# wyf-ACCEPT/BackToReality

Measured on NVIDIA B200. Metric: Pointnet2Backbone fwd+bwd scenes/sec @40k pts, higher is better.
Workload: dtype tf32 fwd / bf16 bwd operands, f32 accumulate

## Files before the change

### backtoreality_b200/_lib.py

```python
import ctypes
import os

_HERE = os.path.dirname(os.path.abspath(__file__))
LIB_PATH = os.environ.get("B2R_LIB") or os.path.join(_HERE, "libb2r.so")

_vp = ctypes.c_void_p
_i = ctypes.c_int
_f = ctypes.c_float
_ip = ctypes.POINTER(ctypes.c_int)

SIGNATURES = {
    "b2r_version": [],
    "b2r_status_string": [_i],
    "b2r_last_error": [],
    "b2r_struct_bytes": [_i],
    "b2r_ref_block_threads": [_i],
    "b2r_fps": [_vp, _i, _i, _i, _vp, _vp],
    "b2r_fps_ex": [_vp, _i, _i, _i, _vp, _i, _vp],
    "b2r_fps_plan": [_i, _i, _ip, _ip, _ip, _ip],
    "b2r_fps_workspace_bytes": [_i, _i],
    "b2r_fps_ws": [_vp, _i, _i, _i, _vp, _i, _vp, ctypes.c_longlong, _vp],
    "b2r_fps_sort": [_vp, _i, _i, _vp, ctypes.c_longlong, _vp],
    "b2r_fps_ws_presorted": [_vp, _i, _i, _i, _vp, _i, _vp, ctypes.c_longlong, _vp],
    "b2r_gather_fwd": [_vp, _vp, _i, _i, _i, _i, _vp, _vp],
    "b2r_gather_bwd": [_vp, _vp, _i, _i, _i, _i, _vp, _vp],
    "b2r_ball_query": [_vp, _vp, _i, _i, _i, _f, _i, _vp, _vp],
    "b2r_ball_query_workspace_bytes": [_i, _i],
    "b2r_ball_query_grid": [_vp, _vp, _i, _i, _i, _f, _i, _vp, _vp, ctypes.c_longlong, _vp],
    "b2r_group_fwd": [_vp, _vp, _i, _i, _i, _i, _i, _vp, _vp],
    "b2r_group_bwd": [_vp, _vp, _i, _i, _i, _i, _i, _vp, _vp],
    "b2r_three_nn": [_vp, _vp, _i, _i, _i, _vp, _vp, _vp],
    "b2r_three_interp_fwd": [_vp, _vp, _vp, _i, _i, _i, _i, _vp, _vp],
    "b2r_three_interp_bwd": [_vp, _vp, _vp, _i, _i, _i, _i, _vp, _vp],
    "b2r_scatter_plan_bytes": [_i, ctypes.c_longlong, _i, _i, _i],
    "b2r_scatter_plan": [_vp, _vp, _i, ctypes.c_longlong, _i, _i, _vp, ctypes.c_longlong, _vp],
    "b2r_group_bwd_plan": [_vp, _vp, _i, _i, _i, _i, _i, _vp, _vp],
    "b2r_three_interp_bwd_plan": [_vp, _vp, _i, _i, _i, _i, _vp, _vp],
    "b2r_adam_state_bytes": [],
    "b2r_adam_flat_step": [_vp, _vp, _vp, _vp, ctypes.c_longlong, _vp, _f, _f, _f, _f, _f, _f, _vp],
    "b2r_nn_argmin": [_vp, _vp, _i, _i, _i, _i, _i, _f, _vp, _vp, _vp],
    "b2r_query_group_fwd": [_vp, _vp, _vp, _vp, _i, _i, _i, _i, _i, _f, _i, _vp, _vp],
    "b2r_query_group_bwd": [_vp, _vp, _i, _i, _i, _i, _i, _f, _i, _vp, _vp, _vp, _vp],
}
_RESTYPES = {"b2r_status_string": ctypes.c_char_p, "b2r_last_error": ctypes.c_char_p,
             "b2r_fps_workspace_bytes": ctypes.c_longlong,
             "b2r_scatter_plan_bytes": ctypes.c_longlong,
             "b2r_ball_query_workspace_bytes": ctypes.c_longlong,
             "b2r_mlp_weight_image_bytes": ctypes.c_longlong}


class SaLayer(ctypes.Structure):
    _fields_ = [
        ("B", _i), ("N", _i), ("NP", _i), ("NS", _i), ("Cin", _i), ("Cout", _i),
        ("mode", _i), ("epilogue", _i),
        ("xyz", _vp), ("new_xyz", _vp), ("feat_t", _vp), ("idx", _vp),
        ("radius", _f), ("normalize_xyz", _i),
        ("z_prev", _vp), ("scale_prev", _vp), ("shift_prev", _vp),
        ("w_image", _vp), ("z", _vp), ("stats", _vp),
        ("zmax", _vp), ("zmin", _vp), ("amax", _vp), ("amin", _vp),
        ("sm_limit", _i),
        ("cidx", _vp), ("ccen", _vp), ("cmeta", _vp),
    ]


SIGNATURES.update({
    "b2r_mlp_weight_image_bytes": [_i, _i, _i],
    "b2r_mlp_pack_weight": [_vp, _i, _i, _i, _vp, _vp],
    "b2r_sa_layer_fwd": [ctypes.POINTER(SaLayer), _vp],
    "b2r_sa_layer_fwd_supported": [_i, _i, _i, _i, _i, _i, _i],
    "b2r_bn_finalize": [_vp, _i, ctypes.c_double, _vp, _vp, _f, _f, _vp, _vp, _vp, _vp, _vp, _vp,
                        _vp, _vp],
    "b2r_pool_finalize": [_vp, _vp, _vp, _vp, _i, _i, _i, _vp, _vp, _vp],
    "b2r_to_point_major": [_vp, _i, _i, _i, _vp, _vp],
})



class SaLayerBwd(ctypes.Structure):
    _fields_ = [
        ("B", _i), ("N", _i), ("NP", _i), ("NS", _i), ("Cin", _i), ("Cout", _i), ("mode", _i),
        ("xyz", _vp), ("new_xyz", _vp), ("feat_t", _vp), ("idx", _vp),
        ("radius", _f), ("normalize_xyz", _i),
        ("z_prev", _vp), ("scale_prev", _vp), ("shift_prev", _vp),
        ("w_image_bf16", _vp), ("dz", _vp), ("gr", _vp), ("z", _vp),
        ("dysel", _vp), ("asel", _vp),
        ("coef_a", _vp), ("coef_b", _vp), ("coef_c", _vp),
        ("dW", _vp), ("gr_prev", _vp), ("stats_prev", _vp),
        ("g_feat_t", _vp), ("g_xyz", _vp), ("g_new_xyz", _vp),
        ("sm_limit", _i),
        ("cidx", _vp), ("ccen", _vp), ("cmeta", _vp),
    ]


SIGNATURES.update({
    "b2r_mlp_weight_bf16_image_bytes": [_i, _i, _i],
    "b2r_mlp_pack_weight_bf16": [_vp, _i, _i, _i, _vp, _vp],
    "b2r_sa_layer_bwd": [ctypes.POINTER(SaLayerBwd), _vp],
    "b2r_sa_layer_bwd_supported": [_i, _i, _i, _i, _i, _i, _i],
    "b2r_pool_bwd_prep": [_vp, _vp, _vp, _vp, _vp, _vp, _vp, _vp, _i, _i, _i, _vp, _vp, _vp, _vp],
    "b2r_bn_bwd_finalize": [_vp, _i, ctypes.c_double, _vp, _vp, _vp, _i, _vp, _vp, _vp, _vp, _vp,
                            _vp, _vp, _vp, _vp],
})
_RESTYPES["b2r_mlp_weight_bf16_image_bytes"] = ctypes.c_longlong

SIGNATURES.update({
    "b2r_compact_capacity": [_i, _i, _i],
    "b2r_compact_workspace_bytes": [_i, _i],
    "b2r_compact_plan": [_vp, _i, _i, _i, _i, _vp, _vp, _vp, _vp, _vp],
    "b2r_sa_layer_fwd_tile": [_i] * 8,
    "b2r_sa_layer_bwd_tile": [_i] * 9,
})
_RESTYPES["b2r_compact_capacity"] = ctypes.c_longlong
_RESTYPES["b2r_compact_workspace_bytes"] = ctypes.c_longlong



class DenseLayer(ctypes.Structure):
    _fields_ = [
        ("M", _i), ("Cin", _i), ("Cout", _i),
        ("in_", _vp), ("ld_in", _i), ("sc_in", _vp), ("sh_in", _vp),
        ("w_img", _vp), ("bias", _vp), ("z", _vp), ("ld_z", _i), ("stats", _vp),
    ]


class DenseLayerBwd(ctypes.Structure):
    _fields_ = [
        ("M", _i), ("Cin", _i), ("Cout", _i),
        ("in_", _vp), ("ld_in", _i), ("sc_in", _vp), ("sh_in", _vp),
        ("g", _vp), ("zz", _vp), ("ld_g", _i),
        ("ca", _vp), ("cb", _vp), ("cc", _vp),
        ("wt_img", _vp), ("gin", _vp), ("ld_gin", _i), ("stats_in", _vp), ("dW", _vp),
    ]


_ll = ctypes.c_longlong
SIGNATURES.update({
    "b2r_bn_bwd_finalize_ex": [_vp, _i, ctypes.c_double, _vp, _vp, _vp, _i, _vp, _vp, _vp, _vp, _vp,
                               _vp, _vp, _vp, _vp, _vp],
    "b2r_dense_image_bytes": [_i, _i],
    "b2r_dense_pack": [_vp, _i, _i, _vp, _vp, _vp],
    "b2r_dense_fwd": [ctypes.POINTER(DenseLayer), _vp],
    "b2r_dense_bwd": [ctypes.POINTER(DenseLayerBwd), _vp],
    "b2r_interp_cat_fwd": [_vp, _vp, _vp, _vp, _i, _i, _i, _i, _i, _vp, _vp],
    "b2r_interp_cat_bwd": [_vp, _i, _vp, _vp, _i, _i, _i, _i, _i, _vp, _vp, _vp],
    "b2r_vote_tail_fwd": [_vp, _i, _vp, _vp, _ll, _i, _vp, _vp, _vp, _vp],
    "b2r_vote_tail_bwd": [_vp, _vp, _vp, _vp, _ll, _i, _i, _vp, _vp, _vp],
})
_RESTYPES["b2r_dense_image_bytes"] = ctypes.c_longlong

_lib = None


class B2RError(RuntimeError):
    """A libb2r call returned a negative status."""


def lib():
    global _lib
    if _lib is None:
        if not os.path.isfile(LIB_PATH):
            raise ImportError(
                "libb2r.so not found at %s -- build it with "
                "`python -c 'import __graft_entry__ as g; g.build()'` "
                "(there is no CPU or PyTorch fallback for these ops)" % LIB_PATH)
        l = ctypes.CDLL(LIB_PATH)
        for name, argtypes in SIGNATURES.items():
            fn = getattr(l, name)
            fn.argtypes = argtypes
            fn.restype = _RESTYPES.get(name, ctypes.c_int)
        _lib = l
    return _lib


def check(status, what):
    if status != 0:
        l = lib()
        raise B2RError("%s failed: %s (%s)" % (
            what, l.b2r_status_string(status).decode(), l.b2r_last_error().decode()))
```

### backtoreality_b200/csrc/mlp.cu

```cuda
#include "mlp_common.cuh"

namespace b2r {
using namespace mlp;
namespace {

__global__ void pack_weight_kernel(const float *__restrict__ w, int Cout, int Cin, int gather,
                                   int Kp, int Cout_pad, float *__restrict__ image) {
  const int KA = (Kp + 31) >> 5;
  const long long total = (long long)Cout_pad * KA * 32;
  for (long long e = (long long)blockIdx.x * blockDim.x + threadIdx.x; e < total;
       e += (long long)gridDim.x * blockDim.x) {
    const int m = (int)(e / (KA * 32)), kp = (int)(e % (KA * 32));
    float v = 0.f;
    if (m < Cout && kp < Kp) {
      int k = -1;
      if (gather) {
        const int C = Cin - 3, Cf4 = (C + 3) & ~3;
        if (kp < C) k = 3 + kp;
        else if (kp >= Cf4 && kp < Cf4 + 3) k = kp - Cf4;
      } else if (kp < Cin) {
        k = kp;
      }
      if (k >= 0) v = __uint_as_float(to_tf32(w[(size_t)m * Cin + k]));
    }
    const uint32_t off = sw128_off(m, kp >> 2, Cout_pad) + (kp & 3) * 4;
    image[off >> 2] = v;
  }
}

struct LayerArgs {
  int B, N, NP, NS, Cin, Cout, mode, epilogue;
  const float *xyz, *new_xyz, *feat_t;
  const int *idx;
  float radius;
  int normalize_xyz;
  const float *z_prev, *scale_prev, *shift_prev;
  const float *w_image;
  float *z;
  double *stats;
  float *zmax, *zmin;
  int *amax, *amin;
  int Kp, Cout_pad, num_tiles, chf_shift, ns_shift, raw_stage;
  const int *cidx, *ccen, *cmeta;
};

constexpr int kFwdEpiThreads = 256, kFwdProdThreads = 224, kFwdMmaWarp = 8;
constexpr int kFwdThreads = kFwdEpiThreads + 32 + kFwdProdThreads;

struct FwdSmem {
  uint32_t w_off, w_bytes, x_off[2], x_bytes, raw_off[2], raw_bytes, scale_off, idx_off, cen_off,
      bar_off, total;
};
__host__ __device__ inline FwdSmem fwd_smem_layout(int Kp, int Cout_pad, int NT, int raw_cin,
                                                   int cmp = 0) {
  FwdSmem s;
  const uint32_t KA = (uint32_t)(Kp + 31) >> 5;
  s.w_off = 0;
  s.w_bytes = (uint32_t)Cout_pad * KA * 128u;
  s.x_bytes = (uint32_t)NT * KA * 128u;
  s.x_off[0] = s.w_bytes;
  s.x_off[1] = s.w_bytes + s.x_bytes;
  s.raw_bytes = (uint32_t)NT * raw_cin * 4u;
  s.raw_off[0] = s.x_off[1] + s.x_bytes;
  s.raw_off[1] = s.raw_off[0] + s.raw_bytes;
  s.scale_off = s.raw_off[1] + s.raw_bytes;
  s.idx_off = s.scale_off + 2u * Kp * 4u;
  s.cen_off = s.idx_off + (uint32_t)NT * 4u;
  s.bar_off = (s.cen_off + (cmp ? 3u * (uint32_t)NT * 4u + 32u : 0u) + 15u) & ~15u;
  s.total = s.bar_off + 11 * 8 + 16 + 1024;
  return s;
}
__device__ __forceinline__ void fwd_bar_epi() {
  asm volatile("bar.sync 1, %0;" ::"n"(kFwdEpiThreads));
}
__device__ __forceinline__ void fwd_bar_prod() {
  asm volatile("bar.sync 2, %0;" ::"n"(kFwdProdThreads));
}
__device__ __forceinline__ void mbar_arrive1(uint32_t bar) {
  asm volatile("mbarrier.arrive.shared::cta.b64 _, [%0];" ::"r"(bar) : "memory");
}

template <int NT, bool CMP>
__global__ void __launch_bounds__(kFwdThreads, 1) sa_layer_fwd_kernel(const LayerArgs a) {
  extern __shared__ __align__(1024) uint8_t smem_raw[];
  uint8_t *base = reinterpret_cast<uint8_t *>((reinterpret_cast<uintptr_t>(smem_raw) + 1023) &
                                              ~(uintptr_t)1023);
  const FwdSmem L = fwd_smem_layout(a.Kp, a.Cout_pad, NT, a.raw_stage ? a.Cin : 0, CMP ? 1 : 0);
  uint8_t *s_w = base + L.w_off;
  float *s_scale = reinterpret_cast<float *>(base + L.scale_off);
  float *s_shift = s_scale + a.Kp;
  int *s_idx = reinterpret_cast<int *>(base + L.idx_off);
  int *s_cenp = reinterpret_cast<int *>(base + L.cen_off);
  int *s_cene = s_cenp + NT;
  int *s_meta = s_cene + 2 * NT;
  uint64_t *s_bar = reinterpret_cast<uint64_t *>(base + L.bar_off);
  uint32_t *s_tmem = reinterpret_cast<uint32_t *>(s_bar + 11);
  auto bar = [&](int i) { return smem_u32(&s_bar[i]); };

  const int tid = threadIdx.x, warp = tid >> 5, lane = tid & 31;
  const int MT = a.Cout_pad >> 7;
  constexpr int NCH = NT / 32;
  constexpr uint32_t kTmemCols = 512;
  const int grid = (int)gridDim.x;
  int num_tiles = a.num_tiles;
  if constexpr (CMP) {
    num_tiles = __ldg(a.cmeta + 8) / NT;
    if (tid < 8) s_meta[tid] = __ldg(a.cmeta + tid);
  }

  if (tid == 0) {
    for (int i = 0; i < 11; ++i) mbar_init(bar(i), 1);
    asm volatile("fence.mbarrier_init.release.cluster;" ::: "memory");
  }
  if (warp == kFwdMmaWarp) tmem_alloc(smem_u32(s_tmem), kTmemCols);
  for (uint32_t i = tid * 16; i < 2u * L.x_bytes; i += kFwdThreads * 16)
    *reinterpret_cast<uint4 *>(base + L.x_off[0] + i) = make_uint4(0, 0, 0, 0);
  if (a.mode == 1)
    for (int i = tid; i < a.Cin; i += kFwdThreads) {
      s_scale[i] = a.scale_prev[i];
      s_shift[i] = a.shift_prev[i];
    }
  fence_async_smem();
  tc_fence_before();
  __syncthreads();
  tc_fence_after();
  const uint32_t tmem_base = *s_tmem;
  if (tid == 0) {
    mbar_expect_tx(bar(8), L.w_bytes);
    bulk_g2s(smem_u32(s_w), a.w_image, L.w_bytes, bar(8));
  }

  if (warp > kFwdMmaWarp) {
    const int ptid = tid - (kFwdEpiThreads + 32);
    const long long per_scene = (long long)a.NP * a.NS;
    GatherSrc gsrc;
    gsrc.xyz = a.xyz; gsrc.new_xyz = a.new_xyz; gsrc.feat_t = a.feat_t;
    gsrc.N = a.N; gsrc.NP = a.NP; gsrc.NS = a.NS; gsrc.C = a.Cin - 3;
    gsrc.Cf4 = (a.Cin - 3 + 3) & ~3;
    gsrc.chf_shift = a.chf_shift; gsrc.radius = a.radius; gsrc.normalize_xyz = a.normalize_xyz;
    if (a.raw_stage && ptid == 0) {
      for (int k = 0; k < 2; ++k) {
        const long long tile = (long long)blockIdx.x + (long long)k * grid;
        if (tile < num_tiles) {
          mbar_expect_tx(bar(9 + k), L.raw_bytes);
          bulk_g2s(smem_u32(base + L.raw_off[k]), a.z_prev + (size_t)(tile * NT) * a.Cin,
                   L.raw_bytes, bar(9 + k));
        }
      }
    }
    int nidx = 0, ncen = 0;
    for (int k = 0, tile = blockIdx.x; tile < num_tiles; tile += grid, ++k) {
      const int s = k & 1, n = k >> 1;
      mbar_wait(bar(2 + s), (uint32_t)((n & 1) ^ 1));
      const long long pos0 = (long long)tile * NT;
      uint8_t *sx = base + L.x_off[s];
      if (CMP && a.mode == 0) {
        if (ptid < NT) {
          s_idx[ptid] = (k == 0) ? a.cidx[pos0 + ptid] : nidx;
          s_cenp[ptid] = (k == 0) ? a.ccen[pos0 + ptid] : ncen;
          if (tile + grid < num_tiles) {
            nidx = __ldg(a.cidx + pos0 + (long long)grid * NT + ptid);
            ncen = __ldg(a.ccen + pos0 + (long long)grid * NT + ptid);
          }
        }
        fwd_bar_prod();
        build_x_gather<NT, kFwdProdThreads>(gsrc, 0, 0, s_idx, sx, ptid,
                                            [](int row, int ch) { return sw128_off(row, ch, NT); },
                                            s_cenp);
      } else if (a.mode == 0) {
        if (ptid < NT) {
          s_idx[ptid] = (k == 0) ? a.idx[pos0 + ptid] : nidx;
          if (tile + grid < num_tiles) nidx = __ldg(a.idx + pos0 + (long long)grid * NT + ptid);
        }
        fwd_bar_prod();
        const int b = (int)(pos0 / per_scene);
        const int in_scene0 = (int)(pos0 - (long long)b * per_scene);
        build_x_gather<NT, kFwdProdThreads>(gsrc, b, in_scene0, s_idx, sx, ptid,
                                            [](int row, int ch) { return sw128_off(row, ch, NT); });
      } else if (a.raw_stage) {
        const int CH = a.Cin >> 2;
        const int total = NT * CH;
        const int chs = (CH & (CH - 1)) == 0 ? 31 - __clz(CH) : -1;
        mbar_wait(bar(9 + s), (uint32_t)(n & 1));
        const float4 *src = reinterpret_cast<const float4 *>(base + L.raw_off[s]);
        for (int i = ptid; i < total; i += kFwdProdThreads) {
          const float4 t = src[i];
          const int row = chs >= 0 ? (i >> chs) : (i / CH), ch = i - row * CH;
          const float4 sc = *reinterpret_cast<const float4 *>(s_scale + ch * 4);
          const float4 sh = *reinterpret_cast<const float4 *>(s_shift + ch * 4);
          uint4 out;
          out.x = to_tf32(fmaxf(fmaf(t.x, sc.x, sh.x), 0.f));
          out.y = to_tf32(fmaxf(fmaf(t.y, sc.y, sh.y), 0.f));
          out.z = to_tf32(fmaxf(fmaf(t.z, sc.z, sh.z), 0.f));
          out.w = to_tf32(fmaxf(fmaf(t.w, sc.w, sh.w), 0.f));
          *reinterpret_cast<uint4 *>(sx + sw128_off(row, ch, NT)) = out;
        }
      } else {
        const int CH = a.Cin >> 2;
        const int total = NT * CH;
        const int chs = (CH & (CH - 1)) == 0 ? 31 - __clz(CH) : -1;
        if (ptid == 0 && tile + 2 * grid < num_tiles)
          prefetch_l2(a.z_prev + (size_t)(pos0 + 2ll * grid * NT) * a.Cin, (uint32_t)total * 16u);
        const float4 *src = reinterpret_cast<const float4 *>(a.z_prev + (size_t)pos0 * a.Cin);
        for (int i0 = ptid; i0 < total; i0 += kFwdProdThreads * 8) {
          float4 t[8];
#pragma unroll
          for (int u = 0; u < 8; ++u) {
            const int i = i0 + u * kFwdProdThreads;
            if (i < total) t[u] = __ldg(src + i);
          }
#pragma unroll
          for (int u = 0; u < 8; ++u) {
            const int i = i0 + u * kFwdProdThreads;
            if (i < total) {
              const int row = chs >= 0 ? (i >> chs) : (i / CH), ch = i - row * CH;
              const float4 sc = *reinterpret_cast<const float4 *>(s_scale + ch * 4);
              const float4 sh = *reinterpret_cast<const float4 *>(s_shift + ch * 4);
              uint4 out;
              out.x = to_tf32(fmaxf(fmaf(t[u].x, sc.x, sh.x), 0.f));
              out.y = to_tf32(fmaxf(fmaf(t[u].y, sc.y, sh.y), 0.f));
              out.z = to_tf32(fmaxf(fmaf(t[u].z, sc.z, sh.z), 0.f));
              out.w = to_tf32(fmaxf(fmaf(t[u].w, sc.w, sh.w), 0.f));
              *reinterpret_cast<uint4 *>(sx + sw128_off(row, ch, NT)) = out;
            }
          }
        }
      }
      fence_async_smem();
      fwd_bar_prod();
      if (ptid == 0) {
        mbar_arrive1(bar(0 + s));
        if (a.raw_stage && tile + 2 * grid < num_tiles) {
          mbar_expect_tx(bar(9 + s), L.raw_bytes);
          bulk_g2s(smem_u32(base + L.raw_off[s]),
                   a.z_prev + (size_t)(pos0 + 2ll * grid * NT) * a.Cin, L.raw_bytes, bar(9 + s));
        }
      }
    }
  } else if (warp == kFwdMmaWarp) {
    if (lane == 0) {
      mbar_wait(bar(8), 0);
      const uint32_t wa = smem_u32(s_w);
      const int KS = (a.Kp + 7) >> 3;
      const uint32_t idesc = idesc_tf32(NT);
      for (int k = 0, tile = blockIdx.x; tile < num_tiles; tile += grid, ++k) {
        const int s = k & 1, n = k >> 1;
        const uint32_t xa = smem_u32(base + L.x_off[s]);
        mbar_wait(bar(0 + s), (uint32_t)(n & 1));
        mbar_wait(bar(6 + s), (uint32_t)((n & 1) ^ 1));
        tc_fence_after();
        for (int m = 0; m < MT; ++m)
          for (int ks = 0; ks < KS; ++ks) {
            const uint32_t koff = (uint32_t)(ks >> 2) * 1024u;
            const uint64_t da = smem_desc_sw128(wa + koff * (uint32_t)(a.Cout_pad >> 3) +
                                                (uint32_t)m * 16u * 1024u + (uint32_t)(ks & 3) * 32u);
            const uint64_t db =
                smem_desc_sw128(xa + koff * (uint32_t)(NT >> 3) + (uint32_t)(ks & 3) * 32u);
            umma_tf32(tmem_base + (uint32_t)((s * MT + m) * NT), da, db, idesc, ks > 0 ? 1u : 0u);
          }
        umma_commit(bar(4 + s));
        umma_commit(bar(2 + s));
      }
    }
    __syncwarp();
  } else {
    const int q = warp & 3, h = warp >> 2;
    const uint32_t lane_addr = (uint32_t)(q * 32) << 16;
    double acc_s[2] = {0.0, 0.0}, acc_ss[2] = {0.0, 0.0};
    constexpr int kGroups = NT / 8;
    const bool split = a.epilogue == 0 || NT / 2 >= a.NS;
    const int sg_begin = split ? h * (kGroups / 2) : 0;
    const int sg_end = split ? sg_begin + kGroups / 2 : (h == 0 ? kGroups : 0);
    int ncen_e = -1;
    if constexpr (CMP) {
      if (a.epilogue == 1) {
        if (tid < NT)
          s_cene[tid] = ((int)blockIdx.x < num_tiles) ? a.ccen[(long long)blockIdx.x * NT + tid] : -1;
        fwd_bar_epi();
      }
    }
    for (int k = 0, tile = blockIdx.x; tile < num_tiles; tile += grid, ++k) {
      const int s = k & 1, n = k >> 1;
      const long long pos0 = (long long)tile * NT;
      TileClass tc;
      tc.ns = a.NS; tc.live = NT; tc.wx = 0.f;
      if constexpr (CMP) {
        tc = tile_class(s_meta, pos0, a.NS);
        if (a.epilogue == 1 && tid < NT && tile + grid < num_tiles)
          ncen_e = __ldg(a.ccen + pos0 + (long long)grid * NT + tid);
      }
      const int nsm = tc.ns - 1;
      const int p64 = (int)(pos0 & 63);
      mbar_wait(bar(4 + s), (uint32_t)(n & 1));
      tc_fence_after();
#pragma unroll
      for (int m = 0; m < 2; ++m) {
        if (m >= MT) continue;
        const int c = m * 128 + q * 32 + lane;
        const bool c_ok = c < a.Cout;
        float ts = 0.f, tss = 0.f;
        float mx = 0.f, mn = 0.f, mx1 = 0.f, mn1 = 0.f;
        int ax = 0, an = 0, ax1 = 0, an1 = 0;
        const uint32_t t0 = tmem_base + lane_addr + (uint32_t)((s * MT + m) * NT);
        auto process = [&](const uint32_t (&r)[8], int sg) {
          if (!c_ok) return;
          const int col0 = sg * 8;
          if (a.epilogue == 0) {
            float *zp = a.z + (size_t)(pos0 + col0) * a.Cout + c;
#pragma unroll
            for (int i = 0; i < 8; ++i) zp[(size_t)i * a.Cout] = __uint_as_float(r[i]);
          }
          if (col0 >= tc.live) return;
          const int s0 = (p64 + col0) & nsm;
          float t = 0.f, tt = 0.f, tb = 0.f, ttb = 0.f;
#pragma unroll
          for (int i = 0; i < 8; i += 2) {
            const float x = __uint_as_float(r[i]), y = __uint_as_float(r[i + 1]);
            t += x;
            tt = fmaf(x, x, tt);
            tb += y;
            ttb = fmaf(y, y, ttb);
          }
          t += tb;
          tt += ttb;
          if (CMP && s0 == 0) {
            const float x0 = __uint_as_float(r[0]);
            t = fmaf(tc.wx, x0, t);
            tt = fmaf(tc.wx * x0, x0, tt);
          }
          ts += t;
          tss += tt;
          if (a.epilogue == 1) {
            if (s0 == 0) {
              mx = mx1 = -INFINITY; mn = mn1 = INFINITY; ax = an = ax1 = an1 = 0;
            }
#pragma unroll
            for (int i = 0; i < 8; i += 2) {
              const float x = __uint_as_float(r[i]), y = __uint_as_float(r[i + 1]);
              if (x > mx) { mx = x; ax = s0 + i; }
              if (x < mn) { mn = x; an = s0 + i; }
              if (y > mx1) { mx1 = y; ax1 = s0 + i + 1; }
              if (y < mn1) { mn1 = y; an1 = s0 + i + 1; }
            }
            if (s0 + 8 == tc.ns) {
              if (mx1 > mx || (mx1 == mx && ax1 < ax)) { mx = mx1; ax = ax1; }
              if (mn1 < mn || (mn1 == mn && an1 < an)) { mn = mn1; an = an1; }
              long long centre;
              if constexpr (CMP) centre = s_cene[(k & 1) * NT + col0];
              else centre = (pos0 + col0) >> a.ns_shift;
              if (centre >= 0) {
                const size_t o = (size_t)centre * a.Cout + c;
                a.zmax[o] = mx; a.zmin[o] = mn; a.amax[o] = ax; a.amin[o] = an;
              }
            }
          }
        };
        uint32_t ra[8], rb[8];
        if (sg_begin < sg_end) cuda::ptx::tcgen05_ld_32x32b(ra, t0 + (uint32_t)(sg_begin * 8));
#pragma unroll 1
        for (int sg = sg_begin; sg < sg_end; sg += 2) {
          asm volatile("tcgen05.wait::ld.sync.aligned;" ::: "memory");
          if (sg + 1 < sg_end) cuda::ptx::tcgen05_ld_32x32b(rb, t0 + (uint32_t)((sg + 1) * 8));
          process(ra, sg);
          if (sg + 1 < sg_end) {
            asm volatile("tcgen05.wait::ld.sync.aligned;" ::: "memory");
            if (sg + 2 < sg_end) cuda::ptx::tcgen05_ld_32x32b(ra, t0 + (uint32_t)((sg + 2) * 8));
            process(rb, sg + 1);
          }
        }
        acc_s[m] += (double)ts;
        acc_ss[m] += (double)tss;
      }
      if constexpr (CMP) {
        if (a.epilogue == 1 && tid < NT) s_cene[((k + 1) & 1) * NT + tid] = ncen_e;
      }
      tc_fence_before();
      fwd_bar_epi();
      if (tid == 0) mbar_arrive1(bar(6 + s));
    }
    if (a.stats != nullptr) {
#pragma unroll
      for (int m = 0; m < 2; ++m) {
        const int c = m * 128 + q * 32 + lane;
        if (m < MT && c < a.Cout) {
          atomicAdd(a.stats + c, acc_s[m]);
          atomicAdd(a.stats + a.Cout + c, acc_ss[m]);
        }
      }
    }
  }
  tc_fence_before();
  __syncthreads();
  if (warp == kFwdMmaWarp) tmem_dealloc(tmem_base, kTmemCols);
}

__global__ void bn_finalize_kernel(const double *__restrict__ stats, int Cch, double inv_count,
                                   float unbias,
                                   const float *__restrict__ gamma, const float *__restrict__ beta,
                                   float eps, float momentum, float *__restrict__ running_mean,
                                   float *__restrict__ running_var, float *__restrict__ scale,
                                   float *__restrict__ shift, float *__restrict__ mean_out,
                                   float *__restrict__ invstd_out,
                                   long long *__restrict__ num_batches_tracked) {
  const int ch = blockIdx.x * blockDim.x + threadIdx.x;
  if (ch == 0 && num_batches_tracked != nullptr) *num_batches_tracked += 1;
  if (ch >= Cch) return;
  const double mean = stats[ch] * inv_count;
  double var = fma(stats[Cch + ch], inv_count, -mean * mean);
  if (var < 0.0) var = 0.0;
  const float invstd = 1.0f / sqrtf((float)var + eps);
  const float g = gamma ? gamma[ch] : 1.f, bta = beta ? beta[ch] : 0.f;
  scale[ch] = g * invstd;
  shift[ch] = bta - (float)mean * g * invstd;
  if (mean_out) mean_out[ch] = (float)mean;
  if (invstd_out) invstd_out[ch] = invstd;
  if (running_mean) {
    const float unbiased = (float)var * unbias;
    running_mean[ch] = (1.f - momentum) * running_mean[ch] + momentum * (float)mean;
    running_var[ch] = (1.f - momentum) * running_var[ch] + momentum * unbiased;
  }
}

__global__ void pool_finalize_kernel(const float *__restrict__ zmax, const float *__restrict__ zmin,
                                     const float *__restrict__ scale,
                                     const float *__restrict__ shift, int NP, int Cch,
                                     float *__restrict__ out_cm, float *__restrict__ out_pm) {
  __shared__ float t[32][33];
  const int b = blockIdx.z;
  const int j0 = blockIdx.x * 32, c0 = blockIdx.y * 32;
  const int ch = c0 + threadIdx.x;
  const float s = ch < Cch ? scale[ch] : 0.f, sh = ch < Cch ? shift[ch] : 0.f;
  for (int i = threadIdx.y; i < 32; i += blockDim.y) {
    const int j = j0 + i;
    float y = 0.f;
    if (j < NP && ch < Cch) {
      const size_t e = ((size_t)b * NP + j) * Cch + ch;
      const float z = s >= 0.f ? zmax[e] : zmin[e];
      y = fmaxf(fmaf(z, s, sh), 0.f);
      if (out_pm) out_pm[e] = y;
    }
    t[i][threadIdx.x] = y;
  }
  if (out_cm == nullptr) return;
  __syncthreads();
  for (int i = threadIdx.y; i < 32; i += blockDim.y) {
    const int cc = c0 + i, j = j0 + threadIdx.x;
    if (cc < Cch && j < NP) out_cm[((size_t)b * Cch + cc) * NP + j] = t[threadIdx.x][i];
  }
}

__global__ void to_point_major_kernel(const float *__restrict__ in, int Cch, int N,
                                      float *__restrict__ out) {
  __shared__ float t[32][33];
  const int b = blockIdx.z;
  const int n0 = blockIdx.x * 32, c0 = blockIdx.y * 32;
  in += (size_t)b * Cch * N;
  out += (size_t)b * Cch * N;
  for (int i = threadIdx.y; i < 32; i += blockDim.y) {
    const int cc = c0 + i, n = n0 + threadIdx.x;
    t[i][threadIdx.x] = (cc < Cch && n < N) ? in[(size_t)cc * N + n] : 0.f;
  }
  __syncthreads();
  for (int i = threadIdx.y; i < 32; i += blockDim.y) {
    const int n = n0 + i, cc = c0 + threadIdx.x;
    if (n < N && cc < Cch) out[(size_t)n * Cch + cc] = t[threadIdx.x][i];
  }
}

}
}

using namespace b2r;

extern "C" long long b2r_mlp_weight_image_bytes(int Cout, int Cin, int gather) {
  if (Cout <= 0 || Cin <= 0) return 0;
  const int Kp = packed_k(Cin, gather);
  const int KA = (Kp + 31) >> 5;
  const int Cout_pad = (Cout + 127) & ~127;
  return (long long)Cout_pad * KA * 128;
}

extern "C" int b2r_mlp_pack_weight(const float *w, int Cout, int Cin, int gather, float *image,
                                   void *stream) {
  B2R_REQUIRE(w && image && Cout > 0 && Cin > 0, "b2r_mlp_pack_weight: bad argument");
  B2R_REQUIRE(!gather || Cin >= 3, "b2r_mlp_pack_weight: gather layers need Cin >= 3");
  const int Kp = packed_k(Cin, gather);
  const int KA = (Kp + 31) >> 5;
  const int Cout_pad = (Cout + 127) & ~127;
  const long long total = (long long)Cout_pad * KA * 32;
  pack_weight_kernel<<<ceil_div(total, 256), 256, 0, static_cast<cudaStream_t>(stream)>>>(
      w, Cout, Cin, gather, Kp, Cout_pad, image);
  B2R_CHECK_LAUNCH();
  return B2R_OK;
}

namespace {
int fwd_pick_nt(int Kp, int Cout_pad, int Cin, int mode, int epilogue, int NS, long long M,
                long long per_scene, int *raw_stage, int cmp = 0) {
  const int MT = Cout_pad >> 7;
  for (int raw = (mode == 1 ? 1 : 0); raw >= 0; --raw)
    for (int nt : {128, 64, 32}) {
      if (M % nt) continue;
      if (!cmp && mode == 0 && per_scene % nt) continue;
      if (epilogue == 1 && (nt % NS) != 0) continue;
      if (raw && nt < 64) continue;
      const FwdSmem L = fwd_smem_layout(Kp, Cout_pad, nt, raw ? Cin : 0, cmp);
      if (L.total <= 227u * 1024u && 2 * MT * nt <= 512) {
        *raw_stage = raw;
        return nt;
      }
    }
  *raw_stage = 0;
  return 0;
}
}

extern "C" int b2r_sa_layer_fwd_supported(int B, int NP, int NS, int Cin, int Cout, int gather,
                                          int pooled) {
  if (B <= 0 || NP <= 0 || NS <= 0 || Cin <= 0 || Cout <= 0 || Cout > 256) return 0;
  if (gather ? Cin < 3 : (Cin % 4) != 0) return 0;
  if (pooled && !(NS == 16 || NS == 32 || NS == 64)) return 0;
  const long long per_scene = (long long)NP * NS, M = (long long)B * per_scene;
  int raw = 0;
  return fwd_pick_nt(packed_k(Cin, gather), (Cout + 127) & ~127, Cin, gather ? 0 : 1,
                     pooled ? 1 : 0, NS, M, per_scene, &raw) > 0 ? 1 : 0;
}

extern "C" int b2r_sa_layer_fwd_tile(int B, int NP, int NS, int Cin, int Cout, int gather,
                                     int pooled, int compact) {
  if (B <= 0 || NP <= 0 || NS <= 0 || Cin <= 0 || Cout <= 0 || Cout > 256) return 0;
  const long long per_scene = (long long)NP * NS;
  const long long M = compact ? b2r_compact_capacity(B, NP, NS) : (long long)B * per_scene;
  int raw = 0;
  return fwd_pick_nt(packed_k(Cin, gather), (Cout + 127) & ~127, Cin, gather ? 0 : 1,
                     pooled ? 1 : 0, NS, M, per_scene, &raw, compact ? 1 : 0);
}

extern "C" int b2r_sa_layer_fwd(const b2r_sa_layer *d, void *stream) {
  B2R_REQUIRE(d != nullptr, "b2r_sa_layer_fwd: null descriptor");
  B2R_REQUIRE(d->B > 0 && d->NP > 0 && d->NS > 0 && d->Cin > 0 && d->Cout > 0,
              "b2r_sa_layer_fwd: non-positive size");
  B2R_REQUIRE(d->mode == 0 || d->mode == 1, "b2r_sa_layer_fwd: mode must be 0 or 1");
  B2R_REQUIRE(d->epilogue == 0 || d->epilogue == 1, "b2r_sa_layer_fwd: epilogue must be 0 or 1");
  B2R_REQUIRE(d->w_image != nullptr, "b2r_sa_layer_fwd: null weight image");
  LayerArgs a;
  a.B = d->B; a.N = d->N; a.NP = d->NP; a.NS = d->NS; a.Cin = d->Cin; a.Cout = d->Cout;
  a.mode = d->mode; a.epilogue = d->epilogue;
  a.xyz = d->xyz; a.new_xyz = d->new_xyz; a.feat_t = d->feat_t; a.idx = d->idx;
  a.radius = d->radius; a.normalize_xyz = d->normalize_xyz;
  a.z_prev = d->z_prev; a.scale_prev = d->scale_prev; a.shift_prev = d->shift_prev;
  a.w_image = d->w_image; a.z = d->z; a.stats = d->stats;
  a.zmax = d->zmax; a.zmin = d->zmin; a.amax = d->amax; a.amin = d->amin;
  a.Kp = packed_k(d->Cin, d->mode == 0);
  a.Cout_pad = (d->Cout + 127) & ~127;
  a.chf_shift = pow2_shift(((d->Cin - 3 + 3) & ~3) >> 2);
  a.ns_shift = pow2_shift(d->NS);
  a.cidx = d->cidx; a.ccen = d->ccen; a.cmeta = d->cmeta;
  const int cmp = d->cmeta != nullptr ? 1 : 0;
  B2R_REQUIRE(!cmp || (d->cidx && d->ccen), "b2r_sa_layer_fwd: a plan needs cidx, ccen and cmeta");
  if (cmp && !(d->NS == 16 || d->NS == 32 || d->NS == 64)) {
    set_error("b2r_sa_layer_fwd: a compacted plan needs nsample 16/32/64 (got %d)", d->NS);
    return B2R_ERR_UNSUPPORTED;
  }
  const long long M = cmp ? b2r_compact_capacity(d->B, d->NP, d->NS)
                          : (long long)d->B * d->NP * d->NS;
  const long long per_scene = (long long)d->NP * d->NS;
  if (d->mode == 0) {
    B2R_REQUIRE(d->Cin >= 3 && d->xyz && d->new_xyz && (d->idx || cmp) && (d->feat_t || d->Cin == 3),
                "b2r_sa_layer_fwd: gather mode needs xyz, new_xyz, idx (and feat_t when Cin > 3)");
    B2R_REQUIRE(d->Cin == 3 || ((reinterpret_cast<uintptr_t>(d->feat_t) & 15u) == 0),
                "b2r_sa_layer_fwd: feat_t must be 16-byte aligned");
  } else {
    B2R_REQUIRE(d->z_prev && d->scale_prev && d->shift_prev && (d->Cin % 4) == 0,
                "b2r_sa_layer_fwd: dense mode needs z_prev/scale/shift and Cin %% 4 == 0");
  }
  if (d->epilogue == 0) {
    B2R_REQUIRE(d->z != nullptr, "b2r_sa_layer_fwd: epilogue 0 needs z");
  } else {
    B2R_REQUIRE(d->zmax && d->zmin && d->amax && d->amin,
                "b2r_sa_layer_fwd: epilogue 1 needs pool outputs");
    if (!(d->NS == 16 || d->NS == 32 || d->NS == 64)) {
      set_error("b2r_sa_layer_fwd: pooling supports nsample 16/32/64 (got %d)", d->NS);
      return B2R_ERR_UNSUPPORTED;
    }
  }
  if (a.Cout_pad > 256) {
    set_error("b2r_sa_layer_fwd: needs Cout <= 256 (got %d)", d->Cout);
    return B2R_ERR_UNSUPPORTED;
  }
  if (thin::fwd_applicable(d)) return thin::fwd_launch(d, stream);
  const int NT = fwd_pick_nt(a.Kp, a.Cout_pad, d->Cin, d->mode, d->epilogue, d->NS, M, per_scene,
                             &a.raw_stage, cmp);
  if (NT == 0) {
    set_error("b2r_sa_layer_fwd: layer Cin=%d Cout=%d M=%lld NP*NS=%lld does not fit (needs "
              "B*NP*NS %% 32 == 0, gather layers NP*NS %% 32 == 0, operands within 227 KB)",
              d->Cin, d->Cout, M, per_scene);
    return B2R_ERR_UNSUPPORTED;
  }
  const FwdSmem L = fwd_smem_layout(a.Kp, a.Cout_pad, NT, a.raw_stage ? d->Cin : 0, cmp);
  a.num_tiles = (int)(M / NT);
  int sms = kNumSMs;
  if (d->sm_limit > 0 && d->sm_limit < kNumSMs) sms = d->sm_limit;
  const int grid = a.num_tiles < sms ? a.num_tiles : sms;
  cudaStream_t st = static_cast<cudaStream_t>(stream);
#define B2R_LAUNCH_FWD(NTV, CMPV)                                                               \
  do {                                                                                          \
    B2R_CUDA(cudaFuncSetAttribute(sa_layer_fwd_kernel<NTV, CMPV>,                               \
                                  cudaFuncAttributeMaxDynamicSharedMemorySize, (int)L.total));  \
    sa_layer_fwd_kernel<NTV, CMPV><<<grid, kFwdThreads, L.total, st>>>(a);                      \
  } while (0)
  if (cmp) {
    if (NT == 128) B2R_LAUNCH_FWD(128, true);
    else if (NT == 64) B2R_LAUNCH_FWD(64, true);
    else B2R_LAUNCH_FWD(32, true);
  } else {
    if (NT == 128) B2R_LAUNCH_FWD(128, false);
    else if (NT == 64) B2R_LAUNCH_FWD(64, false);
    else B2R_LAUNCH_FWD(32, false);
  }
#undef B2R_LAUNCH_FWD
  B2R_CHECK_LAUNCH();
  return B2R_OK;
}

extern "C" int b2r_bn_finalize(const double *stats, int C, double count, const float *gamma,
                               const float *beta, float eps, float momentum, float *running_mean,
                               float *running_var, float *scale, float *shift, float *mean_out,
                               float *invstd_out, long long *num_batches_tracked, void *stream) {
  B2R_REQUIRE(stats && scale && shift && C > 0 && count > 0, "b2r_bn_finalize: bad argument");
  bn_finalize_kernel<<<ceil_div(C, 128), 128, 0, static_cast<cudaStream_t>(stream)>>>(
      stats, C, 1.0 / count, count > 1.0 ? (float)(count / (count - 1.0)) : 1.0f, gamma, beta, eps,
      momentum, running_mean, running_var, scale, shift,
      mean_out, invstd_out, num_batches_tracked);
  B2R_CHECK_LAUNCH();
  return B2R_OK;
}

extern "C" int b2r_pool_finalize(const float *zmax, const float *zmin, const float *scale,
                                 const float *shift, int B, int NP, int C, float *out_cm,
                                 float *out_pm, void *stream) {
  B2R_REQUIRE(zmax && zmin && scale && shift && B > 0 && NP > 0 && C > 0,
              "b2r_pool_finalize: bad argument");
  B2R_REQUIRE(B <= 65535, "b2r_pool_finalize: B=%d exceeds gridDim.z", B);
  dim3 grid(ceil_div(NP, 32), ceil_div(C, 32), B), block(32, 8);
  pool_finalize_kernel<<<grid, block, 0, static_cast<cudaStream_t>(stream)>>>(
      zmax, zmin, scale, shift, NP, C, out_cm, out_pm);
  B2R_CHECK_LAUNCH();
  return B2R_OK;
}

extern "C" int b2r_to_point_major(const float *in, int B, int C, int N, float *out, void *stream) {
  B2R_REQUIRE(B >= 0 && C >= 0 && N >= 0, "b2r_to_point_major: negative size");
  if (B == 0 || C == 0 || N == 0) return B2R_OK;
  B2R_REQUIRE(in && out, "b2r_to_point_major: null pointer");
  dim3 grid(ceil_div(N, 32), ceil_div(C, 32), B), block(32, 8);
  to_point_major_kernel<<<grid, block, 0, static_cast<cudaStream_t>(stream)>>>(in, C, N, out);
  B2R_CHECK_LAUNCH();
  return B2R_OK;
}
```

### backtoreality_b200/csrc/mlp_bwd.cu

```cuda
#include <cuda_bf16.h>

#include "mlp_common.cuh"

namespace b2r {
using namespace mlp;
namespace {

constexpr int kBwdWarps = 12;
constexpr int kBwdThreads = kBwdWarps * 32;

struct BwdArgs {
  int B, N, NP, NS, Cin, Cout, mode, top;
  const float *xyz, *new_xyz, *feat_t;
  const int *idx;
  float radius;
  int normalize_xyz;
  const float *z_prev, *scale_prev, *shift_prev;
  const void *w_image;
  const float *dz;
  const float *gr, *z;
  const float *dysel;
  const int *asel;
  const float *coef_a, *coef_b, *coef_c;
  float *dW;
  float *gr_prev;
  double *stats_prev;
  float *g_feat_t, *g_xyz, *g_new_xyz;
  int do_dgrad;
  int Kp, KA, WA, Cout_pad, num_tiles;
  int ch8_shift;
  int ns_shift;
  const int *cidx, *ccen, *cmeta;
};

__host__ __device__ inline int packed_k16(int Cin, int gather) {
  if (!gather) return (Cin + 7) & ~7;
  return ((Cin - 3 + 7) & ~7) + 8;
}

struct BwdSmem {
  uint32_t w_off, w_bytes, x_off[2], dz_off[2], x_bytes, dz_bytes, coef_off, scale_off, idx_off,
      cen_off, meta_off, route_off, flush_off, bar_off, total;
};
__host__ __device__ inline BwdSmem bwd_smem_layout(int Kp, int KA, int WA, int Cout, int Cout_pad,
                                                   int NT, int top, int cmp = 0) {
  BwdSmem s;
  s.w_off = 0;
  s.w_bytes = (uint32_t)Cout_pad * WA * 128u;
  s.x_bytes = (uint32_t)NT * KA * 128u;
  s.dz_bytes = (uint32_t)NT * (Cout_pad >> 6) * 128u;
  uint32_t o = s.w_bytes;
  for (int st = 0; st < 2; ++st) {
    s.x_off[st] = o;
    o += s.x_bytes;
    s.dz_off[st] = o;
    o += s.dz_bytes;
  }
  s.coef_off = o;
  s.scale_off = s.coef_off + 3u * Cout * 4u;
  s.idx_off = s.scale_off + 2u * Kp * 4u;
  s.cen_off = s.idx_off + 4u * (uint32_t)NT * 4u;
  s.meta_off = s.cen_off + (cmp ? 4u * (uint32_t)NT * 4u : 0u);
  s.route_off = (s.meta_off + (cmp ? 32u : 0u) + 15u) & ~15u;
  s.flush_off = s.route_off +
                (top ? 4u * (uint32_t)(NT / (cmp ? 8 : 16)) * Cout_pad * 4u : 0u);
  const uint32_t flush_bytes = 8u * 32u * 33u * 4u;
  if (cmp && 2u * (s.x_bytes + s.dz_bytes) >= flush_bytes) {
    s.bar_off = s.flush_off;
    s.flush_off = s.x_off[0];
  } else {
    s.bar_off = s.flush_off + flush_bytes;
  }
  s.total = s.bar_off + 13 * 8 + 16 + 1024;
  return s;
}

__device__ __forceinline__ uint32_t bf_off(int row, int chunk, int rows) {
  const int a = chunk >> 3, c = chunk & 7, g = row >> 3, r8 = row & 7;
  return (uint32_t)(((a * (rows >> 3) + g) << 10) + (r8 << 7) + ((c ^ r8) << 4));
}
__host__ __device__ constexpr uint32_t idesc_bf16(int n, int a_mn, int b_mn) {
  return (1u << 4) | (1u << 7) | (1u << 10) | ((uint32_t)a_mn << 15) | ((uint32_t)b_mn << 16) |
         ((uint32_t)(n >> 3) << 17) | ((128u >> 4) << 24);
}
__device__ __forceinline__ void umma_bf16(uint32_t d_tmem, uint64_t a_desc, uint64_t b_desc,
                                          uint32_t idesc, uint32_t accumulate) {
  asm volatile(
      "{\n\t"
      ".reg .pred p;\n\t"
      "setp.ne.b32 p, %4, 0;\n\t"
      "tcgen05.mma.cta_group::1.kind::f16 [%0], %1, %2, %3, p;\n\t"
      "}" ::"r"(d_tmem),
      "l"(a_desc), "l"(b_desc), "r"(idesc), "r"(accumulate)
      : "memory");
}
__device__ __forceinline__ void mbar_arrive(uint32_t bar) {
  asm volatile("mbarrier.arrive.shared::cta.b64 _, [%0];" ::"r"(bar) : "memory");
}
__device__ __forceinline__ uint32_t pack_bf16(float lo, float hi) {
  const __nv_bfloat162 v = __floats2bfloat162_rn(lo, hi);
  return *reinterpret_cast<const uint32_t *>(&v);
}
template <int N>
__device__ __forceinline__ void bar_named(int id) {
  asm volatile("bar.sync %0, %1;" ::"r"(id), "n"(N));
}

__global__ void pack_weight_bf16_kernel(const float *__restrict__ w, int Cout, int Cin, int gather,
                                        int Kp, int Cout_pad, int WA,
                                        __nv_bfloat16 *__restrict__ image) {
  const long long total = (long long)Cout_pad * WA * 64;
  for (long long e = (long long)blockIdx.x * blockDim.x + threadIdx.x; e < total;
       e += (long long)gridDim.x * blockDim.x) {
    const int co = (int)(e / (WA * 64)), kp = (int)(e % (WA * 64));
    float v = 0.f;
    if (co < Cout && kp < Kp) {
      int k = -1;
      if (gather) {
        const int C = Cin - 3, Cf8 = (C + 7) & ~7;
        if (kp < C) k = 3 + kp;
        else if (kp >= Cf8 && kp < Cf8 + 3) k = kp - Cf8;
      } else if (kp < Cin) {
        k = kp;
      }
      if (k >= 0) v = w[(size_t)co * Cin + k];
    }
    image[(bf_off(co, kp >> 3, Cout_pad) >> 1) + (kp & 7)] = __float2bfloat16_rn(v);
  }
}

template <int NT, int EW, int MODE, int TOP, bool CMP>
__global__ void __launch_bounds__(kBwdThreads, 1) sa_layer_bwd_kernel(const BwdArgs a) {
  constexpr int kMode = MODE;
  constexpr bool kTop = TOP != 0;
  constexpr int kRC = CMP ? NT / 8 : NT / 16;
  constexpr int kEpiThreads = EW * 32, kProdThreads = (kBwdWarps - 1 - EW) * 32;
  auto bar_epi = [] { bar_named<kEpiThreads>(1); };
  auto bar_prod = [] { bar_named<kProdThreads>(2); };
  extern __shared__ __align__(1024) uint8_t smem_raw[];
  uint8_t *base = reinterpret_cast<uint8_t *>((reinterpret_cast<uintptr_t>(smem_raw) + 1023) &
                                              ~(uintptr_t)1023);
  const BwdSmem L = bwd_smem_layout(a.Kp, a.KA, a.WA, a.Cout, a.Cout_pad, NT, kTop, CMP ? 1 : 0);
  uint8_t *s_w = base + L.w_off;
  float *s_ca = reinterpret_cast<float *>(base + L.coef_off);
  float *s_cb = s_ca + a.Cout;
  float *s_cc = s_cb + a.Cout;
  float *s_scale = reinterpret_cast<float *>(base + L.scale_off);
  float *s_shift = s_scale + a.Kp;
  int *s_idx4 = reinterpret_cast<int *>(base + L.idx_off);
  int *s_cen4 = reinterpret_cast<int *>(base + L.cen_off);
  int *s_meta = reinterpret_cast<int *>(base + L.meta_off);
  float *s_dy = reinterpret_cast<float *>(base + L.route_off);
  int *s_as = reinterpret_cast<int *>(s_dy + 2 * kRC * a.Cout_pad);
  uint64_t *s_bar = reinterpret_cast<uint64_t *>(base + L.bar_off);
  uint32_t *s_tmem = reinterpret_cast<uint32_t *>(s_bar + 13);
  auto bar = [&](int i) { return smem_u32(&s_bar[i]); };

  const int tid = threadIdx.x, warp = tid >> 5, lane = tid & 31;
  const int KA = a.KA;
  const int MTp = (KA + 1) >> 1;
  const int MTl = a.Cout_pad >> 7;
  constexpr int NCH = NT / 32;
  const bool has_coef = a.dz == nullptr;
  const int w12 = ((kTop && MTl > (a.do_dgrad ? MTp : 0)) ? MTl : (a.do_dgrad ? MTp : 0)) * NT;
  const uint32_t d3_col0 = 2u * (uint32_t)w12;
  constexpr uint32_t kTmemCols = 512;
  const long long per_scene = (long long)a.NP * a.NS;
  const int C = a.Cin - 3, Cf8 = (C + 7) & ~7;
  int num_tiles = a.num_tiles;
  if constexpr (CMP) {
    num_tiles = __ldg(a.cmeta + 8) / NT;
    if (tid < 8) s_meta[tid] = __ldg(a.cmeta + tid);
  }

  if (tid == 0) {
    for (int i = 0; i < 13; ++i)
      mbar_init(bar(i), (i == 0 || i == 1) ? (uint32_t)(kProdThreads / 32)
                        : (i == 10 || i == 11) ? (uint32_t)EW : 1u);
    asm volatile("fence.mbarrier_init.release.cluster;" ::: "memory");
  }
  if (warp == EW) tmem_alloc(smem_u32(s_tmem), kTmemCols);
  {
    const uint32_t zb = 2u * (L.x_bytes + L.dz_bytes);
    for (uint32_t i = tid * 16; i < zb; i += kBwdThreads * 16)
      *reinterpret_cast<uint4 *>(base + L.x_off[0] + i) = make_uint4(0, 0, 0, 0);
  }
  if (kMode == 1)
    for (int i = tid; i < a.Cin; i += kBwdThreads) {
      s_scale[i] = a.scale_prev[i];
      s_shift[i] = a.shift_prev[i];
    }
  if (has_coef)
    for (int i = tid; i < a.Cout; i += kBwdThreads) {
      s_ca[i] = a.coef_a[i];
      s_cb[i] = a.coef_b[i];
      s_cc[i] = a.coef_c[i];
    }
  fence_async_smem();
  tc_fence_before();
  __syncthreads();
  tc_fence_after();
  const uint32_t tmem_base = *s_tmem;
  const bool need_w = kTop || a.do_dgrad;
  if (tid == 0 && need_w) {
    mbar_expect_tx(bar(12), L.w_bytes);
    bulk_g2s(smem_u32(s_w), a.w_image, L.w_bytes, bar(12));
  }
  const int grid = (int)gridDim.x;

  if (warp > EW) {
    const int ptid = tid - (kEpiThreads + 32);
    const int CH8 = a.Cout >> 3;
    const int ch8s = (CH8 & (CH8 - 1)) == 0 ? 31 - __clz(CH8) : -1;
    const int CHx = a.Cin >> 3;
    const int chxs = (CHx > 0 && (CHx & (CHx - 1)) == 0) ? 31 - __clz(CHx) : -1;
    int nidx = 0, ncen = 0;
    for (int k = 0, tile = blockIdx.x; tile < num_tiles; tile += grid, ++k) {
      const int s = k & 1, n = k >> 1;
      mbar_wait(bar(2 + s), (uint32_t)((n & 1) ^ 1));
      const long long pos0 = (long long)tile * NT;
      uint8_t *sx = base + L.x_off[s], *sdz = base + L.dz_off[s];
      int *s_idx = s_idx4 + (k & 3) * NT;
      int *s_cen = s_cen4 + (k & 3) * NT;
      TileClass tc{};
      int p64 = 0;
      if constexpr (CMP) {
        tc = tile_class(s_meta, pos0, a.NS);
        p64 = (int)(pos0 & 63);
      }
      if (ptid == 0 && tile + 2 * grid < num_tiles) {
        const size_t pn = (size_t)(pos0 + 2ll * grid * NT);
        if (!kTop) {
          if (!has_coef) prefetch_l2(a.dz + pn * a.Cout, (uint32_t)NT * a.Cout * 4u);
          else {
            prefetch_l2(a.gr + pn * a.Cout, (uint32_t)NT * a.Cout * 4u);
            prefetch_l2(a.z + pn * a.Cout, (uint32_t)NT * a.Cout * 4u);
          }
        }
        if (kMode == 1) prefetch_l2(a.z_prev + pn * a.Cin, (uint32_t)NT * a.Cin * 4u);
      }
      if (!kTop) {
        const int total = NT * CH8;
        const size_t o0 = (size_t)pos0 * a.Cout;
        for (int i0 = ptid; i0 < total; i0 += kProdThreads * 4) {
          float4 g[4][2], zz[4][2];
#pragma unroll
          for (int u = 0; u < 4; ++u) {
            const int i = i0 + u * kProdThreads;
            if (i < total) {
              if (!has_coef) {
                const float4 *p = reinterpret_cast<const float4 *>(a.dz + o0) + 2 * i;
                g[u][0] = __ldg(p); g[u][1] = __ldg(p + 1);
              } else {
                const float4 *p = reinterpret_cast<const float4 *>(a.gr + o0) + 2 * i;
                const float4 *qz = reinterpret_cast<const float4 *>(a.z + o0) + 2 * i;
                g[u][0] = __ldg(p); g[u][1] = __ldg(p + 1);
                zz[u][0] = __ldg(qz); zz[u][1] = __ldg(qz + 1);
              }
            }
          }
#pragma unroll
          for (int u = 0; u < 4; ++u) {
            const int i = i0 + u * kProdThreads;
            if (i < total) {
              const int row = ch8s >= 0 ? (i >> ch8s) : (i / CH8), ch = i - row * CH8;
              float v[8] = {g[u][0].x, g[u][0].y, g[u][0].z, g[u][0].w,
                            g[u][1].x, g[u][1].y, g[u][1].z, g[u][1].w};
              if (has_coef) {
                const float zv[8] = {zz[u][0].x, zz[u][0].y, zz[u][0].z, zz[u][0].w,
                                     zz[u][1].x, zz[u][1].y, zz[u][1].z, zz[u][1].w};
                float ca8[8], cb8[8], cc8[8];
                *reinterpret_cast<float4 *>(ca8) = *reinterpret_cast<const float4 *>(s_ca + ch * 8);
                *reinterpret_cast<float4 *>(ca8 + 4) = *reinterpret_cast<const float4 *>(s_ca + ch * 8 + 4);
                *reinterpret_cast<float4 *>(cb8) = *reinterpret_cast<const float4 *>(s_cb + ch * 8);
                *reinterpret_cast<float4 *>(cb8 + 4) = *reinterpret_cast<const float4 *>(s_cb + ch * 8 + 4);
                *reinterpret_cast<float4 *>(cc8) = *reinterpret_cast<const float4 *>(s_cc + ch * 8);
                *reinterpret_cast<float4 *>(cc8 + 4) = *reinterpret_cast<const float4 *>(s_cc + ch * 8 + 4);
                if constexpr (CMP) {
                  const float wgt = row < tc.live
                                        ? ((((p64 + row) & (tc.ns - 1)) == 0) ? 1.f + tc.wx : 1.f)
                                        : 0.f;
#pragma unroll
                  for (int e = 0; e < 8; ++e)
                    v[e] = fmaf(ca8[e], v[e], wgt * fmaf(cb8[e], zv[e], cc8[e]));
                } else {
#pragma unroll
                  for (int e = 0; e < 8; ++e) v[e] = fmaf(ca8[e], v[e], fmaf(cb8[e], zv[e], cc8[e]));
                }
              }
              *reinterpret_cast<uint4 *>(sdz + bf_off(row, ch, NT)) =
                  make_uint4(pack_bf16(v[0], v[1]), pack_bf16(v[2], v[3]), pack_bf16(v[4], v[5]),
                             pack_bf16(v[6], v[7]));
            }
          }
        }
      }
      if (kMode == 0) {
        if constexpr (kProdThreads < NT) {
          for (int r = ptid; r < NT; r += kProdThreads) {
            if constexpr (CMP) {
              s_idx[r] = __ldg(a.cidx + pos0 + r);
              s_cen[r] = __ldg(a.ccen + pos0 + r);
            } else {
              s_idx[r] = __ldg(a.idx + pos0 + r);
            }
          }
        } else if (ptid < NT) {
          if constexpr (CMP) {
            s_idx[ptid] = (k == 0) ? a.cidx[pos0 + ptid] : nidx;
            s_cen[ptid] = (k == 0) ? a.ccen[pos0 + ptid] : ncen;
            if (tile + grid < num_tiles) {
              nidx = __ldg(a.cidx + pos0 + (long long)grid * NT + ptid);
              ncen = __ldg(a.ccen + pos0 + (long long)grid * NT + ptid);
            }
          } else {
            s_idx[ptid] = (k == 0) ? a.idx[pos0 + ptid] : nidx;
            if (tile + grid < num_tiles) nidx = __ldg(a.idx + pos0 + (long long)grid * NT + ptid);
          }
        }
        bar_prod();
        const int b = CMP ? 0 : (int)(pos0 / per_scene);
        const int in_scene0 = CMP ? 0 : (int)(pos0 - (long long)b * per_scene);
        const int CH8f = Cf8 >> 3;
        for (int row = ptid; row < NT; row += kProdThreads) {
          const int p = s_idx[row];
          const int j = CMP ? max(s_cen[row], 0) : (in_scene0 + row) / a.NS;
          const float *pp = a.xyz + ((size_t)b * a.N + p) * 3;
          const float *qq = a.new_xyz + ((size_t)b * a.NP + j) * 3;
          const float px = __ldg(pp), py = __ldg(pp + 1), pz = __ldg(pp + 2);
          const float qx = __ldg(qq), qy = __ldg(qq + 1), qz = __ldg(qq + 2);
          float d0 = __fsub_rn(px, qx), d1 = __fsub_rn(py, qy), d2 = __fsub_rn(pz, qz);
          if (a.normalize_xyz) {
            d0 = __fdiv_rn(d0, a.radius);
            d1 = __fdiv_rn(d1, a.radius);
            d2 = __fdiv_rn(d2, a.radius);
          }
          *reinterpret_cast<uint4 *>(sx + bf_off(row, CH8f, NT)) =
              make_uint4(pack_bf16(d0, d1), pack_bf16(d2, 0.f), 0u, 0u);
        }
        if (CH8f > 0) {
          const float *fb = a.feat_t + (size_t)b * a.N * C;
          const int total = NT * CH8f;
          if ((C & 7) == 0) {
            for (int i0 = ptid; i0 < total; i0 += kProdThreads * 4) {
              float4 t[4][2];
#pragma unroll
              for (int u = 0; u < 4; ++u) {
                const int i = i0 + u * kProdThreads;
                if (i < total) {
                  const int row = a.ch8_shift >= 0 ? (i >> a.ch8_shift) : (i / CH8f);
                  const int ch = i - row * CH8f;
                  const float4 *p =
                      reinterpret_cast<const float4 *>(fb + (size_t)s_idx[row] * C) + 2 * ch;
                  t[u][0] = __ldg(p); t[u][1] = __ldg(p + 1);
                }
              }
#pragma unroll
              for (int u = 0; u < 4; ++u) {
                const int i = i0 + u * kProdThreads;
                if (i < total) {
                  const int row = a.ch8_shift >= 0 ? (i >> a.ch8_shift) : (i / CH8f);
                  const int ch = i - row * CH8f;
                  *reinterpret_cast<uint4 *>(sx + bf_off(row, ch, NT)) =
                      make_uint4(pack_bf16(t[u][0].x, t[u][0].y), pack_bf16(t[u][0].z, t[u][0].w),
                                 pack_bf16(t[u][1].x, t[u][1].y), pack_bf16(t[u][1].z, t[u][1].w));
                }
              }
            }
          } else {
            for (int i = ptid; i < total; i += kProdThreads) {
              const int row = i / CH8f, ch = i - row * CH8f;
              const float *src = fb + (size_t)s_idx[row] * C + ch * 8;
              float f[8];
#pragma unroll
              for (int e = 0; e < 8; ++e) f[e] = (ch * 8 + e < C) ? __ldg(src + e) : 0.f;
              *reinterpret_cast<uint4 *>(sx + bf_off(row, ch, NT)) =
                  make_uint4(pack_bf16(f[0], f[1]), pack_bf16(f[2], f[3]), pack_bf16(f[4], f[5]),
                             pack_bf16(f[6], f[7]));
            }
          }
        }
      } else {
        const int CH = a.Cin >> 3;
        const int total = NT * CH;
        const float4 *src = reinterpret_cast<const float4 *>(a.z_prev + (size_t)pos0 * a.Cin);
        for (int i0 = ptid; i0 < total; i0 += kProdThreads * 4) {
          float4 t[4][2];
#pragma unroll
          for (int u = 0; u < 4; ++u) {
            const int i = i0 + u * kProdThreads;
            if (i < total) { t[u][0] = __ldg(src + 2 * i); t[u][1] = __ldg(src + 2 * i + 1); }
          }
#pragma unroll
          for (int u = 0; u < 4; ++u) {
            const int i = i0 + u * kProdThreads;
            if (i < total) {
              const int row = chxs >= 0 ? (i >> chxs) : (i / CH), ch = i - row * CH;
              const float *sc = s_scale + ch * 8, *sh = s_shift + ch * 8;
              const float x0 = fmaxf(fmaf(t[u][0].x, sc[0], sh[0]), 0.f);
              const float x1 = fmaxf(fmaf(t[u][0].y, sc[1], sh[1]), 0.f);
              const float x2 = fmaxf(fmaf(t[u][0].z, sc[2], sh[2]), 0.f);
              const float x3 = fmaxf(fmaf(t[u][0].w, sc[3], sh[3]), 0.f);
              const float x4 = fmaxf(fmaf(t[u][1].x, sc[4], sh[4]), 0.f);
              const float x5 = fmaxf(fmaf(t[u][1].y, sc[5], sh[5]), 0.f);
              const float x6 = fmaxf(fmaf(t[u][1].z, sc[6], sh[6]), 0.f);
              const float x7 = fmaxf(fmaf(t[u][1].w, sc[7], sh[7]), 0.f);
              *reinterpret_cast<uint4 *>(sx + bf_off(row, ch, NT)) =
                  make_uint4(pack_bf16(x0, x1), pack_bf16(x2, x3), pack_bf16(x4, x5),
                             pack_bf16(x6, x7));
            }
          }
        }
      }
      fence_async_smem();
      __syncwarp();
      if (lane == 0) mbar_arrive(bar(0 + s));
    }
  } else if (warp == EW) {
    if (lane == 0) {
      if (need_w) mbar_wait(bar(12), 0);
      const uint32_t wa = smem_u32(s_w);
      const uint32_t lbo_w = (uint32_t)(a.Cout_pad >> 3) * 1024u;
      const uint32_t lbo_t = (uint32_t)(NT >> 3) * 1024u;
      const int KS16 = (a.Kp + 15) >> 4, KSl16 = (a.Cout + 15) >> 4;
      for (int k = 0, tile = blockIdx.x; tile < num_tiles; tile += grid, ++k) {
        const int s = k & 1, n = k >> 1;
        const uint32_t xa = smem_u32(base + L.x_off[s]), dza = smem_u32(base + L.dz_off[s]);
        const uint32_t d12 = tmem_base + (uint32_t)(s * w12);
        mbar_wait(bar(0 + s), (uint32_t)(n & 1));
        mbar_wait(bar(10 + s), (uint32_t)((n & 1) ^ 1));
        tc_fence_after();
        if (kTop) {
          for (int ml = 0; ml < MTl; ++ml)
            for (int ks = 0; ks < KS16; ++ks) {
              const uint64_t ad = smem_desc_sw128(wa + (uint32_t)(ks >> 2) * lbo_w +
                                                  (uint32_t)ml * 16u * 1024u + (uint32_t)(ks & 3) * 32u);
              const uint64_t bd =
                  smem_desc_sw128(xa + (uint32_t)(ks >> 2) * lbo_t + (uint32_t)(ks & 3) * 32u);
              umma_bf16(d12 + (uint32_t)ml * NT, ad, bd, idesc_bf16(NT, 0, 0), ks > 0 ? 1u : 0u);
            }
          umma_commit(bar(4 + s));
          mbar_wait(bar(6 + s), (uint32_t)(n & 1));
          tc_fence_after();
        }
        if (a.do_dgrad) {
          for (int m = 0; m < MTp; ++m)
            for (int ks = 0; ks < KSl16; ++ks) {
              const uint64_t ad = smem_desc_sw128_mn(
                  wa + (uint32_t)(2 * m) * lbo_w + (uint32_t)ks * 2048u, lbo_w, 1024u);
              const uint64_t bd =
                  smem_desc_sw128(dza + (uint32_t)(ks >> 2) * lbo_t + (uint32_t)(ks & 3) * 32u);
              umma_bf16(d12 + (uint32_t)m * NT, ad, bd, idesc_bf16(NT, 1, 0), ks > 0 ? 1u : 0u);
            }
        }
        for (int ml = 0; ml < MTl; ++ml)
          for (int a0 = 0; a0 < KA; a0 += 4) {
            const int na = (KA - a0) < 4 ? (KA - a0) : 4;
            const uint32_t idw = idesc_bf16(na * 64, 1, 1);
            for (int k16 = 0; k16 < NT / 16; ++k16) {
              const uint64_t ad = smem_desc_sw128_mn(
                  dza + (uint32_t)(2 * ml) * lbo_t + (uint32_t)k16 * 2048u, lbo_t, 1024u);
              const uint64_t bd = smem_desc_sw128_mn(
                  xa + (uint32_t)a0 * lbo_t + (uint32_t)k16 * 2048u, lbo_t, 1024u);
              umma_bf16(tmem_base + d3_col0 + (uint32_t)(ml * KA + a0) * 64u, ad, bd, idw,
                        (k > 0 || k16 > 0) ? 1u : 0u);
            }
          }
        umma_commit(bar(8 + s));
        umma_commit(bar(2 + s));
      }
    }
    __syncwarp();
  } else {
    const int q = warp & 3, h = warp >> 2;
    const uint32_t lane_addr = (uint32_t)(q * 32) << 16;
    float s1[3] = {0.f, 0.f, 0.f}, s2[3] = {0.f, 0.f, 0.f};
    double d1[3] = {0.0, 0.0, 0.0}, d2[3] = {0.0, 0.0, 0.0};
    int ntiles = 0;
    auto fetch_route = [&](int k, int tile) {
      if (tile < num_tiles) {
        const int s = k & 1;
        const long long pos0 = (long long)tile * NT;
        int ns_t = a.NS, shift_t = a.ns_shift;
        if constexpr (CMP) {
          ns_t = tile_class(s_meta, pos0, a.NS).ns;
          shift_t = 31 - __clz(ns_t);
        }
        const long long centre0 = pos0 >> shift_t;
        const int base_s = (int)(pos0 & (ns_t - 1));
        const int ncen = ((base_s + NT - 1) >> shift_t) + 1;
        float *my_dy = s_dy + (size_t)s * kRC * a.Cout_pad;
        int *my_as = s_as + (size_t)s * kRC * a.Cout_pad;
        int cg_lane = -1;
        if constexpr (CMP) {
          if (lane < ncen) cg_lane = __ldg(a.ccen + pos0 + (lane == 0 ? 0 : lane * ns_t - base_s));
        }
        for (int c = 0; c < ncen; ++c) {
          long long cg = centre0 + c;
          if constexpr (CMP) cg = __shfl_sync(0xffffffffu, cg_lane, c);
          for (int ml = 0; ml < MTl; ++ml) {
            const int co = ml * 128 + q * 32 + lane;
            if (co < a.Cout) {
              if constexpr (CMP) {
                if (cg < 0) {
                  my_dy[c * a.Cout_pad + co] = 0.f;
                  my_as[c * a.Cout_pad + co] = -1;
                  continue;
                }
              }
              const size_t o = (size_t)cg * a.Cout + co;
              asm volatile("cp.async.ca.shared.global [%0], [%1], 4;" ::"r"(
                               smem_u32(my_dy + c * a.Cout_pad + co)),
                           "l"(a.dysel + o)
                           : "memory");
              asm volatile("cp.async.ca.shared.global [%0], [%1], 4;" ::"r"(
                               smem_u32(my_as + c * a.Cout_pad + co)),
                           "l"(a.asel + o)
                           : "memory");
            }
          }
        }
      }
      asm volatile("cp.async.commit_group;" ::: "memory");
    };
    auto produce_dz = [&](int k, int tile) {
      const int s = k & 1, n = k >> 1;
      const long long pos0 = (long long)tile * NT;
      const uint32_t d12 = tmem_base + (uint32_t)(s * w12);
      uint8_t *sdz = base + L.dz_off[s];
      TileClass tc{};
      int ns_t = a.NS, shift_t = a.ns_shift;
      if constexpr (CMP) {
        tc = tile_class(s_meta, pos0, a.NS);
        ns_t = tc.ns;
        shift_t = 31 - __clz(ns_t);
      }
      const int ns_mask = ns_t - 1;
      const int base_s = (int)(pos0 & ns_mask);
      const float *my_dy = s_dy + (size_t)s * kRC * a.Cout_pad;
      const int *my_as = s_as + (size_t)s * kRC * a.Cout_pad;
      asm volatile("cp.async.wait_group 1;" ::: "memory");
      mbar_wait(bar(4 + s), (uint32_t)(n & 1));
      tc_fence_after();
#pragma unroll
      for (int ml = 0; ml < 2; ++ml) {
        if (ml >= MTl) continue;
        const int co = ml * 128 + q * 32 + lane;
        const bool ok = co < a.Cout;
        const float ca = ok ? s_ca[co] : 0.f, cb = ok ? s_cb[co] : 0.f, cc = ok ? s_cc[co] : 0.f;
#pragma unroll
        for (int c0 = 0; c0 < NCH; c0 += (EW == 8 ? 2 : 1)) {
          const int ch = c0 + (EW == 8 ? h : 0);
          uint32_t r[32];
          cuda::ptx::tcgen05_ld_32x32b(r, d12 + lane_addr + (uint32_t)(ml * NT + ch * 32));
          asm volatile("tcgen05.wait::ld.sync.aligned;" ::: "memory");
          if (ok && CMP) {
#pragma unroll
            for (int sg = 0; sg < 4; ++sg) {
              const int colb = ch * 32 + sg * 8;
              const int t0 = base_s + colb;
              const int c = t0 >> shift_t;
              const int s0 = t0 & ns_mask;
              const float dyv = my_dy[c * a.Cout_pad + co];
              const int as = my_as[c * a.Cout_pad + co] - s0;
              const float w0 = colb < tc.live ? 1.f : 0.f;
#pragma unroll
              for (int i = 0; i < 8; ++i) {
                const float dy = (i == as) ? dyv : 0.f;
                const float wgt = (s0 + i == 0) ? w0 * (1.f + tc.wx) : w0;
                const float v =
                    fmaf(ca, dy, wgt * fmaf(cb, __uint_as_float(r[sg * 8 + i]), cc));
                *reinterpret_cast<__nv_bfloat16 *>(
                    sdz + bf_off(colb + i, co >> 3, NT) + (co & 7) * 2) = __float2bfloat16_rn(v);
              }
            }
          } else if (ok) {
#pragma unroll
            for (int hf = 0; hf < 2; ++hf) {
              const int t0 = base_s + ch * 32 + hf * 16;
              const int c = t0 >> a.ns_shift;
              const int s0 = t0 & ns_mask;
              const float dyv = my_dy[c * a.Cout_pad + co];
              const int as = my_as[c * a.Cout_pad + co] - s0;
#pragma unroll
              for (int i = 0; i < 16; ++i) {
                const float dy = (i == as) ? dyv : 0.f;
                const float v = fmaf(ca, dy, fmaf(cb, __uint_as_float(r[hf * 16 + i]), cc));
                *reinterpret_cast<__nv_bfloat16 *>(
                    sdz + bf_off(ch * 32 + hf * 16 + i, co >> 3, NT) + (co & 7) * 2) =
                    __float2bfloat16_rn(v);
              }
            }
          }
        }
      }
      tc_fence_before();
      fence_async_smem();
      bar_epi();
      if (tid == 0) mbar_arrive(bar(6 + s));
      fetch_route(k + 2, tile + 2 * grid);
    };
    if (kTop) {
      fetch_route(0, blockIdx.x);
      fetch_route(1, blockIdx.x + grid);
      if ((int)blockIdx.x < num_tiles) produce_dz(0, blockIdx.x);
    }
    for (int k = 0, tile = blockIdx.x; tile < num_tiles; tile += grid, ++k, ++ntiles) {
      const int s = k & 1, n = k >> 1;
      const long long pos0 = (long long)tile * NT;
      const uint32_t d12 = tmem_base + (uint32_t)(s * w12);
      const int *s_idx = s_idx4 + (k & 3) * NT;
      const int *s_cen = s_cen4 + (k & 3) * NT;
      if (kTop && tile + grid < num_tiles) produce_dz(k + 1, tile + grid);
      mbar_wait(bar(8 + s), (uint32_t)(n & 1));
      tc_fence_after();
      if (a.do_dgrad) {
        int tile_b = 0, in_scene0 = 0;
        if (kMode == 0 && !CMP) {
          tile_b = (int)(pos0 / per_scene);
          in_scene0 = (int)(pos0 - (long long)tile_b * per_scene);
        }
        int ns_t = a.NS;
        if constexpr (CMP) {
          if (kMode == 0) {
            ns_t = tile_class(s_meta, pos0, a.NS).ns;
            in_scene0 = (int)(pos0 & 63);
          }
        }
#pragma unroll
        for (int m = 0; m < 3; ++m) {
          if (m >= MTp) continue;
#pragma unroll
          for (int c0 = 0; c0 < NCH; c0 += (EW == 8 ? 2 : 1)) {
            const int cc = c0 + (EW == 8 ? h : 0);
            uint32_t r[32];
            cuda::ptx::tcgen05_ld_32x32b(r, d12 + lane_addr + (uint32_t)(m * NT + cc * 32));
            asm volatile("tcgen05.wait::ld.sync.aligned;" ::: "memory");
            const int kp = m * 128 + q * 32 + lane;
            const long long p0 = pos0 + cc * 32;
            if (kMode == 1) {
              if (kp < a.Cin) {
                const float sc = s_scale[kp], sh = s_shift[kp];
                const float *zp = a.z_prev + (size_t)p0 * a.Cin + kp;
                float *gp = a.gr_prev + (size_t)p0 * a.Cin + kp;
                float t1 = 0.f, t2 = 0.f;
                float zv[32];
#pragma unroll
                for (int i = 0; i < 32; ++i) zv[i] = __ldg(zp + (size_t)i * a.Cin);
#pragma unroll
                for (int i = 0; i < 32; ++i) {
                  const float g = fmaf(zv[i], sc, sh) > 0.f ? __uint_as_float(r[i]) : 0.f;
                  gp[(size_t)i * a.Cin] = g;
                  t1 += g;
                  t2 = fmaf(g, zv[i], t2);
                }
                s1[m] += t1;
                s2[m] += t2;
              }
            } else {
              const bool is_feat = kp < C;
              const int e = kp - Cf8;
              const bool is_xyz = (e >= 0 && e < 3);
              if (is_feat && a.g_feat_t != nullptr) {
                float *gb = a.g_feat_t + (size_t)tile_b * a.N * C + kp;
#pragma unroll
                for (int i = 0; i < 32; ++i)
                  atomicAdd(gb + (size_t)s_idx[cc * 32 + i] * C, __uint_as_float(r[i]));
              } else if (is_xyz && (a.g_xyz != nullptr || a.g_new_xyz != nullptr)) {
                float run = 0.f;
                float *gx = a.g_xyz != nullptr ? a.g_xyz + (size_t)tile_b * a.N * 3 + e : nullptr;
#pragma unroll
                for (int i = 0; i < 32; ++i) {
                  const int ins = in_scene0 + cc * 32 + i;
                  float v = __uint_as_float(r[i]);
                  if (a.normalize_xyz) v = __fdiv_rn(v, a.radius);
                  if (gx != nullptr) atomicAdd(gx + (size_t)s_idx[cc * 32 + i] * 3, v);
                  run += v;
                  if constexpr (CMP) {
                    if (((ins + 1) & (ns_t - 1)) == 0 || i == 31) {
                      const int cg = s_cen[cc * 32 + i];
                      if (a.g_new_xyz != nullptr && cg >= 0)
                        atomicAdd(a.g_new_xyz + (size_t)cg * 3 + e, -run);
                      run = 0.f;
                    }
                  } else if (((ins + 1) % a.NS) == 0 || i == 31) {
                    if (a.g_new_xyz != nullptr)
                      atomicAdd(a.g_new_xyz + ((size_t)tile_b * a.NP + ins / a.NS) * 3 + e, -run);
                    run = 0.f;
                  }
                }
              }
            }
          }
        }
        if (kMode == 1) {
#pragma unroll
          for (int m = 0; m < 3; ++m) {
            d1[m] += (double)s1[m];
            d2[m] += (double)s2[m];
            s1[m] = 0.f;
            s2[m] = 0.f;
          }
        }
      }
      tc_fence_before();
      __syncwarp();
      if (lane == 0) mbar_arrive(bar(10 + s));
    }

    if (a.do_dgrad && kMode == 1 && a.stats_prev != nullptr) {
#pragma unroll
      for (int m = 0; m < 3; ++m) {
        const int kp = m * 128 + q * 32 + lane;
        if (m < MTp && kp < a.Cin) {
          atomicAdd(a.stats_prev + kp, d1[m]);
          atomicAdd(a.stats_prev + a.Cin + kp, d2[m]);
        }
      }
    }
    if (ntiles > 0) {
      tc_fence_after();
      float *stg = reinterpret_cast<float *>(base + L.flush_off) + warp * (32 * 33);
      for (int ml = 0; ml < MTl; ++ml) {
        const int co0 = ml * 128 + q * 32;
        for (int at = (EW == 8 ? h : 0); at < KA * 2; at += (EW == 8 ? 2 : 1)) {
          uint32_t r[32];
          cuda::ptx::tcgen05_ld_32x32b(
              r, tmem_base + lane_addr + d3_col0 + (uint32_t)(ml * KA * 64 + at * 32));
          asm volatile("tcgen05.wait::ld.sync.aligned;" ::: "memory");
#pragma unroll
          for (int i = 0; i < 32; ++i) stg[lane * 33 + i] = __uint_as_float(r[i]);
          __syncwarp();
          const int kp = at * 32 + lane;
          int kk = -1;
          if (kMode == 0) {
            if (kp < C) kk = 3 + kp;
            else if (kp >= Cf8 && kp < Cf8 + 3) kk = kp - Cf8;
          } else if (kp < a.Cin) {
            kk = kp;
          }
          if (kk >= 0) {
            const int rows = min(32, a.Cout - co0);
            for (int rr = 0; rr < rows; ++rr)
              atomicAdd(a.dW + (size_t)(co0 + rr) * a.Cin + kk, stg[rr * 33 + lane]);
          }
          __syncwarp();
        }
      }
    }
  }
  tc_fence_before();
  __syncthreads();
  if (warp == EW) tmem_dealloc(tmem_base, kTmemCols);
}

__global__ void pool_bwd_prep_kernel(const float *__restrict__ dout_cm,
                                     const float *__restrict__ dout_pm,
                                     const float *__restrict__ zmax, const float *__restrict__ zmin,
                                     const int *__restrict__ amax, const int *__restrict__ amin,
                                     const float *__restrict__ scale,
                                     const float *__restrict__ shift, int NP, int Cch,
                                     float *__restrict__ dysel, int *__restrict__ asel,
                                     double *__restrict__ stats) {
  __shared__ float t[32][33];
  __shared__ double r1[8][32], r2[8][32];
  const int b = blockIdx.z;
  const int j0 = blockIdx.x * 32, c0 = blockIdx.y * 32;
  if (dout_cm != nullptr) {
    for (int i = threadIdx.y; i < 32; i += blockDim.y) {
      const int cc = c0 + i, j = j0 + threadIdx.x;
      t[i][threadIdx.x] = (cc < Cch && j < NP) ? dout_cm[((size_t)b * Cch + cc) * NP + j] : 0.f;
    }
    __syncthreads();
  }
  const int ch = c0 + threadIdx.x;
  const float s = ch < Cch ? scale[ch] : 0.f, sh = ch < Cch ? shift[ch] : 0.f;
  const bool pos = s >= 0.f;
  double a1 = 0.0, a2 = 0.0;
  for (int i = threadIdx.y; i < 32; i += blockDim.y) {
    const int j = j0 + i;
    if (j < NP && ch < Cch) {
      const size_t o = ((size_t)b * NP + j) * Cch + ch;
      const float zs = pos ? zmax[o] : zmin[o];
      const int as = pos ? amax[o] : amin[o];
      float g = dout_cm != nullptr ? t[threadIdx.x][i] : 0.f;
      if (dout_pm != nullptr) g += dout_pm[o];
      g = fmaf(zs, s, sh) > 0.f ? g : 0.f;
      dysel[o] = g;
      asel[o] = as;
      a1 += (double)g;
      a2 += (double)g * (double)zs;
    }
  }
  r1[threadIdx.y][threadIdx.x] = a1;
  r2[threadIdx.y][threadIdx.x] = a2;
  __syncthreads();
  if (threadIdx.y == 0 && ch < Cch) {
    for (int k = 1; k < 8; ++k) {
      a1 += r1[k][threadIdx.x];
      a2 += r2[k][threadIdx.x];
    }
    atomicAdd(stats + ch, a1);
    atomicAdd(stats + Cch + ch, a2);
  }
}

__global__ void bn_bwd_finalize_kernel(const double *__restrict__ stats, int Cch, double count,
                                       double inv_count,
                                       const float *__restrict__ gamma,
                                       const float *__restrict__ mean,
                                       const float *__restrict__ invstd, int training,
                                       float *__restrict__ coef_a, float *__restrict__ coef_b,
                                       float *__restrict__ coef_c, float *__restrict__ k1_out,
                                       float *__restrict__ k2_out, float *__restrict__ gs_out,
                                       float *__restrict__ dgamma, float *__restrict__ dbeta,
                                       float *__restrict__ dbias_conv) {
  const int ch = blockIdx.x * blockDim.x + threadIdx.x;
  if (ch >= Cch) return;
  const double S1 = stats[ch], S2 = stats[Cch + ch];
  const double mu = (double)mean[ch], is = (double)invstd[ch];
  const double g = gamma ? (double)gamma[ch] : 1.0;
  const double sx = (S2 - mu * S1) * is;
  const double gs = g * is;
  double k1 = 0.0, k2 = 0.0;
  if (training) {
    k1 = S1 * inv_count;
    k2 = sx * inv_count;
  }
  const double b = -gs * k2 * is;
  if (coef_a) coef_a[ch] = (float)gs;
  if (coef_b) coef_b[ch] = (float)b;
  if (coef_c) coef_c[ch] = (float)(-gs * k1 - b * mu);
  if (k1_out) k1_out[ch] = (float)k1;
  if (k2_out) k2_out[ch] = (float)k2;
  if (gs_out) gs_out[ch] = (float)gs;
  if (dgamma) dgamma[ch] = (float)sx;
  if (dbeta) dbeta[ch] = (float)S1;
  if (dbias_conv) dbias_conv[ch] = (float)(gs * S1 + count * (b * mu + (-gs * k1 - b * mu)));
}

}

}

using namespace b2r;

namespace {
struct Geometry {
  int Kp, KA, WA, Cout_pad;
};
Geometry bwd_geometry(int Cout, int Cin, int gather) {
  Geometry g;
  g.Kp = packed_k16(Cin, gather);
  g.KA = (g.Kp + 63) >> 6;
  const int MTp = (g.KA + 1) >> 1;
  g.WA = g.KA > 2 * MTp ? g.KA : 2 * MTp;
  g.Cout_pad = (Cout + 127) & ~127;
  return g;
}
}

namespace {
int bwd_pick_nt(const Geometry &g, int Cout, int mode, int top, int do_dgrad, int NS, long long M,
                long long per_scene, int cmp = 0) {
  const int MTp = (g.KA + 1) >> 1, MTl = g.Cout_pad >> 7;
  if (MTp > 3) return 0;
  for (int nt : {128, 64, 32}) {
    if (M % nt) continue;
    if (!cmp && mode == 0 && per_scene % nt) continue;
    if (top && (nt % NS) != 0 && (NS % nt) != 0) continue;
    const BwdSmem L = bwd_smem_layout(g.Kp, g.KA, g.WA, Cout, g.Cout_pad, nt, top, cmp);
    const int w12 = ((top && MTl > (do_dgrad ? MTp : 0)) ? MTl : (do_dgrad ? MTp : 0)) * nt;
    const int cols = 2 * w12 + MTl * g.KA * 64;
    if (L.total <= 227u * 1024u && cols <= 512) return nt;
  }
  return 0;
}
}

extern "C" int b2r_sa_layer_bwd_supported(int B, int NP, int NS, int Cin, int Cout, int gather,
                                          int top) {
  if (B <= 0 || NP <= 0 || NS <= 0 || Cin <= 0 || Cout <= 0) return 0;
  if (Cout > 256 || (Cout % 8) != 0 || (!gather && (Cin % 8) != 0) || (gather && Cin < 3)) return 0;
  if (top && pow2_shift(NS) < 0) return 0;
  const Geometry g = bwd_geometry(Cout, Cin, gather);
  const long long per_scene = (long long)NP * NS, M = (long long)B * per_scene;
  return bwd_pick_nt(g, Cout, gather ? 0 : 1, top, 1, NS, M, per_scene) > 0 ? 1 : 0;
}

extern "C" int b2r_sa_layer_bwd_tile(int B, int NP, int NS, int Cin, int Cout, int gather, int top,
                                     int dgrad, int compact) {
  if (B <= 0 || NP <= 0 || NS <= 0 || Cin <= 0 || Cout <= 0) return 0;
  const Geometry g = bwd_geometry(Cout, Cin, gather);
  const long long per_scene = (long long)NP * NS;
  const long long M = compact ? b2r_compact_capacity(B, NP, NS) : (long long)B * per_scene;
  return bwd_pick_nt(g, Cout, gather ? 0 : 1, top, dgrad, NS, M, per_scene, compact ? 1 : 0);
}

extern "C" long long b2r_mlp_weight_bf16_image_bytes(int Cout, int Cin, int gather) {
  if (Cout <= 0 || Cin <= 0) return 0;
  const Geometry g = bwd_geometry(Cout, Cin, gather);
  return (long long)g.Cout_pad * g.WA * 128;
}

extern "C" int b2r_mlp_pack_weight_bf16(const float *w, int Cout, int Cin, int gather, void *image,
                                        void *stream) {
  B2R_REQUIRE(w && image && Cout > 0 && Cin > 0, "b2r_mlp_pack_weight_bf16: bad argument");
  B2R_REQUIRE(!gather || Cin >= 3, "b2r_mlp_pack_weight_bf16: gather layers need Cin >= 3");
  const Geometry g = bwd_geometry(Cout, Cin, gather);
  const long long total = (long long)g.Cout_pad * g.WA * 64;
  pack_weight_bf16_kernel<<<ceil_div(total, 256), 256, 0, static_cast<cudaStream_t>(stream)>>>(
      w, Cout, Cin, gather, g.Kp, g.Cout_pad, g.WA, static_cast<__nv_bfloat16 *>(image));
  B2R_CHECK_LAUNCH();
  return B2R_OK;
}

extern "C" int b2r_sa_layer_bwd(const b2r_sa_layer_bwd_desc *d, void *stream) {
  B2R_REQUIRE(d != nullptr, "b2r_sa_layer_bwd: null descriptor");
  B2R_REQUIRE(d->B > 0 && d->NP > 0 && d->NS > 0 && d->Cin > 0 && d->Cout > 0,
              "b2r_sa_layer_bwd: non-positive size");
  B2R_REQUIRE(d->mode == 0 || d->mode == 1, "b2r_sa_layer_bwd: mode must be 0 or 1");
  B2R_REQUIRE(d->dW != nullptr, "b2r_sa_layer_bwd: null dW");
  const bool top = d->dysel != nullptr;
  B2R_REQUIRE(d->dz != nullptr || (d->coef_a && d->coef_b && d->coef_c &&
                                   ((d->gr && d->z) || (top && d->asel))),
              "b2r_sa_layer_bwd: needs dz, or gr + z + coef_a/b/c, or dysel + asel + coef_a/b/c");
  BwdArgs a;
  a.B = d->B; a.N = d->N; a.NP = d->NP; a.NS = d->NS; a.Cin = d->Cin; a.Cout = d->Cout;
  a.mode = d->mode;
  a.top = (d->dz == nullptr && top) ? 1 : 0;
  a.xyz = d->xyz; a.new_xyz = d->new_xyz; a.feat_t = d->feat_t; a.idx = d->idx;
  a.radius = d->radius; a.normalize_xyz = d->normalize_xyz;
  a.z_prev = d->z_prev; a.scale_prev = d->scale_prev; a.shift_prev = d->shift_prev;
  a.w_image = d->w_image_bf16;
  a.dz = d->dz; a.gr = d->gr; a.z = d->z; a.dysel = d->dysel; a.asel = d->asel;
  a.coef_a = d->coef_a; a.coef_b = d->coef_b; a.coef_c = d->coef_c;
  a.dW = d->dW; a.gr_prev = d->gr_prev; a.stats_prev = d->stats_prev;
  a.g_feat_t = d->g_feat_t; a.g_xyz = d->g_xyz; a.g_new_xyz = d->g_new_xyz;
  const Geometry g = bwd_geometry(d->Cout, d->Cin, d->mode == 0);
  a.Kp = g.Kp; a.KA = g.KA; a.WA = g.WA; a.Cout_pad = g.Cout_pad;
  a.ch8_shift = pow2_shift((((d->Cin - 3 + 7) & ~7) >> 3));
  a.ns_shift = pow2_shift(d->NS);
  a.cidx = d->cidx; a.ccen = d->ccen; a.cmeta = d->cmeta;
  const int cmp = d->cmeta != nullptr ? 1 : 0;
  B2R_REQUIRE(!cmp || (d->cidx && d->ccen), "b2r_sa_layer_bwd: a plan needs cidx, ccen and cmeta");
  if (cmp && !(d->NS == 16 || d->NS == 32 || d->NS == 64)) {
    set_error("b2r_sa_layer_bwd: a compacted plan needs nsample 16/32/64 (got %d)", d->NS);
    return B2R_ERR_UNSUPPORTED;
  }
  if (a.top && a.ns_shift < 0) {
    set_error("b2r_sa_layer_bwd: the pooled top layer needs a power-of-two nsample (got %d)", d->NS);
    return B2R_ERR_UNSUPPORTED;
  }
  a.num_tiles = 0;
  if (d->mode == 0) {
    B2R_REQUIRE(d->Cin >= 3 && d->xyz && d->new_xyz && (d->idx || cmp) && (d->feat_t || d->Cin == 3),
                "b2r_sa_layer_bwd: gather mode needs xyz, new_xyz, idx (and feat_t when Cin > 3)");
    a.do_dgrad = (d->g_feat_t != nullptr && d->Cin > 3) || d->g_xyz != nullptr ||
                 d->g_new_xyz != nullptr;
  } else {
    B2R_REQUIRE(d->z_prev && d->scale_prev && d->shift_prev,
                "b2r_sa_layer_bwd: dense mode needs z_prev/scale/shift");
    B2R_REQUIRE(d->gr_prev != nullptr, "b2r_sa_layer_bwd: dense mode needs gr_prev");
    a.do_dgrad = 1;
  }
  B2R_REQUIRE(!(a.do_dgrad || a.top) || d->w_image_bf16 != nullptr,
              "b2r_sa_layer_bwd: null weight image");
  if (thin::bwd_applicable(d)) return thin::bwd_launch(d, stream);
  const long long M = cmp ? b2r_compact_capacity(d->B, d->NP, d->NS)
                          : (long long)d->B * d->NP * d->NS;
  const long long per_scene = (long long)d->NP * d->NS;
  if (a.Cout_pad > 256 || (d->Cout % 8) != 0 || (d->mode == 1 && (d->Cin % 8) != 0)) {
    set_error("b2r_sa_layer_bwd: needs Cout %% 8 == 0, Cout <= 256, dense Cin %% 8 == 0 "
              "(Cin=%d Cout=%d)", d->Cin, d->Cout);
    return B2R_ERR_UNSUPPORTED;
  }
  const int NT = bwd_pick_nt(g, d->Cout, d->mode, a.top, a.do_dgrad, d->NS, M, per_scene, cmp);
  if (NT == 0) {
    set_error("b2r_sa_layer_bwd: layer Cin=%d Cout=%d M=%lld does not fit shared memory / TMEM",
              d->Cin, d->Cout, M);
    return B2R_ERR_UNSUPPORTED;
  }
  const BwdSmem L = bwd_smem_layout(a.Kp, a.KA, a.WA, a.Cout, a.Cout_pad, NT, a.top, cmp);
  a.num_tiles = (int)(M / NT);
  int sms = kNumSMs;
  if (d->sm_limit > 0 && d->sm_limit < kNumSMs) sms = d->sm_limit;
  const int grid = a.num_tiles < sms ? a.num_tiles : sms;
  cudaStream_t st = static_cast<cudaStream_t>(stream);
#define B2R_LAUNCH_BWD2(NTV, EWV, MV, TV, CV)                                                   \
  do {                                                                                          \
    B2R_CUDA(cudaFuncSetAttribute(sa_layer_bwd_kernel<NTV, EWV, MV, TV, CV>,                    \
                                  cudaFuncAttributeMaxDynamicSharedMemorySize, (int)L.total));  \
    sa_layer_bwd_kernel<NTV, EWV, MV, TV, CV><<<grid, kBwdThreads, L.total, st>>>(a);           \
  } while (0)
#define B2R_LAUNCH_BWD1(NTV, EWV, MV, TV)                                                       \
  do {                                                                                          \
    if (cmp) B2R_LAUNCH_BWD2(NTV, EWV, MV, TV, true); else B2R_LAUNCH_BWD2(NTV, EWV, MV, TV, false); \
  } while (0)
#define B2R_LAUNCH_BWD(NTV, EWTOP)                                                              \
  do {                                                                                          \
    if (a.top) {                                                                                \
      if (a.mode == 0) B2R_LAUNCH_BWD1(NTV, EWTOP, 0, 1); else B2R_LAUNCH_BWD1(NTV, EWTOP, 1, 1); \
    } else {                                                                                    \
      if (a.mode == 0) B2R_LAUNCH_BWD1(NTV, 4, 0, 0); else B2R_LAUNCH_BWD1(NTV, 4, 1, 0);       \
    }                                                                                           \
  } while (0)
  if (NT == 128) B2R_LAUNCH_BWD(128, 8);
  else if (NT == 64) B2R_LAUNCH_BWD(64, 8);
  else B2R_LAUNCH_BWD(32, 4);
#undef B2R_LAUNCH_BWD
#undef B2R_LAUNCH_BWD1
#undef B2R_LAUNCH_BWD2
  B2R_CHECK_LAUNCH();
  return B2R_OK;
}

extern "C" int b2r_pool_bwd_prep(const float *dout_cm, const float *dout_pm, const float *zmax,
                                 const float *zmin, const int *amax, const int *amin,
                                 const float *scale, const float *shift, int B, int NP, int C,
                                 float *dysel, int *asel, double *stats, void *stream) {
  B2R_REQUIRE((dout_cm || dout_pm) && zmax && zmin && amax && amin && scale && shift && dysel &&
                  asel && stats && B > 0 && NP > 0 && C > 0 && C <= 1024,
              "b2r_pool_bwd_prep: bad argument");
  B2R_REQUIRE(B <= 65535, "b2r_pool_bwd_prep: B=%d exceeds gridDim.z", B);
  dim3 grid(ceil_div(NP, 32), ceil_div(C, 32), B), block(32, 8);
  pool_bwd_prep_kernel<<<grid, block, 0, static_cast<cudaStream_t>(stream)>>>(
      dout_cm, dout_pm, zmax, zmin, amax, amin, scale, shift, NP, C, dysel, asel, stats);
  B2R_CHECK_LAUNCH();
  return B2R_OK;
}

extern "C" int b2r_bn_bwd_finalize_ex(const double *stats, int C, double count, const float *gamma,
                                      const float *mean, const float *invstd, int training,
                                      float *coef_a, float *coef_b, float *coef_c, float *k1,
                                      float *k2, float *gs, float *dgamma, float *dbeta,
                                      float *dbias_conv, void *stream) {
  B2R_REQUIRE(stats && mean && invstd && C > 0 && count > 0, "b2r_bn_bwd_finalize: bad argument");
  bn_bwd_finalize_kernel<<<ceil_div(C, 128), 128, 0, static_cast<cudaStream_t>(stream)>>>(
      stats, C, count, 1.0 / count, gamma, mean, invstd, training, coef_a, coef_b, coef_c, k1, k2, gs, dgamma,
      dbeta, dbias_conv);
  B2R_CHECK_LAUNCH();
  return B2R_OK;
}

extern "C" int b2r_bn_bwd_finalize(const double *stats, int C, double count, const float *gamma,
                                   const float *mean, const float *invstd, int training,
                                   float *coef_a, float *coef_b, float *coef_c, float *k1,
                                   float *k2, float *gs, float *dgamma, float *dbeta,
                                   void *stream) {
  return b2r_bn_bwd_finalize_ex(stats, C, count, gamma, mean, invstd, training, coef_a, coef_b,
                                coef_c, k1, k2, gs, dgamma, dbeta, nullptr, stream);
}
```

### backtoreality_b200/csrc/mlp_common.cuh

```cuda
#pragma once
#include <cuda/ptx>

#include "common.cuh"

namespace b2r {
namespace mlp {


__device__ __forceinline__ uint32_t to_tf32(float x) {
  uint32_t r;
  asm("cvt.rna.tf32.f32 %0, %1;" : "=r"(r) : "f"(x));
  return r;
}
__device__ __forceinline__ void mbar_init(uint32_t bar, uint32_t count) {
  asm volatile("mbarrier.init.shared::cta.b64 [%0], %1;" ::"r"(bar), "r"(count) : "memory");
}
__device__ __forceinline__ void mbar_expect_tx(uint32_t bar, uint32_t bytes) {
  asm volatile("mbarrier.arrive.expect_tx.shared::cta.b64 _, [%0], %1;" ::"r"(bar), "r"(bytes)
               : "memory");
}
__device__ __forceinline__ void mbar_wait(uint32_t bar, uint32_t parity) {
  asm volatile(
      "{\n\t"
      ".reg .pred p;\n\t"
      "MLP_WAIT_%=:\n\t"
      "mbarrier.try_wait.parity.shared::cta.b64 p, [%0], %1;\n\t"
      "@p bra MLP_DONE_%=;\n\t"
      "bra MLP_WAIT_%=;\n\t"
      "MLP_DONE_%=:\n\t"
      "}" ::"r"(bar),
      "r"(parity)
      : "memory");
}
__device__ __forceinline__ void bulk_g2s(uint32_t dst, const void *src, uint32_t bytes,
                                         uint32_t bar) {
  asm volatile(
      "cp.async.bulk.shared::cluster.global.mbarrier::complete_tx::bytes [%0], [%1], %2, [%3];" ::
          "r"(dst),
      "l"(src), "r"(bytes), "r"(bar)
      : "memory");
}
__device__ __forceinline__ void prefetch_l2(const void *p, uint32_t bytes) {
  asm volatile("cp.async.bulk.prefetch.L2.global [%0], %1;" ::"l"(p), "r"(bytes) : "memory");
}
__device__ __forceinline__ void fence_async_smem() {
  asm volatile("fence.proxy.async.shared::cta;" ::: "memory");
}
__device__ __forceinline__ void tc_fence_before() {
  asm volatile("tcgen05.fence::before_thread_sync;" ::: "memory");
}
__device__ __forceinline__ void tc_fence_after() {
  asm volatile("tcgen05.fence::after_thread_sync;" ::: "memory");
}
__device__ __forceinline__ void tmem_alloc(uint32_t smem_dst, uint32_t ncols) {
  asm volatile("tcgen05.alloc.cta_group::1.sync.aligned.shared::cta.b32 [%0], %1;" ::"r"(smem_dst),
               "r"(ncols)
               : "memory");
  asm volatile("tcgen05.relinquish_alloc_permit.cta_group::1.sync.aligned;" ::: "memory");
}
__device__ __forceinline__ void tmem_dealloc(uint32_t taddr, uint32_t ncols) {
  asm volatile("tcgen05.dealloc.cta_group::1.sync.aligned.b32 %0, %1;" ::"r"(taddr), "r"(ncols)
               : "memory");
}
__device__ __forceinline__ void umma_tf32(uint32_t d_tmem, uint64_t a_desc, uint64_t b_desc,
                                          uint32_t idesc, uint32_t accumulate) {
  asm volatile(
      "{\n\t"
      ".reg .pred p;\n\t"
      "setp.ne.b32 p, %4, 0;\n\t"
      "tcgen05.mma.cta_group::1.kind::tf32 [%0], %1, %2, %3, p;\n\t"
      "}" ::"r"(d_tmem),
      "l"(a_desc), "l"(b_desc), "r"(idesc), "r"(accumulate)
      : "memory");
}
__device__ __forceinline__ void umma_commit(uint32_t bar) {
  asm volatile("tcgen05.commit.cta_group::1.mbarrier::arrive::one.shared::cluster.b64 [%0];" ::"r"(
                   bar)
               : "memory");
}

__device__ __forceinline__ uint64_t smem_desc_sw128(uint32_t saddr) {
  uint64_t d = 0;
  d |= (uint64_t)((saddr >> 4) & 0x3fffu);
  d |= (uint64_t)1 << 16;
  d |= (uint64_t)(1024u >> 4) << 32;
  d |= (uint64_t)1 << 46;
  d |= (uint64_t)2 << 61;
  return d;
}
__host__ __device__ constexpr uint32_t idesc_tf32(int n) {
  return (1u << 4) | (2u << 7) | (2u << 10) | ((uint32_t)(n >> 3) << 17) | ((128u >> 4) << 24);
}

__device__ __forceinline__ uint64_t smem_desc_sw128_mn(uint32_t saddr, uint32_t lbo, uint32_t sbo) {
  uint64_t d = 0;
  d |= (uint64_t)((saddr >> 4) & 0x3fffu);
  d |= (uint64_t)((lbo >> 4) & 0x3fffu) << 16;
  d |= (uint64_t)((sbo >> 4) & 0x3fffu) << 32;
  d |= (uint64_t)1 << 46;
  d |= (uint64_t)2 << 61;
  return d;
}
__device__ __forceinline__ uint32_t sw128_off(int row, int chunk, int rows) {
  const int a = chunk >> 3, c = chunk & 7, g = row >> 3, r8 = row & 7;
  return (uint32_t)(((a * (rows >> 3) + g) << 10) + (r8 << 7) + ((c ^ r8) << 4));
}

__host__ __device__ inline int packed_k(int Cin, int gather) {
  if (!gather) return (Cin + 3) & ~3;
  const int C = Cin - 3;
  return ((C + 3) & ~3) + 4;
}

struct GatherSrc {
  const float *xyz, *new_xyz, *feat_t;
  int N, NP, NS, C, Cf4;
  int chf_shift;
  float radius;
  int normalize_xyz;
};

template <int NT, int NTHREADS, class OffFn>
__device__ __forceinline__ void build_x_gather(const GatherSrc &g, int b, int in_scene0,
                                               const int *s_idx, uint8_t *s_x, int tid,
                                               OffFn off, const int *s_cen = nullptr) {
  const int C = g.C, CHf = g.Cf4 >> 2;
  for (int row = tid; row < NT; row += NTHREADS) {
    const int p = s_idx[row];
    const int j = s_cen != nullptr ? max(s_cen[row], 0) : (in_scene0 + row) / g.NS;
    const float *pp = g.xyz + ((size_t)b * g.N + p) * 3;
    const float *qq = g.new_xyz + ((size_t)b * g.NP + j) * 3;
    const float px = __ldg(pp), py = __ldg(pp + 1), pz = __ldg(pp + 2);
    const float qx = __ldg(qq), qy = __ldg(qq + 1), qz = __ldg(qq + 2);
    float d0 = __fsub_rn(px, qx), d1 = __fsub_rn(py, qy), d2 = __fsub_rn(pz, qz);
    if (g.normalize_xyz) {
      d0 = __fdiv_rn(d0, g.radius);
      d1 = __fdiv_rn(d1, g.radius);
      d2 = __fdiv_rn(d2, g.radius);
    }
    *reinterpret_cast<uint4 *>(s_x + off(row, CHf)) =
        make_uint4(to_tf32(d0), to_tf32(d1), to_tf32(d2), 0u);
  }
  if (CHf == 0) return;
  const float *fb = g.feat_t + (size_t)b * g.N * C;
  const int total = NT * CHf;
  if ((C & 3) == 0) {
    for (int i0 = tid; i0 < total; i0 += NTHREADS * 8) {
      float4 t[8];
#pragma unroll
      for (int u = 0; u < 8; ++u) {
        const int i = i0 + u * NTHREADS;
        if (i < total) {
          const int row = g.chf_shift >= 0 ? (i >> g.chf_shift) : (i / CHf);
          const int ch = i - row * CHf;
          t[u] = __ldg(reinterpret_cast<const float4 *>(fb + (size_t)s_idx[row] * C) + ch);
        }
      }
#pragma unroll
      for (int u = 0; u < 8; ++u) {
        const int i = i0 + u * NTHREADS;
        if (i < total) {
          const int row = g.chf_shift >= 0 ? (i >> g.chf_shift) : (i / CHf);
          const int ch = i - row * CHf;
          *reinterpret_cast<uint4 *>(s_x + off(row, ch)) =
              make_uint4(to_tf32(t[u].x), to_tf32(t[u].y), to_tf32(t[u].z), to_tf32(t[u].w));
        }
      }
    }
  } else {
    for (int i = tid; i < total; i += NTHREADS) {
      const int row = g.chf_shift >= 0 ? (i >> g.chf_shift) : (i / CHf);
      const int ch = i - row * CHf;
      const float *src = fb + (size_t)s_idx[row] * C + ch * 4;
      float f[4] = {0.f, 0.f, 0.f, 0.f};
#pragma unroll
      for (int e = 0; e < 4; ++e)
        if (ch * 4 + e < C) f[e] = __ldg(src + e);
      *reinterpret_cast<uint4 *>(s_x + off(row, ch)) =
          make_uint4(to_tf32(f[0]), to_tf32(f[1]), to_tf32(f[2]), to_tf32(f[3]));
    }
  }
}

struct TileClass {
  int ns;
  int live;
  float wx;
};
__device__ __forceinline__ TileClass tile_class(const int *m, long long pos0, int NS) {
  const int p = (int)pos0;
  const int c = (p >= m[0]) + (p >= m[1]) + (p >= m[2]);
  TileClass t;
  t.ns = 8 << c;
  t.live = m[4 + c] - p;
  t.wx = (float)(NS - t.ns);
  return t;
}

inline int pow2_shift(int v) {
  if (v < 1 || (v & (v - 1))) return -1;
  int s = 0;
  while ((1 << s) < v) ++s;
  return s;
}

}

namespace thin {
bool fwd_applicable(const b2r_sa_layer *d);
int fwd_launch(const b2r_sa_layer *d, void *stream);
bool bwd_applicable(const b2r_sa_layer_bwd_desc *d);
int bwd_launch(const b2r_sa_layer_bwd_desc *d, void *stream);
}
}
```

### backtoreality_b200/csrc/mlp_thin.cu

```cuda
#include <stdlib.h>

#include "mlp_common.cuh"

namespace b2r {
namespace thin {
namespace {

using mlp::sw128_off;
using mlp::to_tf32;

constexpr int kThreads = 256, kWarps = kThreads / 32;
constexpr int kCtasPerSM = 2;
constexpr int kMaxK = 8;

struct ThinArgs {
  int N, NP, NS, C, K, Cout;
  long long M, per_scene;
  const float *xyz, *new_xyz, *feat_t;
  const int *idx;
  float radius;
  int normalize_xyz;
  const float *w_image;
  int Cout_pad, Cf4;
  float *z;
  double *stats;
  const float *gr, *zin, *coef_a, *coef_b, *coef_c;
  float *dW;
  const int *cidx, *ccen, *cmeta;
};

template <int KM, bool CMP>
__device__ __forceinline__ void gather_row(const ThinArgs &a, long long pos, float (&x)[KM]) {
  size_t prow;
  long long centre;
  if constexpr (CMP) {
    prow = (size_t)__ldg(a.cidx + pos);
    centre = max(__ldg(a.ccen + pos), 0);
  } else {
    const int b = (int)(pos / a.per_scene);
    centre = pos / a.NS;
    prow = (size_t)b * a.N + __ldg(a.idx + pos);
  }
  const float *pp = a.xyz + prow * 3;
  const float *qq = a.new_xyz + (size_t)centre * 3;
  float d0 = __fsub_rn(__ldg(pp), __ldg(qq));
  float d1 = __fsub_rn(__ldg(pp + 1), __ldg(qq + 1));
  float d2 = __fsub_rn(__ldg(pp + 2), __ldg(qq + 2));
  if (a.normalize_xyz) {
    d0 = __fdiv_rn(d0, a.radius);
    d1 = __fdiv_rn(d1, a.radius);
    d2 = __fdiv_rn(d2, a.radius);
  }
  x[0] = d0; x[1] = d1; x[2] = d2;
  const float *ff = a.feat_t + prow * a.C;
#pragma unroll
  for (int c = 0; c < KM - 3; ++c) x[3 + c] = c < a.C ? __ldg(ff + c) : 0.f;
}

template <int LP, int KM, bool CMP>
__global__ void __launch_bounds__(kThreads, kCtasPerSM) thin_fwd_kernel(const ThinArgs a) {
  constexpr int PPW = 32 / LP, ITERS = 32 / PPW;
  const int lane = threadIdx.x & 31, warp = threadIdx.x >> 5;
  const int sub = lane / LP, c4 = (lane % LP) * 4;
  __shared__ double s_red[kWarps][2][LP * 4];
  __shared__ int s_meta[8];
  long long M = a.M;
  if constexpr (CMP) {
    M = __ldg(a.cmeta + 8);
    if (threadIdx.x < 8) s_meta[threadIdx.x] = __ldg(a.cmeta + threadIdx.x);
    __syncthreads();
  }

  float w[4][KM];
#pragma unroll
  for (int e = 0; e < 4; ++e)
#pragma unroll
    for (int k = 0; k < KM; ++k) {
      float v = 0.f;
      if (k < a.K) {
        const int kp = k < 3 ? a.Cf4 + k : k - 3;
        v = a.w_image[(sw128_off(c4 + e, kp >> 2, a.Cout_pad) >> 2) + (kp & 3)];
      }
      w[e][k] = v;
    }

  double acc_s[4] = {0, 0, 0, 0}, acc_ss[4] = {0, 0, 0, 0};
  const long long nchunks = M >> 5, cstride = (long long)gridDim.x * kWarps;
  long long chunk = (long long)blockIdx.x * kWarps + warp;
  float xn[KM];
  if (chunk < nchunks) gather_row<KM, CMP>(a, (chunk << 5) + lane, xn);
  for (; chunk < nchunks; chunk += cstride) {
    const long long pos0 = chunk << 5;
    float x[KM];
#pragma unroll
    for (int k = 0; k < KM; ++k) x[k] = __uint_as_float(to_tf32(xn[k]));
    if (chunk + cstride < nchunks) gather_row<KM, CMP>(a, ((chunk + cstride) << 5) + lane, xn);
    mlp::TileClass tc{};
    int p64 = 0;
    if constexpr (CMP) {
      tc = mlp::tile_class(s_meta, pos0, a.NS);
      p64 = (int)(pos0 & 63);
    }
    float ts[4] = {0, 0, 0, 0}, tss[4] = {0, 0, 0, 0};
    float *zrow = a.z + (size_t)pos0 * a.Cout + c4;
#pragma unroll 4
    for (int it = 0; it < ITERS; ++it) {
      const int src = it * PPW + sub;
      float xr[KM];
#pragma unroll
      for (int k = 0; k < KM; ++k) xr[k] = __shfl_sync(0xffffffffu, x[k], src);
      float zz[4];
      float wgt = 1.f;
      if constexpr (CMP)
        wgt = src < tc.live ? ((((p64 + src) & (tc.ns - 1)) == 0) ? 1.f + tc.wx : 1.f) : 0.f;
#pragma unroll
      for (int e = 0; e < 4; ++e) {
        float s = 0.f;
#pragma unroll
        for (int k = 0; k < KM; ++k)
          if (k < a.K) s = fmaf(w[e][k], xr[k], s);
        zz[e] = s;
        if constexpr (CMP) {
          ts[e] = fmaf(wgt, s, ts[e]);
          tss[e] = fmaf(wgt * s, s, tss[e]);
        } else {
          ts[e] += s;
          tss[e] = fmaf(s, s, tss[e]);
        }
      }
      stg_stream_v4(reinterpret_cast<float4 *>(zrow + (size_t)src * a.Cout),
                    make_float4(zz[0], zz[1], zz[2], zz[3]));
    }
#pragma unroll
    for (int e = 0; e < 4; ++e) {
      acc_s[e] += (double)ts[e];
      acc_ss[e] += (double)tss[e];
    }
  }
  if (a.stats == nullptr) return;
#pragma unroll
  for (int e = 0; e < 4; ++e) {
#pragma unroll
    for (int o = LP; o < 32; o <<= 1) {
      acc_s[e] += __shfl_xor_sync(0xffffffffu, acc_s[e], o);
      acc_ss[e] += __shfl_xor_sync(0xffffffffu, acc_ss[e], o);
    }
    if (sub == 0) {
      s_red[warp][0][c4 + e] = acc_s[e];
      s_red[warp][1][c4 + e] = acc_ss[e];
    }
  }
  __syncthreads();
  for (int i = threadIdx.x; i < 2 * LP * 4; i += kThreads) {
    const int which = i / (LP * 4), c = i % (LP * 4);
    double t = 0.0;
#pragma unroll
    for (int wv = 0; wv < kWarps; ++wv) t += s_red[wv][which][c];
    atomicAdd(a.stats + (size_t)which * a.Cout + c, t);
  }
}

template <int LP, int KM, bool CMP>
__global__ void __launch_bounds__(kThreads, kCtasPerSM) thin_bwd_kernel(const ThinArgs a) {
  constexpr int PPW = 32 / LP, ITERS = 32 / PPW, UN = 4;
  const int lane = threadIdx.x & 31, warp = threadIdx.x >> 5;
  const int sub = lane / LP, c4 = (lane % LP) * 4;
  __shared__ float s_red[kWarps][LP * 4][KM];
  __shared__ int s_meta[8];
  long long M = a.M;
  if constexpr (CMP) {
    M = __ldg(a.cmeta + 8);
    if (threadIdx.x < 8) s_meta[threadIdx.x] = __ldg(a.cmeta + threadIdx.x);
    __syncthreads();
  }

  float ca[4], cb[4], cc[4];
#pragma unroll
  for (int e = 0; e < 4; ++e) {
    ca[e] = a.coef_a[c4 + e];
    cb[e] = a.coef_b[c4 + e];
    cc[e] = a.coef_c[c4 + e];
  }
  float acc[4][KM];
#pragma unroll
  for (int e = 0; e < 4; ++e)
#pragma unroll
    for (int k = 0; k < KM; ++k) acc[e][k] = 0.f;

  const long long nchunks = M >> 5, cstride = (long long)gridDim.x * kWarps;
  long long chunk = (long long)blockIdx.x * kWarps + warp;
  float xn[KM];
  if (chunk < nchunks) gather_row<KM, CMP>(a, (chunk << 5) + lane, xn);
  for (; chunk < nchunks; chunk += cstride) {
    const long long pos0 = chunk << 5;
    float x[KM];
#pragma unroll
    for (int k = 0; k < KM; ++k) x[k] = xn[k];
    if (chunk + cstride < nchunks) gather_row<KM, CMP>(a, ((chunk + cstride) << 5) + lane, xn);
    mlp::TileClass tc{};
    int p64 = 0;
    if constexpr (CMP) {
      tc = mlp::tile_class(s_meta, pos0, a.NS);
      p64 = (int)(pos0 & 63);
    }
    const int4 *grow = reinterpret_cast<const int4 *>(a.gr + (size_t)pos0 * a.Cout + c4);
    const int4 *zrow = reinterpret_cast<const int4 *>(a.zin + (size_t)pos0 * a.Cout + c4);
    const size_t rstride = (size_t)a.Cout >> 2;
#pragma unroll 1
    for (int it0 = 0; it0 < ITERS; it0 += UN) {
      int4 g[UN], zz[UN];
#pragma unroll
      for (int u = 0; u < UN; ++u) {
        const size_t r = (size_t)((it0 + u) * PPW + sub) * rstride;
        g[u] = ldg_stream_v4(grow + r);
        zz[u] = ldg_stream_v4(zrow + r);
      }
#pragma unroll
      for (int u = 0; u < UN; ++u) {
        const int src = (it0 + u) * PPW + sub;
        float xr[KM];
#pragma unroll
        for (int k = 0; k < KM; ++k) xr[k] = __shfl_sync(0xffffffffu, x[k], src);
        const float gv[4] = {__int_as_float(g[u].x), __int_as_float(g[u].y),
                             __int_as_float(g[u].z), __int_as_float(g[u].w)};
        const float zv[4] = {__int_as_float(zz[u].x), __int_as_float(zz[u].y),
                             __int_as_float(zz[u].z), __int_as_float(zz[u].w)};
        float wgt = 1.f;
        if constexpr (CMP)
          wgt = src < tc.live ? ((((p64 + src) & (tc.ns - 1)) == 0) ? 1.f + tc.wx : 1.f) : 0.f;
#pragma unroll
        for (int e = 0; e < 4; ++e) {
          const float dz = CMP ? fmaf(ca[e], gv[e], wgt * fmaf(cb[e], zv[e], cc[e]))
                               : fmaf(ca[e], gv[e], fmaf(cb[e], zv[e], cc[e]));
#pragma unroll
          for (int k = 0; k < KM; ++k)
            if (k < a.K) acc[e][k] = fmaf(dz, xr[k], acc[e][k]);
        }
      }
    }
  }
#pragma unroll
  for (int e = 0; e < 4; ++e)
#pragma unroll
    for (int k = 0; k < KM; ++k) {
#pragma unroll
      for (int o = LP; o < 32; o <<= 1) acc[e][k] += __shfl_xor_sync(0xffffffffu, acc[e][k], o);
      if (sub == 0) s_red[warp][c4 + e][k] = acc[e][k];
    }
  __syncthreads();
  for (int i = threadIdx.x; i < LP * 4 * a.K; i += kThreads) {
    const int c = i / a.K, k = i % a.K;
    float t = 0.f;
#pragma unroll
    for (int wv = 0; wv < kWarps; ++wv) t += s_red[wv][c][k];
    atomicAdd(a.dW + (size_t)c * a.K + k, t);
  }
}

bool disabled() {
  const char *v = getenv("B2R_NO_THIN");
  return v && *v && *v != '0';
}

bool shape_ok(int Cin, int Cout, long long M, long long per_scene) {
  if (disabled()) return false;
  if (Cin < 3 || Cin > kMaxK) return false;
  if (!(Cout == 32 || Cout == 64 || Cout == 128)) return false;
  return M > 0 && (per_scene % 32) == 0;
}

int grid_for(long long M, int sm_limit) {
  int sms = kNumSMs;
  if (sm_limit > 0 && sm_limit < kNumSMs) sms = sm_limit;
  const long long want = ((M >> 5) + kWarps - 1) / kWarps;
  const long long cap = (long long)sms * kCtasPerSM;
  return (int)(want < cap ? want : cap);
}

}

bool fwd_applicable(const b2r_sa_layer *d) {
  return d->mode == 0 && d->epilogue == 0 &&
         shape_ok(d->Cin, d->Cout, (long long)d->B * d->NP * d->NS, (long long)d->NP * d->NS);
}

int fwd_launch(const b2r_sa_layer *d, void *stream) {
  ThinArgs a = {};
  a.N = d->N; a.NP = d->NP; a.NS = d->NS; a.C = d->Cin - 3; a.K = d->Cin; a.Cout = d->Cout;
  a.per_scene = (long long)d->NP * d->NS;
  a.M = a.per_scene * d->B;
  a.xyz = d->xyz; a.new_xyz = d->new_xyz; a.feat_t = d->feat_t; a.idx = d->idx;
  a.radius = d->radius; a.normalize_xyz = d->normalize_xyz;
  a.w_image = d->w_image;
  a.Cout_pad = (d->Cout + 127) & ~127;
  a.Cf4 = (a.C + 3) & ~3;
  a.z = d->z; a.stats = d->stats;
  a.cidx = d->cidx; a.ccen = d->ccen; a.cmeta = d->cmeta;
  const bool cmp = d->cmeta != nullptr;
  const int grid = grid_for(cmp ? b2r_compact_capacity(d->B, d->NP, d->NS) : a.M, d->sm_limit);
  cudaStream_t st = static_cast<cudaStream_t>(stream);
#define B2R_THIN(LPV)                                                                  \
  do {                                                                               \
    if (cmp) {                                                                       \
      if (a.K <= 4) thin_fwd_kernel<LPV, 4, true><<<grid, kThreads, 0, st>>>(a);     \
      else thin_fwd_kernel<LPV, 8, true><<<grid, kThreads, 0, st>>>(a);              \
    } else {                                                                         \
      if (a.K <= 4) thin_fwd_kernel<LPV, 4, false><<<grid, kThreads, 0, st>>>(a);    \
      else thin_fwd_kernel<LPV, 8, false><<<grid, kThreads, 0, st>>>(a);             \
    }                                                                                \
  } while (0)
  switch (d->Cout) {
    case 32: B2R_THIN(8); break;
    case 64: B2R_THIN(16); break;
    default: B2R_THIN(32); break;
  }
#undef B2R_THIN
  B2R_CHECK_LAUNCH();
  return B2R_OK;
}

bool bwd_applicable(const b2r_sa_layer_bwd_desc *d) {
  const bool dgrad = (d->g_feat_t != nullptr && d->Cin > 3) || d->g_xyz != nullptr ||
                     d->g_new_xyz != nullptr;
  return d->mode == 0 && !dgrad && d->dz == nullptr && d->dysel == nullptr && d->gr && d->z &&
         d->coef_a && d->coef_b && d->coef_c &&
         shape_ok(d->Cin, d->Cout, (long long)d->B * d->NP * d->NS, (long long)d->NP * d->NS);
}

int bwd_launch(const b2r_sa_layer_bwd_desc *d, void *stream) {
  ThinArgs a = {};
  a.N = d->N; a.NP = d->NP; a.NS = d->NS; a.C = d->Cin - 3; a.K = d->Cin; a.Cout = d->Cout;
  a.per_scene = (long long)d->NP * d->NS;
  a.M = a.per_scene * d->B;
  a.xyz = d->xyz; a.new_xyz = d->new_xyz; a.feat_t = d->feat_t; a.idx = d->idx;
  a.radius = d->radius; a.normalize_xyz = d->normalize_xyz;
  a.gr = d->gr; a.zin = d->z;
  a.coef_a = d->coef_a; a.coef_b = d->coef_b; a.coef_c = d->coef_c;
  a.dW = d->dW;
  a.cidx = d->cidx; a.ccen = d->ccen; a.cmeta = d->cmeta;
  const bool cmp = d->cmeta != nullptr;
  const int grid = grid_for(cmp ? b2r_compact_capacity(d->B, d->NP, d->NS) : a.M, d->sm_limit);
  cudaStream_t st = static_cast<cudaStream_t>(stream);
#define B2R_THIN(LPV)                                                                  \
  do {                                                                               \
    if (cmp) {                                                                       \
      if (a.K <= 4) thin_bwd_kernel<LPV, 4, true><<<grid, kThreads, 0, st>>>(a);     \
      else thin_bwd_kernel<LPV, 8, true><<<grid, kThreads, 0, st>>>(a);              \
    } else {                                                                         \
      if (a.K <= 4) thin_bwd_kernel<LPV, 4, false><<<grid, kThreads, 0, st>>>(a);    \
      else thin_bwd_kernel<LPV, 8, false><<<grid, kThreads, 0, st>>>(a);             \
    }                                                                                \
  } while (0)
  switch (d->Cout) {
    case 32: B2R_THIN(8); break;
    case 64: B2R_THIN(16); break;
    default: B2R_THIN(32); break;
  }
#undef B2R_THIN
  B2R_CHECK_LAUNCH();
  return B2R_OK;
}

}
}
```

### backtoreality_b200/fused_sa.py

```python
import ctypes
import os

import torch

from . import _ext, _lib, step_arena

_vp = ctypes.c_void_p


def _ptr(t):
    return _vp(t.data_ptr()) if t is not None else None


def to_point_major(features):
    B, C, N = features.shape
    out = torch.empty((B, N, C), dtype=torch.float32, device=features.device)
    _lib.check(_lib.lib().b2r_to_point_major(_ptr(features), B, C, N, _ptr(out), _ext._stream()),
               "to_point_major")
    _ext.LAUNCHES += 1
    return out


def pack_weight(weight, gather):
    Cout, Cin = weight.shape[0], weight.shape[1]
    w = weight.detach().reshape(Cout, Cin).contiguous()
    nbytes = _lib.lib().b2r_mlp_weight_image_bytes(Cout, Cin, 1 if gather else 0)
    image = torch.empty(nbytes // 4, dtype=torch.float32, device=weight.device)
    _lib.check(_lib.lib().b2r_mlp_pack_weight(_ptr(w), Cout, Cin, 1 if gather else 0, _ptr(image),
                                              _ext._stream()), "mlp_pack_weight")
    _ext.LAUNCHES += 1
    return image


_PREPACKED = {}
_PACK_STREAMS = {}
_PACK_EVENTS = {}


def prepack(mlp_modules, backward=None):
    mlp_modules = [m for m in mlp_modules if m is not None and len(m) > 0]
    if not mlp_modules or not mlp_modules[0][0].conv.weight.is_cuda:
        if not torch.cuda.is_available():
            return
        dev = torch.device("cuda", torch.cuda.current_device())
    else:
        dev = mlp_modules[0][0].conv.weight.device
    for key in [k for k, ent in list(_PREPACKED.items()) if ent[3].device == dev]:
        _PREPACKED.pop(key, None)
    _PACK_EVENTS[dev] = []
    if not mlp_modules or not mlp_modules[0][0].conv.weight.is_cuda:
        return
    if backward is None:
        backward = torch.is_grad_enabled()
    main = torch.cuda.current_stream(dev)
    side = _PACK_STREAMS.get(dev)
    if side is None:
        side = _PACK_STREAMS[dev] = torch.cuda.Stream(device=dev)
    side.wait_stream(main)
    with torch.cuda.stream(side), torch.no_grad():
        for kind in (("tf32", "bf16") if backward else ("tf32",)):
            for mlp in mlp_modules:
                entries = []
                for i, blk in enumerate(mlp):
                    w = blk.conv.weight
                    if kind == "bf16" and not w.requires_grad:
                        continue
                    image = (pack_weight if kind == "tf32" else pack_weight_bf16)(w, gather=(i == 0))
                    entries.append(((id(w), kind), image, w._version, w))
                ev = torch.cuda.Event()
                ev.record(side)
                _PACK_EVENTS[dev].append(ev)
                for key, image, version, w in entries:
                    _PREPACKED[key] = (image, ev, version, w)


def prepack_join():
    if not torch.cuda.is_available():
        return
    dev = torch.device("cuda", torch.cuda.current_device())
    for ev in _PACK_EVENTS.pop(dev, []):
        torch.cuda.current_stream().wait_event(ev)


def _take(weight, kind):
    ent = _PREPACKED.pop((id(weight), kind), None)
    if ent is None or ent[3] is not weight or ent[2] != weight._version:
        return None
    image, ev = ent[0], ent[1]
    main = torch.cuda.current_stream(weight.device)
    main.wait_event(ev)
    image.record_stream(main)
    return image


COMPACT = os.environ.get("B2R_COMPACT", "1") not in ("0", "")
COMPACT_MIN_NS = 32
PLAN_KEYS = ("cidx", "ccen", "cmeta")


def compact_wanted(nsample):
    return COMPACT and nsample in (32, 64) and nsample >= COMPACT_MIN_NS


def compact_plan(idx, N):
    B, NP, NS = idx.shape
    lib = _lib.lib()
    cap = int(lib.b2r_compact_capacity(B, NP, NS))
    dev = idx.device
    cidx = torch.empty(cap, dtype=torch.int32, device=dev)
    ccen = torch.empty(cap, dtype=torch.int32, device=dev)
    cmeta = torch.empty(16, dtype=torch.int32, device=dev)
    ws = torch.empty(int(lib.b2r_compact_workspace_bytes(B, NP)), dtype=torch.uint8, device=dev)
    _lib.check(lib.b2r_compact_plan(_ptr(idx), B, int(N), NP, NS, _ptr(cidx), _ptr(ccen),
                                    _ptr(cmeta), _ptr(ws), _ext._stream()), "compact_plan")
    _ext.LAUNCHES += 3
    return {"cidx": cidx, "ccen": ccen, "cmeta": cmeta}


def supported(mlp_module, xyz, features, idx, pooling="max"):
    if pooling != "max" or not xyz.is_cuda:
        return False
    B, NP, NS = idx.shape
    blocks = list(mlp_module)
    if len(blocks) == 0:
        return False
    lib = _lib.lib()
    for i, blk in enumerate(blocks):
        if not hasattr(blk, "bn") or blk.conv.bias is not None:
            return False
        bn = blk.bn.bn
        if bn.momentum is None or not bn.track_running_stats or not bn.affine:
            return False
        cout, cin = blk.conv.out_channels, blk.conv.in_channels
        gather, top = (1 if i == 0 else 0), (1 if i == len(blocks) - 1 else 0)
        if not lib.b2r_sa_layer_fwd_supported(B, NP, NS, cin, cout, gather, top):
            return False
        if not lib.b2r_sa_layer_bwd_supported(B, NP, NS, cin, cout, gather, top):
            return False
    return True


def _layer_work(B, N, NP, NS, Cin, Cout, gather, pooled, backward):
    M = B * NP * NS
    flops = 2.0 * M * Cin * Cout
    byts = 4.0 * Cin * Cout
    if gather:
        byts += B * (4.0 * (Cin - 3) * N + 12.0 * N + 4.0 * NP * NS)
    if pooled:
        byts += 4.0 * Cout * B * NP
    if backward:
        flops, byts = 2 * flops, 2 * byts
    return (byts, flops)


def sa_mlp_forward(xyz, new_xyz, feat_t, idx, radius, normalize_xyz, mlp_module, training,
                   want_point_major=True, save=None, sm_limit=0, plan=None):
    lib = _lib.lib()
    st = _ext._stream()
    dev = xyz.device
    B, N = xyz.shape[0], xyz.shape[1]
    NP, NS = idx.shape[1], idx.shape[2]
    M = B * NP * NS
    rows = M if plan is None else int(plan["cidx"].shape[0])
    blocks = list(mlp_module)
    L = len(blocks)
    z_prev = scale = shift = None
    zs, bn_saved, images = [], [], []
    stats_all = None
    if training:
        stats_all = step_arena.zeros(sum(2 * b.conv.out_channels for b in blocks), dtype=torch.float64,
                                device=dev)
    stats_off = 0
    zmax = zmin = amax = amin = None
    for i, blk in enumerate(blocks):
        conv, bn = blk.conv, blk.bn.bn
        Cin, Cout = conv.in_channels, conv.out_channels
        last = i == L - 1
        image = _take(conv.weight, "tf32")
        if image is None:
            image = pack_weight(conv.weight, gather=(i == 0))
        images.append(image)
        stats = None
        if training:
            stats = stats_all[stats_off:stats_off + 2 * Cout]
            stats_off += 2 * Cout
        d = _lib.SaLayer()
        d.B, d.N, d.NP, d.NS, d.Cin, d.Cout = B, N, NP, NS, Cin, Cout
        d.mode = 0 if i == 0 else 1
        d.epilogue = 1 if last else 0
        if i == 0:
            d.xyz, d.new_xyz, d.feat_t, d.idx = _ptr(xyz), _ptr(new_xyz), _ptr(feat_t), _ptr(idx)
            d.radius, d.normalize_xyz = float(radius), 1 if normalize_xyz else 0
        else:
            d.z_prev, d.scale_prev, d.shift_prev = _ptr(z_prev), _ptr(scale), _ptr(shift)
        d.w_image = _ptr(image)
        d.sm_limit = int(sm_limit)
        if plan is not None:
            d.cidx, d.ccen, d.cmeta = _ptr(plan["cidx"]), _ptr(plan["ccen"]), _ptr(plan["cmeta"])
        z = None
        if last:
            zmax = torch.empty((B * NP, Cout), dtype=torch.float32, device=dev)
            zmin = torch.empty_like(zmax)
            amax = torch.empty((B * NP, Cout), dtype=torch.int32, device=dev)
            amin = torch.empty_like(amax)
            d.zmax, d.zmin, d.amax, d.amin = _ptr(zmax), _ptr(zmin), _ptr(amax), _ptr(amin)
        else:
            z = torch.empty((rows, Cout), dtype=torch.float32, device=dev)
            d.z = _ptr(z)
        d.stats = _ptr(stats)
        with _ext._timed("sa_layer_fwd", _layer_work(B, N, NP, NS, Cin, Cout, i == 0, last, False)):
            _lib.check(lib.b2r_sa_layer_fwd(ctypes.byref(d), st), "sa_layer_fwd")
        if training:
            scale = torch.empty(Cout, dtype=torch.float32, device=dev)
            shift = torch.empty_like(scale)
            mean = torch.empty_like(scale)
            invstd = torch.empty_like(scale)
            _lib.check(lib.b2r_bn_finalize(_ptr(stats), Cout, float(M), _ptr(bn.weight),
                                           _ptr(bn.bias), float(bn.eps), float(bn.momentum),
                                           _ptr(bn.running_mean), _ptr(bn.running_var),
                                           _ptr(scale), _ptr(shift), _ptr(mean), _ptr(invstd),
                                           _ptr(bn.num_batches_tracked), st),
                       "bn_finalize")
            _ext.LAUNCHES += 1
        else:
            invstd = torch.rsqrt(bn.running_var + bn.eps)
            mean = bn.running_mean
            scale = (bn.weight * invstd).contiguous()
            shift = (bn.bias - bn.running_mean * scale).contiguous()
        zs.append(z)
        bn_saved.append((mean, invstd, scale, shift))
        z_prev = z
    Cl = blocks[-1].conv.out_channels
    out_cm = torch.empty((B, Cl, NP), dtype=torch.float32, device=dev)
    out_pm = torch.empty((B, NP, Cl), dtype=torch.float32, device=dev) if want_point_major else None
    _lib.check(lib.b2r_pool_finalize(_ptr(zmax), _ptr(zmin), _ptr(scale), _ptr(shift), B, NP, Cl,
                                     _ptr(out_cm), _ptr(out_pm), st), "pool_finalize")
    _ext.LAUNCHES += 1
    if save is not None:
        save.update(zs=zs, bn=bn_saved, zmax=zmax, zmin=zmin, amax=amax, amin=amin, images=images,
                    plan=plan)
    return out_cm, out_pm


def pack_weight_bf16(weight, gather):
    Cout, Cin = weight.shape[0], weight.shape[1]
    w = weight.detach().reshape(Cout, Cin).contiguous()
    nbytes = _lib.lib().b2r_mlp_weight_bf16_image_bytes(Cout, Cin, 1 if gather else 0)
    image = torch.empty(nbytes // 2, dtype=torch.bfloat16, device=weight.device)
    _lib.check(_lib.lib().b2r_mlp_pack_weight_bf16(_ptr(w), Cout, Cin, 1 if gather else 0,
                                                   _ptr(image), _ext._stream()),
               "mlp_pack_weight_bf16")
    _ext.LAUNCHES += 1
    return image


def sa_mlp_backward(g_out_cm, xyz, new_xyz, feat_t, idx, radius, normalize_xyz, weights, gammas,
                    training, saved, need_feat, need_xyz, need_new_xyz, sm_limit=0, versioned=None,
                    g_out_pm=None):
    lib = _lib.lib()
    st = _ext._stream()
    dev = xyz.device
    assert g_out_cm is not None or g_out_pm is not None
    B, N = xyz.shape[0], xyz.shape[1]
    NP, NS = idx.shape[1], idx.shape[2]
    M = B * NP * NS
    plan = saved.get("plan")
    rows = M if plan is None else int(plan["cidx"].shape[0])
    L = len(weights)
    zs, bn, images = saved["zs"], saved["bn"], saved["images"]
    f32 = dict(dtype=torch.float32, device=dev)
    dWs, dgammas, dbetas = [None] * L, [None] * L, [None] * L
    tr = 1 if training else 0

    top = L - 1
    Ct = weights[top].shape[0]
    mean, invstd, scale, shift = bn[top]
    stats_all = step_arena.zeros(sum(2 * w.shape[0] for w in weights), dtype=torch.float64, device=dev)
    dW_all = step_arena.zeros(sum(w.numel() for w in weights), **f32)
    s_off, w_off = [0], [0]
    for w in weights:
        s_off.append(s_off[-1] + 2 * w.shape[0])
        w_off.append(w_off[-1] + w.numel())
    stats = stats_all[s_off[top]:s_off[top + 1]]
    dysel = torch.empty((B * NP, Ct), **f32)
    asel = torch.empty((B * NP, Ct), dtype=torch.int32, device=dev)
    _lib.check(lib.b2r_pool_bwd_prep(_ptr(g_out_cm), _ptr(g_out_pm), _ptr(saved["zmax"]), _ptr(saved["zmin"]),
                                     _ptr(saved["amax"]), _ptr(saved["amin"]), _ptr(scale),
                                     _ptr(shift), B, NP, Ct, _ptr(dysel), _ptr(asel), _ptr(stats),
                                     st), "pool_bwd_prep")
    coef = [torch.empty(Ct, **f32) for _ in range(3)]
    dgammas[top], dbetas[top] = torch.empty(Ct, **f32), torch.empty(Ct, **f32)
    _lib.check(lib.b2r_bn_bwd_finalize(_ptr(stats), Ct, float(M), _ptr(gammas[top]), _ptr(mean),
                                       _ptr(invstd), tr, _ptr(coef[0]), _ptr(coef[1]),
                                       _ptr(coef[2]), None, None, None, _ptr(dgammas[top]),
                                       _ptr(dbetas[top]), st), "bn_bwd_finalize")
    _ext.LAUNCHES += 2

    g_feat_t = g_xyz = g_new_xyz = None
    gr = None
    for l in range(L - 1, -1, -1):
        Cout, Cin = weights[l].shape[0], weights[l].shape[1]
        b = _lib.SaLayerBwd()
        b.B, b.N, b.NP, b.NS, b.Cin, b.Cout = B, N, NP, NS, Cin, Cout
        b.mode = 0 if l == 0 else 1
        b.sm_limit = int(sm_limit)
        if plan is not None:
            b.cidx, b.ccen, b.cmeta = _ptr(plan["cidx"]), _ptr(plan["ccen"]), _ptr(plan["cmeta"])
        if l == top:
            b.dysel, b.asel = _ptr(dysel), _ptr(asel)
        else:
            b.gr, b.z = _ptr(gr), _ptr(zs[l])
        b.coef_a, b.coef_b, b.coef_c = _ptr(coef[0]), _ptr(coef[1]), _ptr(coef[2])
        dWs[l] = dW_all[w_off[l]:w_off[l + 1]].view(Cout, Cin)
        b.dW = _ptr(dWs[l])
        need_dgrad = True
        gr_prev = stats_prev = None
        if l == 0:
            b.xyz, b.new_xyz, b.feat_t, b.idx = _ptr(xyz), _ptr(new_xyz), _ptr(feat_t), _ptr(idx)
            b.radius, b.normalize_xyz = float(radius), 1 if normalize_xyz else 0
            if need_feat and feat_t is not None:
                g_feat_t = step_arena.zeros_like(feat_t)
                b.g_feat_t = _ptr(g_feat_t)
            if need_xyz:
                g_xyz = step_arena.zeros_like(xyz)
                b.g_xyz = _ptr(g_xyz)
            if need_new_xyz:
                g_new_xyz = step_arena.zeros_like(new_xyz)
                b.g_new_xyz = _ptr(g_new_xyz)
            need_dgrad = g_feat_t is not None or need_xyz or need_new_xyz
        else:
            b.z_prev, b.scale_prev, b.shift_prev = _ptr(zs[l - 1]), _ptr(bn[l - 1][2]), _ptr(bn[l - 1][3])
            gr_prev = torch.empty((rows, Cin), **f32)
            stats_prev = stats_all[s_off[l - 1]:s_off[l]]
            b.gr_prev, b.stats_prev = _ptr(gr_prev), _ptr(stats_prev)
        image = None
        if need_dgrad or l == top:
            image = _take(versioned[l], "bf16") if versioned is not None else None
            if image is None:
                image = pack_weight_bf16(weights[l], gather=(l == 0))
        b.w_image_bf16 = _ptr(image)
        with _ext._timed("sa_layer_bwd", _layer_work(B, N, NP, NS, Cin, Cout, l == 0, l == top, True)):
            _lib.check(lib.b2r_sa_layer_bwd(ctypes.byref(b), st), "sa_layer_bwd")
        if l > 0:
            mean, invstd, _, _ = bn[l - 1]
            coef = [torch.empty(Cin, **f32) for _ in range(3)]
            dgammas[l - 1], dbetas[l - 1] = torch.empty(Cin, **f32), torch.empty(Cin, **f32)
            _lib.check(lib.b2r_bn_bwd_finalize(_ptr(stats_prev), Cin, float(M), _ptr(gammas[l - 1]),
                                               _ptr(mean), _ptr(invstd), tr, _ptr(coef[0]),
                                               _ptr(coef[1]), _ptr(coef[2]), None, None, None,
                                               _ptr(dgammas[l - 1]), _ptr(dbetas[l - 1]), st),
                       "bn_bwd_finalize")
            _ext.LAUNCHES += 1
            gr = gr_prev
    return g_feat_t, g_xyz, g_new_xyz, dWs, dgammas, dbetas


class _FusedSABlock(torch.autograd.Function):

    @staticmethod
    def forward(ctx, xyz, new_xyz, features, features_pm, idx, radius, normalize_xyz, mlp_module,
                training, sm_limit, want_pm, plan, *params):
        if features_pm is not None:
            feat_t = features_pm
        elif features is None:
            feat_t = None
        elif features.shape[1] == 1:
            feat_t = features.contiguous().reshape(features.shape[0], features.shape[2], 1)
        else:
            feat_t = to_point_major(features.contiguous())
        need = any(ctx.needs_input_grad)
        save = {} if need else None
        fwd_limit, bwd_limit = sm_limit if isinstance(sm_limit, tuple) else (sm_limit, 0)
        out_cm, out_pm = sa_mlp_forward(xyz, new_xyz, feat_t, idx, radius, normalize_xyz,
                                        mlp_module, training, want_point_major=bool(want_pm),
                                        save=save, sm_limit=fwd_limit, plan=plan)
        ctx.set_materialize_grads(False)
        if need:
            ctx.saved = (xyz, new_xyz, feat_t, idx, float(radius), bool(normalize_xyz),
                         bool(training), save, params)
            ctx.bwd_sm_limit = int(bwd_limit)
            ctx.from_pm = features_pm is not None
        if want_pm:
            return out_cm, out_pm
        return out_cm, None

    @staticmethod
    def backward(ctx, g_cm, g_pm):
        xyz, new_xyz, feat_t, idx, radius, normalize_xyz, training, save, params = ctx.saved
        L = len(params) // 3
        n_in = 12
        if g_cm is None and g_pm is None:
            return (None,) * (n_in + 3 * L)
        weights = [params[3 * i].detach().reshape(params[3 * i].shape[0], -1) for i in range(L)]
        gammas = [params[3 * i + 1].detach() for i in range(L)]
        nig = ctx.needs_input_grad
        g_feat_t, g_xyz, g_new_xyz, dWs, dgs, dbs = sa_mlp_backward(
            g_cm.contiguous() if g_cm is not None else None, xyz, new_xyz, feat_t, idx, radius,
            normalize_xyz, weights, gammas, training, save, need_feat=nig[2] or nig[3],
            need_xyz=nig[0], need_new_xyz=nig[1], sm_limit=ctx.bwd_sm_limit,
            versioned=[params[3 * i] for i in range(L)],
            g_out_pm=g_pm.contiguous() if g_pm is not None else None)
        g_features = g_features_pm = None
        if g_feat_t is not None:
            if ctx.from_pm:
                g_features_pm = g_feat_t
            elif g_feat_t.shape[2] == 1:
                g_features = g_feat_t.reshape(g_feat_t.shape[0], 1, g_feat_t.shape[1])
            else:
                g_features = g_feat_t.transpose(1, 2).contiguous()
        out = [g_xyz, g_new_xyz, g_features, g_features_pm] + [None] * (n_in - 4)
        for i in range(L):
            out += [dWs[i].view_as(params[3 * i]), dgs[i], dbs[i]]
        return tuple(out)


def sa_block(xyz, new_xyz, features, idx, radius, normalize_xyz, mlp_module, training,
             sm_limit=0, features_pm=None, want_pm=False, plan=None):
    if plan is None and compact_wanted(idx.shape[2]):
        plan = compact_plan(idx, xyz.shape[1])
    params = []
    for blk in mlp_module:
        params += [blk.conv.weight, blk.bn.bn.weight, blk.bn.bn.bias]
    return _FusedSABlock.apply(xyz, new_xyz, features, features_pm, idx, radius, normalize_xyz,
                               mlp_module, training, sm_limit, bool(want_pm), plan, *params)


NUM_SMS = 148

ENABLED = os.environ.get("B2R_FUSED", "1") not in ("0", "")
```

### include/b2r.h

```cpp
#ifndef B2R_H_
#define B2R_H_

#if defined(__GNUC__)
#define B2R_API __attribute__((visibility("default")))
#else
#define B2R_API
#endif

#ifdef __cplusplus
extern "C" {
#endif

typedef enum b2r_status {
  B2R_OK = 0,
  B2R_ERR_INVALID_ARG = -1,
  B2R_ERR_CUDA = -2,
  B2R_ERR_UNSUPPORTED = -3
} b2r_status;

B2R_API int b2r_version(void);
B2R_API const char *b2r_status_string(int status);
B2R_API const char *b2r_last_error(void);
B2R_API int b2r_struct_bytes(int which);

B2R_API int b2r_ref_block_threads(int work_size);

B2R_API int b2r_fps(const float *xyz, int B, int N, int npoint, int *idx, void *stream);

B2R_API int b2r_fps_ex(const float *xyz, int B, int N, int npoint, int *idx, int cluster_hint,
                       void *stream);

B2R_API long long b2r_fps_workspace_bytes(int B, int N);
B2R_API int b2r_fps_ws(const float *xyz, int B, int N, int npoint, int *idx, int cluster_hint,
                       void *workspace, long long workspace_bytes, void *stream);
B2R_API int b2r_fps_sort(const float *xyz, int B, int N, void *workspace, long long workspace_bytes,
                         void *stream);
B2R_API int b2r_fps_ws_presorted(const float *xyz, int B, int N, int npoint, int *idx, int cluster_hint,
                                 void *workspace, long long workspace_bytes, void *stream);

B2R_API int b2r_fps_plan(int B, int N, int *cluster_size, int *threads, int *points_per_thread,
                 int *smem_bytes);

B2R_API int b2r_gather_fwd(const float *features, const int *idx, int B, int C, int N, int M, float *out,
                   void *stream);

B2R_API int b2r_gather_bwd(const float *grad_out, const int *idx, int B, int C, int N, int M,
                   float *grad_features, void *stream);

B2R_API int b2r_ball_query(const float *new_xyz, const float *xyz, int B, int N, int M, float radius,
                   int nsample, int *idx, void *stream);

B2R_API long long b2r_ball_query_workspace_bytes(int B, int N);
B2R_API int b2r_ball_query_grid(const float *new_xyz, const float *xyz, int B, int N, int M,
                                float radius, int nsample, int *idx, void *workspace,
                                long long workspace_bytes, void *stream);

B2R_API int b2r_group_fwd(const float *features, const int *idx, int B, int C, int N, int NP, int NS,
                  float *out, void *stream);

B2R_API int b2r_group_bwd(const float *grad_out, const int *idx, int B, int C, int N, int NP, int NS,
                  float *grad_features, void *stream);

B2R_API int b2r_three_nn(const float *unknown, const float *known, int B, int n, int m, float *dist2,
                 int *idx, void *stream);

B2R_API int b2r_three_interp_fwd(const float *features, const int *idx, const float *weight, int B, int C,
                         int m, int n, float *out, void *stream);

B2R_API int b2r_three_interp_bwd(const float *grad_out, const int *idx, const float *weight, int B, int C,
                         int n, int m, float *grad_features, void *stream);

B2R_API long long b2r_scatter_plan_bytes(int B, long long entries, int N, int entries_per_source,
                                         int weighted);
B2R_API int b2r_scatter_plan(const int *idx, const float *weight, int B, long long entries, int N,
                             int entries_per_source, void *plan, long long plan_bytes, void *stream);
B2R_API int b2r_group_bwd_plan(const float *grad_out, const void *plan, int B, int C, int N, int NP,
                               int NS, float *grad_features, void *stream);
B2R_API int b2r_three_interp_bwd_plan(const float *grad_out, const void *plan, int B, int C, int n,
                                      int m, float *grad_features, void *stream);

B2R_API int b2r_query_group_fwd(const float *xyz, const float *new_xyz, const float *features,
                        const int *idx, int B, int C, int N, int NP, int NS, float radius,
                        int normalize_xyz, float *out, void *stream);

B2R_API int b2r_query_group_bwd(const float *grad_out, const int *idx, int B, int C, int N, int NP, int NS,
                        float radius, int normalize_xyz, float *grad_xyz, float *grad_new_xyz,
                        float *grad_features, void *stream);


typedef struct b2r_sa_layer {
  int B, N, NP, NS;
  int Cin, Cout;
  int mode, epilogue;
  const float *xyz;
  const float *new_xyz;
  const float *feat_t;
  const int *idx;
  float radius;
  int normalize_xyz;
  const float *z_prev;
  const float *scale_prev;
  const float *shift_prev;
  const float *w_image;
  float *z;
  double *stats;
  float *zmax, *zmin;
  int *amax, *amin;
  int sm_limit;
  const int *cidx, *ccen, *cmeta;
} b2r_sa_layer;

B2R_API long long b2r_mlp_weight_image_bytes(int Cout, int Cin, int gather);
B2R_API int b2r_mlp_pack_weight(const float *w, int Cout, int Cin, int gather, float *image,
                                void *stream);
B2R_API int b2r_sa_layer_fwd(const b2r_sa_layer *desc, void *stream);
B2R_API int b2r_sa_layer_fwd_supported(int B, int NP, int NS, int Cin, int Cout, int gather,
                                       int pooled);

B2R_API int b2r_sa_layer_fwd_tile(int B, int NP, int NS, int Cin, int Cout, int gather, int pooled,
                                  int compact);

B2R_API int b2r_bn_finalize(const double *stats, int C, double count, const float *gamma,
                            const float *beta, float eps, float momentum, float *running_mean,
                            float *running_var, float *scale, float *shift, float *mean_out,
                            float *invstd_out, long long *num_batches_tracked, void *stream);

B2R_API int b2r_pool_finalize(const float *zmax, const float *zmin, const float *scale,
                              const float *shift, int B, int NP, int C, float *out_cm,
                              float *out_pm, void *stream);

B2R_API int b2r_to_point_major(const float *in, int B, int C, int N, float *out, void *stream);

typedef struct b2r_sa_layer_bwd_desc {
  int B, N, NP, NS;
  int Cin, Cout;
  int mode;
  const float *xyz, *new_xyz, *feat_t;
  const int *idx;
  float radius;
  int normalize_xyz;
  const float *z_prev, *scale_prev, *shift_prev;
  const void *w_image_bf16;
  const float *dz;
  const float *gr, *z;
  const float *dysel;
  const int *asel;
  const float *coef_a, *coef_b, *coef_c;
  float *dW;
  float *gr_prev;
  double *stats_prev;
  float *g_feat_t;
  float *g_xyz;
  float *g_new_xyz;
  int sm_limit;
  const int *cidx, *ccen, *cmeta;
} b2r_sa_layer_bwd_desc;

B2R_API long long b2r_mlp_weight_bf16_image_bytes(int Cout, int Cin, int gather);
B2R_API int b2r_mlp_pack_weight_bf16(const float *w, int Cout, int Cin, int gather, void *image,
                                     void *stream);
B2R_API int b2r_sa_layer_bwd(const b2r_sa_layer_bwd_desc *desc, void *stream);
B2R_API int b2r_sa_layer_bwd_supported(int B, int NP, int NS, int Cin, int Cout, int gather,
                                       int top);

B2R_API int b2r_sa_layer_bwd_tile(int B, int NP, int NS, int Cin, int Cout, int gather, int top,
                                  int dgrad, int compact);

B2R_API int b2r_pool_bwd_prep(const float *dout_cm, const float *dout_pm, const float *zmax,
                              const float *zmin, const int *amax, const int *amin,
                              const float *scale, const float *shift, int B, int NP, int C,
                              float *dysel, int *asel, double *stats, void *stream);

B2R_API int b2r_bn_bwd_finalize(const double *stats, int C, double count, const float *gamma,
                                const float *mean, const float *invstd, int training,
                                float *coef_a, float *coef_b, float *coef_c, float *k1, float *k2,
                                float *gs, float *dgamma, float *dbeta, void *stream);
B2R_API int b2r_bn_bwd_finalize_ex(const double *stats, int C, double count, const float *gamma,
                                   const float *mean, const float *invstd, int training,
                                   float *coef_a, float *coef_b, float *coef_c, float *k1,
                                   float *k2, float *gs, float *dgamma, float *dbeta,
                                   float *dbias_conv, void *stream);

B2R_API long long b2r_compact_capacity(int B, int NP, int NS);
B2R_API long long b2r_compact_workspace_bytes(int B, int NP);
B2R_API int b2r_compact_plan(const int *idx, int B, int N, int NP, int NS, int *cidx, int *ccen,
                             int *meta, void *workspace, void *stream);

typedef struct b2r_dense_layer {
  int M, Cin, Cout;
  const float *in;
  int ld_in;
  const float *sc_in, *sh_in;
  const float *w_img;
  const float *bias;
  float *z;
  int ld_z;
  double *stats;
} b2r_dense_layer;

typedef struct b2r_dense_layer_bwd {
  int M, Cin, Cout;
  const float *in;
  int ld_in;
  const float *sc_in, *sh_in;
  const float *g, *zz;
  int ld_g;
  const float *ca, *cb, *cc;
  const float *wt_img;
  float *gin;
  int ld_gin;
  double *stats_in;
  float *dW;
} b2r_dense_layer_bwd;

B2R_API long long b2r_dense_image_bytes(int rows, int k);
B2R_API int b2r_dense_pack(const float *w, int Cout, int Cin, float *w_img, float *wt_img,
                           void *stream);
B2R_API int b2r_dense_fwd(const b2r_dense_layer *desc, void *stream);
B2R_API int b2r_dense_bwd(const b2r_dense_layer_bwd *desc, void *stream);

B2R_API int b2r_interp_cat_fwd(const float *known, const float *skip, const int *idx,
                               const float *weight, int B, int n, int m, int C2, int C1,
                               float *out, void *stream);
B2R_API int b2r_interp_cat_bwd(const float *g, int ld_g, const int *idx, const float *weight, int B,
                               int n, int m, int C2, int C1, float *g_known, float *g_skip,
                               void *stream);
B2R_API int b2r_vote_tail_fwd(const float *net, int ld_net, const float *seed_xyz,
                              const float *seed_feat, long long M, int C, float *vote_xyz,
                              float *out, float *norm, void *stream);
B2R_API int b2r_vote_tail_bwd(const float *g_out, const float *g_vote_xyz, const float *out,
                              const float *norm, long long M, int C, int ld_net, float *g_net,
                              float *g_seed_feat, void *stream);

B2R_API int b2r_nn_argmin(const float *pc1, const float *pc2, int B, int N, int M, int C, int mode,
                          float delta, long long *idx1, long long *idx2, void *stream);

B2R_API int b2r_adam_state_bytes(void);
B2R_API int b2r_adam_flat_step(float *params, const float *grads, float *exp_avg, float *exp_avg_sq,
                               long long n, void *state, float lr, float beta1, float beta2, float eps,
                               float weight_decay, float grad_scale, void *stream);

#ifdef __cplusplus
}
#endif
#endif
```

Measured before the change: 2452.

## Recompute thin first SA layer inside second layer instead of materializing z

When the first SA MLP layer has at most 4 input channels and no input gradients are needed, its output z is no longer written. The second layer's forward and backward kernels instead re-gather the raw xyz/feature row and recompute the thin layer plus BN/ReLU in the producer warps. The first layer's weight gradient is folded from accumulated double-precision sums by a new small kernel, and the separate layer-0 backward pass is dropped. This removes a large activation write and read at the widest layer, at the cost of extra per-tile gather and recompute work, more shared memory, and new template variants.

```diff
diff --git a/backtoreality_b200/_lib.py b/backtoreality_b200/_lib.py
--- a/backtoreality_b200/_lib.py
+++ b/backtoreality_b200/_lib.py
@@ -60,10 +60,12 @@
         ("zmax", _vp), ("zmin", _vp), ("amax", _vp), ("amin", _vp),
         ("sm_limit", _i),
         ("cidx", _vp), ("ccen", _vp), ("cmeta", _vp),
+        ("w_image_prev", _vp), ("Cin_prev", _i),
     ]
 
 
 SIGNATURES.update({
+    "b2r_sa_thin_recompute": [_i, _i, _i, _i, _i],
     "b2r_mlp_weight_image_bytes": [_i, _i, _i],
     "b2r_mlp_pack_weight": [_vp, _i, _i, _i, _vp, _vp],
     "b2r_sa_layer_fwd": [ctypes.POINTER(SaLayer), _vp],
@@ -89,10 +91,12 @@
         ("g_feat_t", _vp), ("g_xyz", _vp), ("g_new_xyz", _vp),
         ("sm_limit", _i),
         ("cidx", _vp), ("ccen", _vp), ("cmeta", _vp),
+        ("w_image_prev", _vp), ("Cin_prev", _i), ("thin_sums", _vp),
     ]
 
 
 SIGNATURES.update({
+    "b2r_thin_fold_dw": [_vp, _vp, _vp, _vp, _i, _i, _vp, _vp],
     "b2r_mlp_weight_bf16_image_bytes": [_i, _i, _i],
     "b2r_mlp_pack_weight_bf16": [_vp, _i, _i, _i, _vp, _vp],
     "b2r_sa_layer_bwd": [ctypes.POINTER(SaLayerBwd), _vp],
diff --git a/backtoreality_b200/csrc/mlp.cu b/backtoreality_b200/csrc/mlp.cu
--- a/backtoreality_b200/csrc/mlp.cu
+++ b/backtoreality_b200/csrc/mlp.cu
@@ -35,6 +35,8 @@
   float radius;
   int normalize_xyz;
   const float *z_prev, *scale_prev, *shift_prev;
+  const float *w_prev;
+  int Cin_prev;
   const float *w_image;
   float *z;
   double *stats;
@@ -49,10 +51,10 @@
 
 struct FwdSmem {
   uint32_t w_off, w_bytes, x_off[2], x_bytes, raw_off[2], raw_bytes, scale_off, idx_off, cen_off,
-      bar_off, total;
+      thin_off, bar_off, total;
 };
 __host__ __device__ inline FwdSmem fwd_smem_layout(int Kp, int Cout_pad, int NT, int raw_cin,
-                                                   int cmp = 0) {
+                                                   int cmp = 0, int thin = 0) {
   FwdSmem s;
   const uint32_t KA = (uint32_t)(Kp + 31) >> 5;
   s.w_off = 0;
@@ -66,7 +68,8 @@
   s.scale_off = s.raw_off[1] + s.raw_bytes;
   s.idx_off = s.scale_off + 2u * Kp * 4u;
   s.cen_off = s.idx_off + (uint32_t)NT * 4u;
-  s.bar_off = (s.cen_off + (cmp ? 3u * (uint32_t)NT * 4u + 32u : 0u) + 15u) & ~15u;
+  s.thin_off = (s.cen_off + (cmp ? 3u * (uint32_t)NT * 4u + 32u : 0u) + 15u) & ~15u;
+  s.bar_off = s.thin_off + (thin ? ((uint32_t)Kp + (uint32_t)NT) * 32u : 0u);
   s.total = s.bar_off + 11 * 8 + 16 + 1024;
   return s;
 }
@@ -80,12 +83,13 @@
   asm volatile("mbarrier.arrive.shared::cta.b64 _, [%0];" ::"r"(bar) : "memory");
 }
 
-template <int NT, bool CMP>
+template <int NT, bool CMP, int XK>
 __global__ void __launch_bounds__(kFwdThreads, 1) sa_layer_fwd_kernel(const LayerArgs a) {
   extern __shared__ __align__(1024) uint8_t smem_raw[];
   uint8_t *base = reinterpret_cast<uint8_t *>((reinterpret_cast<uintptr_t>(smem_raw) + 1023) &
                                               ~(uintptr_t)1023);
-  const FwdSmem L = fwd_smem_layout(a.Kp, a.Cout_pad, NT, a.raw_stage ? a.Cin : 0, CMP ? 1 : 0);
+  const FwdSmem L =
+      fwd_smem_layout(a.Kp, a.Cout_pad, NT, a.raw_stage ? a.Cin : 0, CMP ? 1 : 0, XK > 0 ? 1 : 0);
   uint8_t *s_w = base + L.w_off;
   float *s_scale = reinterpret_cast<float *>(base + L.scale_off);
   float *s_shift = s_scale + a.Kp;
@@ -93,6 +97,8 @@
   int *s_cenp = reinterpret_cast<int *>(base + L.cen_off);
   int *s_cene = s_cenp + NT;
   int *s_meta = s_cene + 2 * NT;
+  float *s_w0 = reinterpret_cast<float *>(base + L.thin_off);
+  float *s_xr = s_w0 + a.Kp * 8;
   uint64_t *s_bar = reinterpret_cast<uint64_t *>(base + L.bar_off);
   uint32_t *s_tmem = reinterpret_cast<uint32_t *>(s_bar + 11);
   auto bar = [&](int i) { return smem_u32(&s_bar[i]); };
@@ -120,6 +126,7 @@
       s_scale[i] = a.scale_prev[i];
       s_shift[i] = a.shift_prev[i];
     }
+  if constexpr (XK > 0) load_thin_weights(a.w_prev, a.Cin, a.Cin_prev, s_w0, tid, kFwdThreads);
   fence_async_smem();
   tc_fence_before();
   __syncthreads();
@@ -149,12 +156,59 @@
       }
     }
     int nidx = 0, ncen = 0;
+    constexpr int XKA = XK > 0 ? XK : 4;
+    ThinRowRaw<XKA> raw{};
+    ThinRowSrc src{};
+    if constexpr (XK > 0)
+      if (ptid < NT) {
+        if ((int)blockIdx.x < num_tiles)
+          raw = thin_row_fetch<XKA>(a, a.Cin_prev - 3,
+                                    thin_row_src<CMP>(a, per_scene, (long long)blockIdx.x * NT + ptid));
+        if ((int)blockIdx.x + grid < num_tiles)
+          src = thin_row_src<CMP>(a, per_scene, (long long)(blockIdx.x + grid) * NT + ptid);
+      }
     for (int k = 0, tile = blockIdx.x; tile < num_tiles; tile += grid, ++k) {
       const int s = k & 1, n = k >> 1;
       mbar_wait(bar(2 + s), (uint32_t)((n & 1) ^ 1));
       const long long pos0 = (long long)tile * NT;
       uint8_t *sx = base + L.x_off[s];
-      if (CMP && a.mode == 0) {
+      if constexpr (XK > 0) {
+        static_assert(kFwdProdThreads >= NT, "one producer thread per row");
+        if (ptid < NT) {
+          float xr[XK];
+          thin_row_finish<XK>(a, raw, xr);
+          round_tf32(xr);
+#pragma unroll
+          for (int kk = 0; kk < XK; ++kk) s_xr[ptid * 8 + kk] = xr[kk];
+          if (tile + grid < num_tiles) raw = thin_row_fetch<XK>(a, a.Cin_prev - 3, src);
+          if (tile + 2 * grid < num_tiles)
+            src = thin_row_src<CMP>(a, per_scene, pos0 + 2ll * grid * NT + ptid);
+        }
+        fwd_bar_prod();
+        const int CH = a.Cin >> 2;
+        const int total = NT * CH;
+        const int chs = (CH & (CH - 1)) == 0 ? 31 - __clz(CH) : -1;
+        for (int i = ptid; i < total; i += kFwdProdThreads) {
+          const int row = chs >= 0 ? (i >> chs) : (i / CH), ch = i - row * CH;
+          float x[XK];
+#pragma unroll
+          for (int kk = 0; kk < XK; ++kk) x[kk] = s_xr[row * 8 + kk];
+          float w[4][XK];
+#pragma unroll
+          for (int kk = 0; kk < XK; ++kk) {
+            const float4 t = *reinterpret_cast<const float4 *>(s_w0 + kk * a.Cin + ch * 4);
+            w[0][kk] = t.x; w[1][kk] = t.y; w[2][kk] = t.z; w[3][kk] = t.w;
+          }
+          uint32_t o[4];
+#pragma unroll
+          for (int e = 0; e < 4; ++e) {
+            const int c = ch * 4 + e;
+            const float z = thin_z<XK>(w[e], x, a.Cin_prev);
+            o[e] = to_tf32(fmaxf(fmaf(z, s_scale[c], s_shift[c]), 0.f));
+          }
+          *reinterpret_cast<uint4 *>(sx + sw128_off(row, ch, NT)) = make_uint4(o[0], o[1], o[2], o[3]);
+        }
+      } else if (CMP && a.mode == 0) {
         if (ptid < NT) {
           s_idx[ptid] = (k == 0) ? a.cidx[pos0 + ptid] : nidx;
           s_cenp[ptid] = (k == 0) ? a.ccen[pos0 + ptid] : ncen;
@@ -496,15 +550,15 @@
 
 namespace {
 int fwd_pick_nt(int Kp, int Cout_pad, int Cin, int mode, int epilogue, int NS, long long M,
-                long long per_scene, int *raw_stage, int cmp = 0) {
+                long long per_scene, int *raw_stage, int cmp = 0, int thin = 0) {
   const int MT = Cout_pad >> 7;
-  for (int raw = (mode == 1 ? 1 : 0); raw >= 0; --raw)
+  for (int raw = (mode == 1 && !thin ? 1 : 0); raw >= 0; --raw)
     for (int nt : {128, 64, 32}) {
       if (M % nt) continue;
       if (!cmp && mode == 0 && per_scene % nt) continue;
       if (epilogue == 1 && (nt % NS) != 0) continue;
       if (raw && nt < 64) continue;
-      const FwdSmem L = fwd_smem_layout(Kp, Cout_pad, nt, raw ? Cin : 0, cmp);
+      const FwdSmem L = fwd_smem_layout(Kp, Cout_pad, nt, raw ? Cin : 0, cmp, thin);
       if (L.total <= 227u * 1024u && 2 * MT * nt <= 512) {
         *raw_stage = raw;
         return nt;
@@ -524,6 +578,10 @@
   int raw = 0;
   return fwd_pick_nt(packed_k(Cin, gather), (Cout + 127) & ~127, Cin, gather ? 0 : 1,
                      pooled ? 1 : 0, NS, M, per_scene, &raw) > 0 ? 1 : 0;
+}
+
+extern "C" int b2r_sa_thin_recompute(int B, int NP, int NS, int Cin, int Cout) {
+  return thin::recompute_ok(B, NP, NS, Cin, Cout) ? 1 : 0;
 }
 
 extern "C" int b2r_sa_layer_fwd_tile(int B, int NP, int NS, int Cin, int Cout, int gather,
@@ -549,6 +607,7 @@
   a.xyz = d->xyz; a.new_xyz = d->new_xyz; a.feat_t = d->feat_t; a.idx = d->idx;
   a.radius = d->radius; a.normalize_xyz = d->normalize_xyz;
   a.z_prev = d->z_prev; a.scale_prev = d->scale_prev; a.shift_prev = d->shift_prev;
+  a.w_prev = d->w_image_prev; a.Cin_prev = d->Cin_prev;
   a.w_image = d->w_image; a.z = d->z; a.stats = d->stats;
   a.zmax = d->zmax; a.zmin = d->zmin; a.amax = d->amax; a.amin = d->amin;
   a.Kp = packed_k(d->Cin, d->mode == 0);
@@ -570,12 +629,19 @@
                 "b2r_sa_layer_fwd: gather mode needs xyz, new_xyz, idx (and feat_t when Cin > 3)");
     B2R_REQUIRE(d->Cin == 3 || ((reinterpret_cast<uintptr_t>(d->feat_t) & 15u) == 0),
                 "b2r_sa_layer_fwd: feat_t must be 16-byte aligned");
+  } else if (d->w_image_prev != nullptr) {
+    B2R_REQUIRE(d->scale_prev && d->shift_prev && (d->Cin % 4) == 0 && d->Cin <= 128 &&
+                    d->Cin_prev >= 3 && d->Cin_prev <= 4 && d->xyz && d->new_xyz &&
+                    (d->idx || cmp) && (d->feat_t || d->Cin_prev == 3),
+                "b2r_sa_layer_fwd: a layer above a thin first layer needs scale/shift, Cin %% 4 "
+                "== 0, Cin <= 128, 3 <= Cin_prev <= 4 and that layer's gather inputs");
   } else {
     B2R_REQUIRE(d->z_prev && d->scale_prev && d->shift_prev && (d->Cin % 4) == 0,
                 "b2r_sa_layer_fwd: dense mode needs z_prev/scale/shift and Cin %% 4 == 0");
   }
   if (d->epilogue == 0) {
-    B2R_REQUIRE(d->z != nullptr, "b2r_sa_layer_fwd: epilogue 0 needs z");
+    B2R_REQUIRE(d->z != nullptr || (d->stats != nullptr && thin::fwd_applicable(d)),
+                "b2r_sa_layer_fwd: epilogue 0 needs z (a thin first layer: z or stats)");
   } else {
     B2R_REQUIRE(d->zmax && d->zmin && d->amax && d->amin,
                 "b2r_sa_layer_fwd: epilogue 1 needs pool outputs");
@@ -589,25 +655,37 @@
     return B2R_ERR_UNSUPPORTED;
   }
   if (thin::fwd_applicable(d)) return thin::fwd_launch(d, stream);
-  const int NT = fwd_pick_nt(a.Kp, a.Cout_pad, d->Cin, d->mode, d->epilogue, d->NS, M, per_scene,
-                             &a.raw_stage, cmp);
+  const int xk = d->mode == 1 && d->w_image_prev != nullptr ? 4 : 0;
+  int NT = fwd_pick_nt(a.Kp, a.Cout_pad, d->Cin, d->mode, d->epilogue, d->NS, M, per_scene,
+                       &a.raw_stage, cmp);
+  if (xk > 0) {
+    a.raw_stage = 0;
+    if (NT > 0 && fwd_smem_layout(a.Kp, a.Cout_pad, NT, 0, cmp, 1).total > 227u * 1024u)
+      NT = fwd_pick_nt(a.Kp, a.Cout_pad, d->Cin, d->mode, d->epilogue, d->NS, M, per_scene,
+                       &a.raw_stage, cmp, 1);
+  }
   if (NT == 0) {
     set_error("b2r_sa_layer_fwd: layer Cin=%d Cout=%d M=%lld NP*NS=%lld does not fit (needs "
               "B*NP*NS %% 32 == 0, gather layers NP*NS %% 32 == 0, operands within 227 KB)",
               d->Cin, d->Cout, M, per_scene);
     return B2R_ERR_UNSUPPORTED;
   }
-  const FwdSmem L = fwd_smem_layout(a.Kp, a.Cout_pad, NT, a.raw_stage ? d->Cin : 0, cmp);
+  const FwdSmem L = fwd_smem_layout(a.Kp, a.Cout_pad, NT, a.raw_stage ? d->Cin : 0, cmp, xk > 0);
   a.num_tiles = (int)(M / NT);
   int sms = kNumSMs;
   if (d->sm_limit > 0 && d->sm_limit < kNumSMs) sms = d->sm_limit;
   const int grid = a.num_tiles < sms ? a.num_tiles : sms;
   cudaStream_t st = static_cast<cudaStream_t>(stream);
+#define B2R_LAUNCH_FWD2(NTV, CMPV, XKV)                                                         \
+  do {                                                                                          \
+    B2R_CUDA(cudaFuncSetAttribute(sa_layer_fwd_kernel<NTV, CMPV, XKV>,                          \
+                                  cudaFuncAttributeMaxDynamicSharedMemorySize, (int)L.total));  \
+    sa_layer_fwd_kernel<NTV, CMPV, XKV><<<grid, kFwdThreads, L.total, st>>>(a);                 \
+  } while (0)
 #define B2R_LAUNCH_FWD(NTV, CMPV)                                                               \
   do {                                                                                          \
-    B2R_CUDA(cudaFuncSetAttribute(sa_layer_fwd_kernel<NTV, CMPV>,                               \
-                                  cudaFuncAttributeMaxDynamicSharedMemorySize, (int)L.total));  \
-    sa_layer_fwd_kernel<NTV, CMPV><<<grid, kFwdThreads, L.total, st>>>(a);                      \
+    if (xk == 4) B2R_LAUNCH_FWD2(NTV, CMPV, 4);                                                 \
+    else B2R_LAUNCH_FWD2(NTV, CMPV, 0);                                                         \
   } while (0)
   if (cmp) {
     if (NT == 128) B2R_LAUNCH_FWD(128, true);
@@ -619,6 +697,7 @@
     else B2R_LAUNCH_FWD(32, false);
   }
 #undef B2R_LAUNCH_FWD
+#undef B2R_LAUNCH_FWD2
   B2R_CHECK_LAUNCH();
   return B2R_OK;
 }
diff --git a/backtoreality_b200/csrc/mlp_bwd.cu b/backtoreality_b200/csrc/mlp_bwd.cu
--- a/backtoreality_b200/csrc/mlp_bwd.cu
+++ b/backtoreality_b200/csrc/mlp_bwd.cu
@@ -16,6 +16,9 @@
   float radius;
   int normalize_xyz;
   const float *z_prev, *scale_prev, *shift_prev;
+  const float *w_prev;
+  int Cin_prev;
+  double *thin_sums;
   const void *w_image;
   const float *dz;
   const float *gr, *z;
@@ -40,10 +43,10 @@
 
 struct BwdSmem {
   uint32_t w_off, w_bytes, x_off[2], dz_off[2], x_bytes, dz_bytes, coef_off, scale_off, idx_off,
-      cen_off, meta_off, route_off, flush_off, bar_off, total;
+      cen_off, meta_off, thin_off, route_off, flush_off, bar_off, total;
 };
 __host__ __device__ inline BwdSmem bwd_smem_layout(int Kp, int KA, int WA, int Cout, int Cout_pad,
-                                                   int NT, int top, int cmp = 0) {
+                                                   int NT, int top, int cmp = 0, int thin = 0) {
   BwdSmem s;
   s.w_off = 0;
   s.w_bytes = (uint32_t)Cout_pad * WA * 128u;
@@ -61,7 +64,8 @@
   s.idx_off = s.scale_off + 2u * Kp * 4u;
   s.cen_off = s.idx_off + 4u * (uint32_t)NT * 4u;
   s.meta_off = s.cen_off + (cmp ? 4u * (uint32_t)NT * 4u : 0u);
-  s.route_off = (s.meta_off + (cmp ? 32u : 0u) + 15u) & ~15u;
+  s.thin_off = (s.meta_off + (cmp ? 32u : 0u) + 15u) & ~15u;
+  s.route_off = s.thin_off + (thin ? ((uint32_t)Kp + 4u * (uint32_t)NT) * 32u : 0u);
   s.flush_off = s.route_off +
                 (top ? 4u * (uint32_t)(NT / (cmp ? 8 : 16)) * Cout_pad * 4u : 0u);
   const uint32_t flush_bytes = 8u * 32u * 33u * 4u;
@@ -129,7 +133,7 @@
   }
 }
 
-template <int NT, int EW, int MODE, int TOP, bool CMP>
+template <int NT, int EW, int MODE, int TOP, bool CMP, int XK>
 __global__ void __launch_bounds__(kBwdThreads, 1) sa_layer_bwd_kernel(const BwdArgs a) {
   constexpr int kMode = MODE;
   constexpr bool kTop = TOP != 0;
@@ -140,7 +144,9 @@
   extern __shared__ __align__(1024) uint8_t smem_raw[];
   uint8_t *base = reinterpret_cast<uint8_t *>((reinterpret_cast<uintptr_t>(smem_raw) + 1023) &
                                               ~(uintptr_t)1023);
-  const BwdSmem L = bwd_smem_layout(a.Kp, a.KA, a.WA, a.Cout, a.Cout_pad, NT, kTop, CMP ? 1 : 0);
+  static_assert(XK == 0 || (MODE == 1 && TOP == 0), "thin recompute: dense non-top layers only");
+  const BwdSmem L =
+      bwd_smem_layout(a.Kp, a.KA, a.WA, a.Cout, a.Cout_pad, NT, kTop, CMP ? 1 : 0, XK > 0 ? 1 : 0);
   uint8_t *s_w = base + L.w_off;
   float *s_ca = reinterpret_cast<float *>(base + L.coef_off);
   float *s_cb = s_ca + a.Cout;
@@ -150,6 +156,8 @@
   int *s_idx4 = reinterpret_cast<int *>(base + L.idx_off);
   int *s_cen4 = reinterpret_cast<int *>(base + L.cen_off);
   int *s_meta = reinterpret_cast<int *>(base + L.meta_off);
+  float *s_w0 = reinterpret_cast<float *>(base + L.thin_off);
+  float *s_xr4 = s_w0 + a.Kp * 8;
   float *s_dy = reinterpret_cast<float *>(base + L.route_off);
   int *s_as = reinterpret_cast<int *>(s_dy + 2 * kRC * a.Cout_pad);
   uint64_t *s_bar = reinterpret_cast<uint64_t *>(base + L.bar_off);
@@ -190,6 +198,7 @@
       s_scale[i] = a.scale_prev[i];
       s_shift[i] = a.shift_prev[i];
     }
+  if constexpr (XK > 0) load_thin_weights(a.w_prev, a.Cin, a.Cin_prev, s_w0, tid, kBwdThreads);
   if (has_coef)
     for (int i = tid; i < a.Cout; i += kBwdThreads) {
       s_ca[i] = a.coef_a[i];
@@ -215,6 +224,20 @@
     const int CHx = a.Cin >> 3;
     const int chxs = (CHx > 0 && (CHx & (CHx - 1)) == 0) ? 31 - __clz(CHx) : -1;
     int nidx = 0, ncen = 0;
+    constexpr int XKA = XK > 0 ? XK : 4;
+    ThinRowRaw<XKA> raw{};
+    double sxa[XKA];
+#pragma unroll
+    for (int kk = 0; kk < XKA; ++kk) sxa[kk] = 0.0;
+    ThinRowSrc src{};
+    if constexpr (XK > 0)
+      if (ptid < NT) {
+        if ((int)blockIdx.x < num_tiles)
+          raw = thin_row_fetch<XKA>(a, a.Cin_prev - 3,
+                                    thin_row_src<CMP>(a, per_scene, (long long)blockIdx.x * NT + ptid));
+        if ((int)blockIdx.x + grid < num_tiles)
+          src = thin_row_src<CMP>(a, per_scene, (long long)(blockIdx.x + grid) * NT + ptid);
+      }
     for (int k = 0, tile = blockIdx.x; tile < num_tiles; tile += grid, ++k) {
       const int s = k & 1, n = k >> 1;
       mbar_wait(bar(2 + s), (uint32_t)((n & 1) ^ 1));
@@ -237,7 +260,7 @@
             prefetch_l2(a.z + pn * a.Cout, (uint32_t)NT * a.Cout * 4u);
           }
         }
-        if (kMode == 1) prefetch_l2(a.z_prev + pn * a.Cin, (uint32_t)NT * a.Cin * 4u);
+        if (kMode == 1 && XK == 0) prefetch_l2(a.z_prev + pn * a.Cin, (uint32_t)NT * a.Cin * 4u);
       }
       if (!kTop) {
         const int total = NT * CH8;
@@ -380,6 +403,55 @@
             }
           }
         }
+      } else if constexpr (XK > 0) {
+        static_assert(kProdThreads >= NT, "one producer thread per row");
+        float *s_xr = s_xr4 + (k & 3) * NT * 8;
+        if (ptid < NT) {
+          float xn[XK];
+          thin_row_finish<XK>(a, raw, xn);
+          float wgt = 1.f;
+          if constexpr (CMP)
+            wgt = ptid < tc.live ? ((((p64 + ptid) & (tc.ns - 1)) == 0) ? 1.f + tc.wx : 1.f) : 0.f;
+#pragma unroll
+          for (int kk = 0; kk < XK; ++kk) {
+            s_xr[ptid * 8 + kk] = xn[kk];
+            sxa[kk] += (double)(wgt * xn[kk]);
+          }
+          round_tf32(xn);
+#pragma unroll
+          for (int kk = 0; kk < XK; ++kk) s_xr[ptid * 8 + 4 + kk] = xn[kk];
+          if (tile + grid < num_tiles) raw = thin_row_fetch<XK>(a, a.Cin_prev - 3, src);
+          if (tile + 2 * grid < num_tiles)
+            src = thin_row_src<CMP>(a, per_scene, pos0 + 2ll * grid * NT + ptid);
+        }
+        bar_prod();
+        const int CH = a.Cin >> 3;
+        const int total = NT * CH;
+        for (int i = ptid; i < total; i += kProdThreads) {
+          const int row = chxs >= 0 ? (i >> chxs) : (i / CH), ch = i - row * CH;
+          float x[XK];
+#pragma unroll
+          for (int kk = 0; kk < XK; ++kk) x[kk] = s_xr[row * 8 + 4 + kk];
+          float v[8];
+#pragma unroll
+          for (int h4 = 0; h4 < 8; h4 += 4) {
+            float w[4][XK];
+#pragma unroll
+            for (int kk = 0; kk < XK; ++kk) {
+              const float4 t = *reinterpret_cast<const float4 *>(s_w0 + kk * a.Cin + ch * 8 + h4);
+              w[0][kk] = t.x; w[1][kk] = t.y; w[2][kk] = t.z; w[3][kk] = t.w;
+            }
+#pragma unroll
+            for (int e = 0; e < 4; ++e) {
+              const int c = ch * 8 + h4 + e;
+              v[h4 + e] =
+                  fmaxf(fmaf(thin_z<XK>(w[e], x, a.Cin_prev), s_scale[c], s_shift[c]), 0.f);
+            }
+          }
+          *reinterpret_cast<uint4 *>(sx + bf_off(row, ch, NT)) =
+              make_uint4(pack_bf16(v[0], v[1]), pack_bf16(v[2], v[3]), pack_bf16(v[4], v[5]),
+                         pack_bf16(v[6], v[7]));
+        }
       } else {
         const int CH = a.Cin >> 3;
         const int total = NT * CH;
@@ -415,6 +487,15 @@
       fence_async_smem();
       __syncwarp();
       if (lane == 0) mbar_arrive(bar(0 + s));
+    }
+    if constexpr (XK > 0) {
+#pragma unroll
+      for (int kk = 0; kk < XK; ++kk) {
+#pragma unroll
+        for (int o = 16; o > 0; o >>= 1) sxa[kk] += __shfl_xor_sync(0xffffffffu, sxa[kk], o);
+        if (lane == 0 && kk < a.Cin_prev)
+          atomicAdd(a.thin_sums + 2 * (size_t)a.Cin * a.Cin_prev + kk, sxa[kk]);
+      }
     }
   } else if (warp == EW) {
     if (lane == 0) {
@@ -476,6 +557,22 @@
     const uint32_t lane_addr = (uint32_t)(q * 32) << 16;
     float s1[3] = {0.f, 0.f, 0.f}, s2[3] = {0.f, 0.f, 0.f};
     double d1[3] = {0.0, 0.0, 0.0}, d2[3] = {0.0, 0.0, 0.0};
+    constexpr int XKA = XK > 0 ? XK : 1;
+    float tg[XKA], tz[XKA];
+    double dg[XKA], dzs[XKA];
+    float w0[XKA];
+#pragma unroll
+    for (int kk = 0; kk < XKA; ++kk) {
+      tg[kk] = tz[kk] = 0.f;
+      dg[kk] = dzs[kk] = 0.0;
+      w0[kk] = 0.f;
+    }
+    if constexpr (XK > 0) {
+      const int kp = q * 32 + lane;
+      if (kp < a.Cin)
+#pragma unroll
+        for (int kk = 0; kk < XK; ++kk) w0[kk] = s_w0[kk * a.Cin + kp];
+    }
     int ntiles = 0;
     auto fetch_route = [&](int k, int tile) {
       if (tile < num_tiles) {
@@ -638,7 +735,43 @@
             asm volatile("tcgen05.wait::ld.sync.aligned;" ::: "memory");
             const int kp = m * 128 + q * 32 + lane;
             const long long p0 = pos0 + cc * 32;
-            if (kMode == 1) {
+            if constexpr (XK > 0) {
+              if (kp < a.Cin) {
+                const float sc = s_scale[kp], sh = s_shift[kp];
+                const float *xr = s_xr4 + (k & 3) * NT * 8 + cc * 32 * 8;
+                TileClass tc{};
+                if constexpr (CMP) tc = tile_class(s_meta, pos0, a.NS);
+                const int p64 = (int)(pos0 & 63);
+                float t1 = 0.f, t2 = 0.f;
+#pragma unroll 4
+                for (int i = 0; i < 32; ++i) {
+                  float x[XK], xt[XK];
+#pragma unroll
+                  for (int kk = 0; kk < XK; ++kk) {
+                    x[kk] = xr[i * 8 + kk];
+                    xt[kk] = xr[i * 8 + 4 + kk];
+                  }
+                  const float z = thin_z<XK>(w0, xt, a.Cin_prev);
+                  const float g = fmaf(z, sc, sh) > 0.f ? __uint_as_float(r[i]) : 0.f;
+                  t1 += g;
+                  t2 = fmaf(g, z, t2);
+                  float wgt = 1.f;
+                  if constexpr (CMP) {
+                    const int row = cc * 32 + i;
+                    wgt = row < tc.live ? ((((p64 + row) & (tc.ns - 1)) == 0) ? 1.f + tc.wx : 1.f)
+                                        : 0.f;
+                  }
+                  const float wz = wgt * z;
+#pragma unroll
+                  for (int kk = 0; kk < XK; ++kk) {
+                    tg[kk] = fmaf(g, x[kk], tg[kk]);
+                    tz[kk] = fmaf(wz, x[kk], tz[kk]);
+                  }
+                }
+                s1[m] += t1;
+                s2[m] += t2;
+              }
+            } else if (kMode == 1) {
               if (kp < a.Cin) {
                 const float sc = s_scale[kp], sh = s_shift[kp];
                 const float *zp = a.z_prev + (size_t)p0 * a.Cin + kp;
@@ -702,6 +835,14 @@
             s2[m] = 0.f;
           }
         }
+        if constexpr (XK > 0) {
+#pragma unroll
+          for (int kk = 0; kk < XK; ++kk) {
+            dg[kk] += (double)tg[kk];
+            dzs[kk] += (double)tz[kk];
+            tg[kk] = tz[kk] = 0.f;
+          }
+        }
       }
       tc_fence_before();
       __syncwarp();
@@ -716,6 +857,18 @@
           atomicAdd(a.stats_prev + kp, d1[m]);
           atomicAdd(a.stats_prev + a.Cin + kp, d2[m]);
         }
+      }
+    }
+    if constexpr (XK > 0) {
+      const int kp = q * 32 + lane, K = a.Cin_prev;
+      if (ntiles > 0 && kp < a.Cin) {
+        double *S1 = a.thin_sums, *Sz = S1 + (size_t)a.Cin * K;
+#pragma unroll
+        for (int kk = 0; kk < XK; ++kk)
+          if (kk < K) {
+            atomicAdd(S1 + kp * K + kk, dg[kk]);
+            atomicAdd(Sz + kp * K + kk, dzs[kk]);
+          }
       }
     }
     if (ntiles > 0) {
@@ -839,6 +992,16 @@
   if (dbias_conv) dbias_conv[ch] = (float)(gs * S1 + count * (b * mu + (-gs * k1 - b * mu)));
 }
 
+__global__ void thin_fold_dw_kernel(const double *__restrict__ sums, const float *__restrict__ ca,
+                                    const float *__restrict__ cb, const float *__restrict__ cc,
+                                    int Cout, int K, float *__restrict__ dW) {
+  const int i = blockIdx.x * blockDim.x + threadIdx.x;
+  if (i >= Cout * K) return;
+  const int c = i / K, k = i - c * K;
+  const double *S1 = sums, *Sz = S1 + (size_t)Cout * K, *sx = Sz + (size_t)Cout * K;
+  dW[i] = (float)((double)ca[c] * S1[i] + (double)cb[c] * Sz[i] + (double)cc[c] * sx[k]);
+}
+
 }
 
 }
@@ -862,14 +1025,14 @@
 
 namespace {
 int bwd_pick_nt(const Geometry &g, int Cout, int mode, int top, int do_dgrad, int NS, long long M,
-                long long per_scene, int cmp = 0) {
+                long long per_scene, int cmp = 0, int thin = 0) {
   const int MTp = (g.KA + 1) >> 1, MTl = g.Cout_pad >> 7;
   if (MTp > 3) return 0;
   for (int nt : {128, 64, 32}) {
     if (M % nt) continue;
     if (!cmp && mode == 0 && per_scene % nt) continue;
     if (top && (nt % NS) != 0 && (NS % nt) != 0) continue;
-    const BwdSmem L = bwd_smem_layout(g.Kp, g.KA, g.WA, Cout, g.Cout_pad, nt, top, cmp);
+    const BwdSmem L = bwd_smem_layout(g.Kp, g.KA, g.WA, Cout, g.Cout_pad, nt, top, cmp, thin);
     const int w12 = ((top && MTl > (do_dgrad ? MTp : 0)) ? MTl : (do_dgrad ? MTp : 0)) * nt;
     const int cols = 2 * w12 + MTl * g.KA * 64;
     if (L.total <= 227u * 1024u && cols <= 512) return nt;
@@ -932,6 +1095,7 @@
   a.xyz = d->xyz; a.new_xyz = d->new_xyz; a.feat_t = d->feat_t; a.idx = d->idx;
   a.radius = d->radius; a.normalize_xyz = d->normalize_xyz;
   a.z_prev = d->z_prev; a.scale_prev = d->scale_prev; a.shift_prev = d->shift_prev;
+  a.w_prev = d->w_image_prev; a.Cin_prev = d->Cin_prev; a.thin_sums = d->thin_sums;
   a.w_image = d->w_image_bf16;
   a.dz = d->dz; a.gr = d->gr; a.z = d->z; a.dysel = d->dysel; a.asel = d->asel;
   a.coef_a = d->coef_a; a.coef_b = d->coef_b; a.coef_c = d->coef_c;
@@ -958,6 +1122,13 @@
                 "b2r_sa_layer_bwd: gather mode needs xyz, new_xyz, idx (and feat_t when Cin > 3)");
     a.do_dgrad = (d->g_feat_t != nullptr && d->Cin > 3) || d->g_xyz != nullptr ||
                  d->g_new_xyz != nullptr;
+  } else if (d->w_image_prev != nullptr) {
+    B2R_REQUIRE(d->scale_prev && d->shift_prev && d->thin_sums && !a.top && d->Cin <= 128 &&
+                    d->Cin_prev >= 3 && d->Cin_prev <= 4 && d->xyz && d->new_xyz &&
+                    (d->idx || cmp) && (d->feat_t || d->Cin_prev == 3),
+                "b2r_sa_layer_bwd: a layer above a thin first layer needs scale/shift, thin_sums, "
+                "a non-pooled layer with Cin <= 128, 3 <= Cin_prev <= 4 and the gather inputs");
+    a.do_dgrad = 1;
   } else {
     B2R_REQUIRE(d->z_prev && d->scale_prev && d->shift_prev,
                 "b2r_sa_layer_bwd: dense mode needs z_prev/scale/shift");
@@ -975,23 +1146,34 @@
               "(Cin=%d Cout=%d)", d->Cin, d->Cout);
     return B2R_ERR_UNSUPPORTED;
   }
-  const int NT = bwd_pick_nt(g, d->Cout, d->mode, a.top, a.do_dgrad, d->NS, M, per_scene, cmp);
+  const int xk = d->mode == 1 && d->w_image_prev != nullptr ? 4 : 0;
+  const int NT =
+      bwd_pick_nt(g, d->Cout, d->mode, a.top, a.do_dgrad, d->NS, M, per_scene, cmp, xk > 0);
   if (NT == 0) {
     set_error("b2r_sa_layer_bwd: layer Cin=%d Cout=%d M=%lld does not fit shared memory / TMEM",
               d->Cin, d->Cout, M);
     return B2R_ERR_UNSUPPORTED;
   }
-  const BwdSmem L = bwd_smem_layout(a.Kp, a.KA, a.WA, a.Cout, a.Cout_pad, NT, a.top, cmp);
+  const BwdSmem L = bwd_smem_layout(a.Kp, a.KA, a.WA, a.Cout, a.Cout_pad, NT, a.top, cmp, xk > 0);
   a.num_tiles = (int)(M / NT);
   int sms = kNumSMs;
   if (d->sm_limit > 0 && d->sm_limit < kNumSMs) sms = d->sm_limit;
   const int grid = a.num_tiles < sms ? a.num_tiles : sms;
   cudaStream_t st = static_cast<cudaStream_t>(stream);
-#define B2R_LAUNCH_BWD2(NTV, EWV, MV, TV, CV)                                                   \
+#define B2R_LAUNCH_BWD3(NTV, EWV, MV, TV, CV, XKV)                                              \
   do {                                                                                          \
-    B2R_CUDA(cudaFuncSetAttribute(sa_layer_bwd_kernel<NTV, EWV, MV, TV, CV>,                    \
+    B2R_CUDA(cudaFuncSetAttribute(sa_layer_bwd_kernel<NTV, EWV, MV, TV, CV, XKV>,               \
                                   cudaFuncAttributeMaxDynamicSharedMemorySize, (int)L.total));  \
-    sa_layer_bwd_kernel<NTV, EWV, MV, TV, CV><<<grid, kBwdThreads, L.total, st>>>(a);           \
+    sa_layer_bwd_kernel<NTV, EWV, MV, TV, CV, XKV><<<grid, kBwdThreads, L.total, st>>>(a);      \
+  } while (0)
+#define B2R_LAUNCH_BWD2(NTV, EWV, MV, TV, CV) B2R_LAUNCH_BWD3(NTV, EWV, MV, TV, CV, 0)
+#define B2R_LAUNCH_THIN1(NTV, XKV)                                                              \
+  do {                                                                                          \
+    if (cmp) B2R_LAUNCH_BWD3(NTV, 4, 1, 0, true, XKV); else B2R_LAUNCH_BWD3(NTV, 4, 1, 0, false, XKV); \
+  } while (0)
+#define B2R_LAUNCH_THIN(NTV)                                                                    \
+  do {                                                                                          \
+    B2R_LAUNCH_THIN1(NTV, 4);                                                                   \
   } while (0)
 #define B2R_LAUNCH_BWD1(NTV, EWV, MV, TV)                                                       \
   do {                                                                                          \
@@ -1005,12 +1187,29 @@
       if (a.mode == 0) B2R_LAUNCH_BWD1(NTV, 4, 0, 0); else B2R_LAUNCH_BWD1(NTV, 4, 1, 0);       \
     }                                                                                           \
   } while (0)
-  if (NT == 128) B2R_LAUNCH_BWD(128, 8);
+  if (xk > 0) {
+    if (NT == 128) B2R_LAUNCH_THIN(128);
+    else if (NT == 64) B2R_LAUNCH_THIN(64);
+    else B2R_LAUNCH_THIN(32);
+  } else if (NT == 128) B2R_LAUNCH_BWD(128, 8);
   else if (NT == 64) B2R_LAUNCH_BWD(64, 8);
   else B2R_LAUNCH_BWD(32, 4);
 #undef B2R_LAUNCH_BWD
 #undef B2R_LAUNCH_BWD1
 #undef B2R_LAUNCH_BWD2
+#undef B2R_LAUNCH_BWD3
+#undef B2R_LAUNCH_THIN
+#undef B2R_LAUNCH_THIN1
+  B2R_CHECK_LAUNCH();
+  return B2R_OK;
+}
+
+extern "C" int b2r_thin_fold_dw(const double *thin_sums, const float *coef_a, const float *coef_b,
+                                const float *coef_c, int Cout, int K, float *dW, void *stream) {
+  B2R_REQUIRE(thin_sums && coef_a && coef_b && coef_c && dW && Cout > 0 && K > 0,
+              "b2r_thin_fold_dw: bad argument");
+  thin_fold_dw_kernel<<<ceil_div(Cout * K, 256), 256, 0, static_cast<cudaStream_t>(stream)>>>(
+      thin_sums, coef_a, coef_b, coef_c, Cout, K, dW);
   B2R_CHECK_LAUNCH();
   return B2R_OK;
 }
diff --git a/backtoreality_b200/csrc/mlp_common.cuh b/backtoreality_b200/csrc/mlp_common.cuh
--- a/backtoreality_b200/csrc/mlp_common.cuh
+++ b/backtoreality_b200/csrc/mlp_common.cuh
@@ -197,6 +197,88 @@
   return t;
 }
 
+struct ThinRowSrc {
+  long long base;
+  int p, c;
+};
+template <bool CMP, class A>
+__device__ __forceinline__ ThinRowSrc thin_row_src(const A &a, long long per_scene, long long pos) {
+  ThinRowSrc s;
+  if constexpr (CMP) {
+    s.base = 0;
+    s.p = __ldg(a.cidx + pos);
+    s.c = __ldg(a.ccen + pos);
+  } else {
+    s.base = (pos / per_scene) * a.N;
+    s.p = __ldg(a.idx + pos);
+    s.c = (int)(pos / a.NS);
+  }
+  return s;
+}
+template <int KM>
+struct ThinRowRaw {
+  float p[3], q[3], f[KM - 3];
+};
+template <int KM, class A>
+__device__ __forceinline__ ThinRowRaw<KM> thin_row_fetch(const A &a, int C, const ThinRowSrc &s) {
+  const size_t prow = (size_t)(s.base + s.p);
+  const long long centre = max(s.c, 0);
+  ThinRowRaw<KM> r;
+#pragma unroll
+  for (int e = 0; e < 3; ++e) {
+    r.p[e] = __ldg(a.xyz + prow * 3 + e);
+    r.q[e] = __ldg(a.new_xyz + (size_t)centre * 3 + e);
+  }
+  const float *ff = a.feat_t + prow * C;
+#pragma unroll
+  for (int c = 0; c < KM - 3; ++c) r.f[c] = c < C ? __ldg(ff + c) : 0.f;
+  return r;
+}
+template <int KM, class A>
+__device__ __forceinline__ void thin_row_finish(const A &a, const ThinRowRaw<KM> &r,
+                                                float (&x)[KM]) {
+#pragma unroll
+  for (int e = 0; e < 3; ++e) {
+    const float d = __fsub_rn(r.p[e], r.q[e]);
+    x[e] = a.normalize_xyz ? __fdiv_rn(d, a.radius) : d;
+  }
+#pragma unroll
+  for (int c = 0; c < KM - 3; ++c) x[3 + c] = r.f[c];
+}
+template <int KM, bool CMP, class A>
+__device__ __forceinline__ void gather_thin_row(const A &a, int C, long long per_scene,
+                                                long long pos, float (&x)[KM]) {
+  thin_row_finish<KM>(a, thin_row_fetch<KM>(a, C, thin_row_src<CMP>(a, per_scene, pos)), x);
+}
+template <int KM>
+__device__ __forceinline__ void round_tf32(float (&x)[KM]) {
+#pragma unroll
+  for (int k = 0; k < KM; ++k) x[k] = __uint_as_float(to_tf32(x[k]));
+}
+
+template <int KM>
+__device__ __forceinline__ float thin_z(const float (&w)[KM], const float (&xr)[KM], int K) {
+  float s = 0.f;
+#pragma unroll
+  for (int k = 0; k < KM; ++k)
+    if (k < K) s = fmaf(w[k], xr[k], s);
+  return s;
+}
+
+__device__ __forceinline__ void load_thin_weights(const float *w_image, int Cout, int K,
+                                                  float *s_w0, int tid, int nthreads) {
+  const int Cf4 = (K - 3 + 3) & ~3, Cout_pad = (Cout + 127) & ~127;
+  for (int i = tid; i < Cout * 8; i += nthreads) {
+    const int c = i >> 3, k = i & 7;
+    float v = 0.f;
+    if (k < K) {
+      const int kp = k < 3 ? Cf4 + k : k - 3;
+      v = w_image[(sw128_off(c, kp >> 2, Cout_pad) >> 2) + (kp & 3)];
+    }
+    s_w0[k * Cout + c] = v;
+  }
+}
+
 inline int pow2_shift(int v) {
   if (v < 1 || (v & (v - 1))) return -1;
   int s = 0;
@@ -207,6 +289,7 @@
 }
 
 namespace thin {
+bool recompute_ok(int B, int NP, int NS, int Cin, int Cout);
 bool fwd_applicable(const b2r_sa_layer *d);
 int fwd_launch(const b2r_sa_layer *d, void *stream);
 bool bwd_applicable(const b2r_sa_layer_bwd_desc *d);
diff --git a/backtoreality_b200/csrc/mlp_thin.cu b/backtoreality_b200/csrc/mlp_thin.cu
--- a/backtoreality_b200/csrc/mlp_thin.cu
+++ b/backtoreality_b200/csrc/mlp_thin.cu
@@ -31,30 +31,7 @@
 
 template <int KM, bool CMP>
 __device__ __forceinline__ void gather_row(const ThinArgs &a, long long pos, float (&x)[KM]) {
-  size_t prow;
-  long long centre;
-  if constexpr (CMP) {
-    prow = (size_t)__ldg(a.cidx + pos);
-    centre = max(__ldg(a.ccen + pos), 0);
-  } else {
-    const int b = (int)(pos / a.per_scene);
-    centre = pos / a.NS;
-    prow = (size_t)b * a.N + __ldg(a.idx + pos);
-  }
-  const float *pp = a.xyz + prow * 3;
-  const float *qq = a.new_xyz + (size_t)centre * 3;
-  float d0 = __fsub_rn(__ldg(pp), __ldg(qq));
-  float d1 = __fsub_rn(__ldg(pp + 1), __ldg(qq + 1));
-  float d2 = __fsub_rn(__ldg(pp + 2), __ldg(qq + 2));
-  if (a.normalize_xyz) {
-    d0 = __fdiv_rn(d0, a.radius);
-    d1 = __fdiv_rn(d1, a.radius);
-    d2 = __fdiv_rn(d2, a.radius);
-  }
-  x[0] = d0; x[1] = d1; x[2] = d2;
-  const float *ff = a.feat_t + prow * a.C;
-#pragma unroll
-  for (int c = 0; c < KM - 3; ++c) x[3 + c] = c < a.C ? __ldg(ff + c) : 0.f;
+  mlp::gather_thin_row<KM, CMP>(a, a.C, a.per_scene, pos, x);
 }
 
 template <int LP, int KM, bool CMP>
@@ -102,7 +79,7 @@
       p64 = (int)(pos0 & 63);
     }
     float ts[4] = {0, 0, 0, 0}, tss[4] = {0, 0, 0, 0};
-    float *zrow = a.z + (size_t)pos0 * a.Cout + c4;
+    float *zrow = a.z != nullptr ? a.z + (size_t)pos0 * a.Cout + c4 : nullptr;
 #pragma unroll 4
     for (int it = 0; it < ITERS; ++it) {
       const int src = it * PPW + sub;
@@ -128,8 +105,9 @@
           tss[e] = fmaf(s, s, tss[e]);
         }
       }
-      stg_stream_v4(reinterpret_cast<float4 *>(zrow + (size_t)src * a.Cout),
-                    make_float4(zz[0], zz[1], zz[2], zz[3]));
+      if (zrow != nullptr)
+        stg_stream_v4(reinterpret_cast<float4 *>(zrow + (size_t)src * a.Cout),
+                      make_float4(zz[0], zz[1], zz[2], zz[3]));
     }
 #pragma unroll
     for (int e = 0; e < 4; ++e) {
@@ -277,6 +255,11 @@
   return (int)(want < cap ? want : cap);
 }
 
+}
+
+bool recompute_ok(int B, int NP, int NS, int Cin, int Cout) {
+  return B > 0 && NP > 0 && NS > 0 && Cin <= 4 &&
+         shape_ok(Cin, Cout, (long long)B * NP * NS, (long long)NP * NS);
 }
 
 bool fwd_applicable(const b2r_sa_layer *d) {
diff --git a/backtoreality_b200/fused_sa.py b/backtoreality_b200/fused_sa.py
--- a/backtoreality_b200/fused_sa.py
+++ b/backtoreality_b200/fused_sa.py
@@ -154,7 +154,7 @@
 
 
 def sa_mlp_forward(xyz, new_xyz, feat_t, idx, radius, normalize_xyz, mlp_module, training,
-                   want_point_major=True, save=None, sm_limit=0, plan=None):
+                   want_point_major=True, save=None, sm_limit=0, plan=None, recompute_first=False):
     lib = _lib.lib()
     st = _ext._stream()
     dev = xyz.device
@@ -164,6 +164,8 @@
     rows = M if plan is None else int(plan["cidx"].shape[0])
     blocks = list(mlp_module)
     L = len(blocks)
+    thin0 = bool(recompute_first and L >= 3 and lib.b2r_sa_thin_recompute(
+        B, NP, NS, blocks[0].conv.in_channels, blocks[0].conv.out_channels))
     z_prev = scale = shift = None
     zs, bn_saved, images = [], [], []
     stats_all = None
@@ -188,11 +190,13 @@
         d.B, d.N, d.NP, d.NS, d.Cin, d.Cout = B, N, NP, NS, Cin, Cout
         d.mode = 0 if i == 0 else 1
         d.epilogue = 1 if last else 0
-        if i == 0:
+        if i == 0 or (i == 1 and thin0):
             d.xyz, d.new_xyz, d.feat_t, d.idx = _ptr(xyz), _ptr(new_xyz), _ptr(feat_t), _ptr(idx)
             d.radius, d.normalize_xyz = float(radius), 1 if normalize_xyz else 0
-        else:
+        if i > 0:
             d.z_prev, d.scale_prev, d.shift_prev = _ptr(z_prev), _ptr(scale), _ptr(shift)
+        if i == 1 and thin0:
+            d.w_image_prev, d.Cin_prev = _ptr(images[0]), blocks[0].conv.in_channels
         d.w_image = _ptr(image)
         d.sm_limit = int(sm_limit)
         if plan is not None:
@@ -204,12 +208,13 @@
             amax = torch.empty((B * NP, Cout), dtype=torch.int32, device=dev)
             amin = torch.empty_like(amax)
             d.zmax, d.zmin, d.amax, d.amin = _ptr(zmax), _ptr(zmin), _ptr(amax), _ptr(amin)
-        else:
+        elif not (i == 0 and thin0):
             z = torch.empty((rows, Cout), dtype=torch.float32, device=dev)
             d.z = _ptr(z)
         d.stats = _ptr(stats)
-        with _ext._timed("sa_layer_fwd", _layer_work(B, N, NP, NS, Cin, Cout, i == 0, last, False)):
-            _lib.check(lib.b2r_sa_layer_fwd(ctypes.byref(d), st), "sa_layer_fwd")
+        if not (i == 0 and thin0 and stats is None):
+            with _ext._timed("sa_layer_fwd", _layer_work(B, N, NP, NS, Cin, Cout, i == 0, last, False)):
+                _lib.check(lib.b2r_sa_layer_fwd(ctypes.byref(d), st), "sa_layer_fwd")
         if training:
             scale = torch.empty(Cout, dtype=torch.float32, device=dev)
             shift = torch.empty_like(scale)
@@ -238,7 +243,7 @@
     _ext.LAUNCHES += 1
     if save is not None:
         save.update(zs=zs, bn=bn_saved, zmax=zmax, zmin=zmin, amax=amax, amin=amin, images=images,
-                    plan=plan)
+                    plan=plan, thin0=thin0)
     return out_cm, out_pm
 
 
@@ -268,6 +273,7 @@
     rows = M if plan is None else int(plan["cidx"].shape[0])
     L = len(weights)
     zs, bn, images = saved["zs"], saved["bn"], saved["images"]
+    thin0 = saved.get("thin0", False)
     f32 = dict(dtype=torch.float32, device=dev)
     dWs, dgammas, dbetas = [None] * L, [None] * L, [None] * L
     tr = 1 if training else 0
@@ -298,7 +304,7 @@
 
     g_feat_t = g_xyz = g_new_xyz = None
     gr = None
-    for l in range(L - 1, -1, -1):
+    for l in range(L - 1, 0 if thin0 else -1, -1):
         Cout, Cin = weights[l].shape[0], weights[l].shape[1]
         b = _lib.SaLayerBwd()
         b.B, b.N, b.NP, b.NS, b.Cin, b.Cout = B, N, NP, NS, Cin, Cout
@@ -315,9 +321,11 @@
         b.dW = _ptr(dWs[l])
         need_dgrad = True
         gr_prev = stats_prev = None
-        if l == 0:
+        thin_sums = None
+        if l == 0 or (l == 1 and thin0):
             b.xyz, b.new_xyz, b.feat_t, b.idx = _ptr(xyz), _ptr(new_xyz), _ptr(feat_t), _ptr(idx)
             b.radius, b.normalize_xyz = float(radius), 1 if normalize_xyz else 0
+        if l == 0:
             if need_feat and feat_t is not None:
                 g_feat_t = step_arena.zeros_like(feat_t)
                 b.g_feat_t = _ptr(g_feat_t)
@@ -330,9 +338,15 @@
             need_dgrad = g_feat_t is not None or need_xyz or need_new_xyz
         else:
             b.z_prev, b.scale_prev, b.shift_prev = _ptr(zs[l - 1]), _ptr(bn[l - 1][2]), _ptr(bn[l - 1][3])
-            gr_prev = torch.empty((rows, Cin), **f32)
+            if l == 1 and thin0:
+                K0 = weights[0].shape[1]
+                thin_sums = step_arena.zeros(2 * Cin * K0 + K0, dtype=torch.float64, device=dev)
+                b.w_image_prev, b.Cin_prev, b.thin_sums = _ptr(images[0]), K0, _ptr(thin_sums)
+            else:
+                gr_prev = torch.empty((rows, Cin), **f32)
+                b.gr_prev = _ptr(gr_prev)
             stats_prev = stats_all[s_off[l - 1]:s_off[l]]
-            b.gr_prev, b.stats_prev = _ptr(gr_prev), _ptr(stats_prev)
+            b.stats_prev = _ptr(stats_prev)
         image = None
         if need_dgrad or l == top:
             image = _take(versioned[l], "bf16") if versioned is not None else None
@@ -351,6 +365,12 @@
                                                _ptr(dgammas[l - 1]), _ptr(dbetas[l - 1]), st),
                        "bn_bwd_finalize")
             _ext.LAUNCHES += 1
+            if thin_sums is not None:
+                dWs[0] = dW_all[w_off[0]:w_off[1]].view(Cin, K0)
+                _lib.check(lib.b2r_thin_fold_dw(_ptr(thin_sums), _ptr(coef[0]), _ptr(coef[1]),
+                                                _ptr(coef[2]), Cin, K0, _ptr(dWs[0]), st),
+                           "thin_fold_dw")
+                _ext.LAUNCHES += 1
             gr = gr_prev
     return g_feat_t, g_xyz, g_new_xyz, dWs, dgammas, dbetas
 
@@ -373,7 +393,8 @@
         fwd_limit, bwd_limit = sm_limit if isinstance(sm_limit, tuple) else (sm_limit, 0)
         out_cm, out_pm = sa_mlp_forward(xyz, new_xyz, feat_t, idx, radius, normalize_xyz,
                                         mlp_module, training, want_point_major=bool(want_pm),
-                                        save=save, sm_limit=fwd_limit, plan=plan)
+                                        save=save, sm_limit=fwd_limit, plan=plan,
+                                        recompute_first=not any(ctx.needs_input_grad[:4]))
         ctx.set_materialize_grads(False)
         if need:
             ctx.saved = (xyz, new_xyz, feat_t, idx, float(radius), bool(normalize_xyz),
diff --git a/include/b2r.h b/include/b2r.h
--- a/include/b2r.h
+++ b/include/b2r.h
@@ -108,6 +108,8 @@
   int *amax, *amin;
   int sm_limit;
   const int *cidx, *ccen, *cmeta;
+  const float *w_image_prev;
+  int Cin_prev;
 } b2r_sa_layer;
 
 B2R_API long long b2r_mlp_weight_image_bytes(int Cout, int Cin, int gather);
@@ -116,6 +118,7 @@
 B2R_API int b2r_sa_layer_fwd(const b2r_sa_layer *desc, void *stream);
 B2R_API int b2r_sa_layer_fwd_supported(int B, int NP, int NS, int Cin, int Cout, int gather,
                                        int pooled);
+B2R_API int b2r_sa_thin_recompute(int B, int NP, int NS, int Cin, int Cout);
 
 B2R_API int b2r_sa_layer_fwd_tile(int B, int NP, int NS, int Cin, int Cout, int gather, int pooled,
                                   int compact);
@@ -154,12 +157,17 @@
   float *g_new_xyz;
   int sm_limit;
   const int *cidx, *ccen, *cmeta;
+  const float *w_image_prev;
+  int Cin_prev;
+  double *thin_sums;
 } b2r_sa_layer_bwd_desc;
 
 B2R_API long long b2r_mlp_weight_bf16_image_bytes(int Cout, int Cin, int gather);
 B2R_API int b2r_mlp_pack_weight_bf16(const float *w, int Cout, int Cin, int gather, void *image,
                                      void *stream);
 B2R_API int b2r_sa_layer_bwd(const b2r_sa_layer_bwd_desc *desc, void *stream);
+B2R_API int b2r_thin_fold_dw(const double *thin_sums, const float *coef_a, const float *coef_b,
+                             const float *coef_c, int Cout, int K, float *dW, void *stream);
 B2R_API int b2r_sa_layer_bwd_supported(int B, int NP, int NS, int Cin, int Cout, int gather,
                                        int top);
 
```

Measured after the change: 2321, median of 6. 5.3% lower.
